# FofanovLab/mtsv_tools

Measured on AMD Instinct MI355X. Metric: reads/sec (whole node), 150bp reads vs MG-index, higher is better.
Workload: dtype u32/i16

## Files before the change

### include/mtsv_amd.h

```cpp
#ifndef MTSV_AMD_H
#define MTSV_AMD_H

#include <stddef.h>
#include <stdint.h>

#ifdef __cplusplus
extern "C" {
#endif

#define MTSV_OK 0
#define MTSV_E_ARG (-1)
#define MTSV_E_IO (-2)
#define MTSV_E_FORMAT (-3)
#define MTSV_E_DEVICE (-4)
#define MTSV_E_LIMIT (-5)
#define MTSV_E_NOMEM (-6)

typedef struct mtsv_index mtsv_index;
typedef struct mtsv_batch mtsv_batch;

typedef struct {
    double edit_rate;
    uint32_t seed_size;
    uint32_t seed_interval;
    double min_seed;
    uint64_t max_hits;
    uint64_t tune_max_hits;
    int64_t max_assignments;
    int64_t max_candidates;
} mtsv_params;

typedef struct {
    uint64_t read;
    uint32_t tax_id;
    uint32_t gi;
    uint32_t edit;
    uint8_t strand;
    uint8_t _pad[3];
    uint64_t offset;
} mtsv_hit;

typedef struct {
    uint64_t n;
    uint64_t n_bins;
    uint32_t occ_k;
    uint64_t sa_s;
    uint64_t file_bytes;
    uint64_t device_bytes;
    uint32_t kmer_k;
    uint32_t sa_full;
} mtsv_index_info_t;

#define MTSV_N_STAGES 8
typedef struct {
    float stage_ms[MTSV_N_STAGES];
    uint64_t n_reads;
    uint64_t n_seed_slots;
    uint64_t n_seed_hits;
    uint64_t lf_steps;
    uint64_t n_candidates;
    uint64_t n_verified;
    uint64_t window_bytes;
    uint64_t n_hits;
    uint64_t n_passes;
    uint64_t n_rounds;
    uint64_t n_lanes;
    uint64_t sw_cell_pairs;
    float sw_prefilter_ms;
    float sw_sweep_ms;
    uint64_t n_sw_passed;
    float sw_diag_ms;
    float sw_bound_ms;
    float edit_ms;
    uint64_t myers_columns;
    uint64_t n_sw_bound_refuted;
    uint64_t verify_turns;
    uint64_t verify_lanes_max;
    uint64_t myers_grid_max;
    uint64_t n_seed_tile_passes;
} mtsv_batch_stats;

const char *mtsv_last_error(void);
const char *mtsv_version(void);
void mtsv_params_default(mtsv_params *p);

int mtsv_device_count(void);

int mtsv_index_load(const char *path, mtsv_index **out);
int mtsv_index_build(uint64_t n_seqs, const uint32_t *tax_ids, const uint32_t *gis,
                     const uint8_t *const *seqs, const uint64_t *seq_lens, uint32_t occ_k,
                     uint64_t sa_s, int n_threads, mtsv_index **out);
int mtsv_index_build_fasta(const char *fasta_path, uint32_t occ_k, uint64_t sa_s, int n_threads,
                           mtsv_index **out);
int mtsv_set_build_device(int hip_device);
int mtsv_index_write(const mtsv_index *ix, const char *path);
int mtsv_index_info(const mtsv_index *ix, mtsv_index_info_t *info);
void mtsv_index_free(mtsv_index *ix);

#define MTSV_DEV_DEFAULT 0u
#define MTSV_DEV_SAMPLED_SA_ONLY 1u
#define MTSV_DEV_NO_KMER_TABLE 2u
#define MTSV_DEV_PACK_ON_DEVICE 4u
int mtsv_index_to_device(mtsv_index *ix, int hip_device, uint32_t flags);


#define MTSV_DEVPART_HEADER 0
#define MTSV_DEVPART_BLOCKS 1
#define MTSV_DEVPART_TEXT 2
#define MTSV_DEVPART_SA_SAMPLE 3
#define MTSV_DEVPART_BINS 4
#define MTSV_DEVPART_BIN_END 5
#define MTSV_DEVPART_BIN_LUT 6
typedef struct {
    uint32_t n, n_blocks;
    uint32_t C[5];
    uint32_t sentinel_row;
    uint32_t sa_s, sa_pow2_shift;
    uint32_t n_bins, bin_lut_shift;
    uint32_t kmer_k;
    uint32_t sa_full;
    uint32_t packed_on_device;
    uint32_t _pad;
    uint64_t device_bytes;
    float pack_ms, copy_ms, accel_build_ms;
    float _pad2;
} mtsv_device_header;
int mtsv_index_download_device(mtsv_index *ix, int hip_device, int part, void **out, uint64_t *bytes);

int mtsv_bin_batch(mtsv_index *ix, int hip_device, const uint8_t *bases, const uint64_t *read_off,
                   uint64_t n_reads, const mtsv_params *params, mtsv_hit **hits, uint64_t *n_hits);
void mtsv_hits_free(mtsv_hit *hits);
void *mtsv_host_alloc(size_t bytes);
void mtsv_host_free(void *p);
int mtsv_host_register(void *p, size_t bytes);
int mtsv_host_unregister(void *p);
int mtsv_bin_batch_multi(mtsv_index *ix, const int *devices, int n_devices, const uint8_t *bases,
                         const uint64_t *read_off, uint64_t n_reads, const mtsv_params *params,
                         mtsv_hit **hits, uint64_t *n_hits);
int mtsv_bin_batch_chunks(mtsv_index *const *chunks, const int *devices, int n_chunks,
                          const uint8_t *bases, const uint64_t *read_off, uint64_t n_reads,
                          const mtsv_params *params, mtsv_hit **hits, uint64_t *n_hits);
uint64_t mtsv_bin_batch_workspace_reads(uint64_t n_reads);

int mtsv_batch_create(mtsv_index *ix, int hip_device, uint64_t max_reads, uint64_t max_bases,
                      uint64_t max_hits_ws, mtsv_batch **out);
int mtsv_batch_create_lanes(mtsv_index *ix, int hip_device, uint64_t max_reads, uint64_t max_bases,
                            uint64_t max_hits_ws, int lanes, mtsv_batch **out);
int mtsv_batch_reserve_host(mtsv_batch *b, uint64_t n_reads, uint64_t n_bases, uint32_t warm_read_len);
#define MTSV_VERIFY_REFERENCE 0
#define MTSV_VERIFY_EDIT_FIRST 1
int mtsv_batch_set_verify_mode(mtsv_batch *b, int mode);
int mtsv_set_default_verify_mode(int mode);
int mtsv_batch_upload(mtsv_batch *b, const uint8_t *bases, const uint64_t *read_off,
                      uint64_t n_reads);
int mtsv_batch_run(mtsv_batch *b, const mtsv_params *params);
int mtsv_batch_run_host(mtsv_batch *b, const uint8_t *bases, const uint64_t *read_off,
                        uint64_t n_reads, const mtsv_params *params);
int mtsv_batch_run_host_parts(mtsv_batch *b, int n_parts, const uint8_t *const *bases, const uint64_t *const *read_off,
                              const uint64_t *n_reads, const mtsv_params *params);
int mtsv_batch_stats_get(const mtsv_batch *b, mtsv_batch_stats *st);

typedef struct {
    uint32_t tax_id;
    uint32_t _pad;
    uint64_t only_hit, only_best, tied_best, not_best;
} mtsv_taxon_stats;
int mtsv_batch_set_taxa_report(mtsv_batch *b, int on);
int mtsv_batch_taxa_report(mtsv_batch *b, mtsv_taxon_stats **rows, uint64_t *n_rows, uint64_t *total_reads,
                           float *device_ms, int reset);
int mtsv_merge_taxa_reports(const mtsv_taxon_stats *a, uint64_t n_a, const mtsv_taxon_stats *b, uint64_t n_b,
                            mtsv_taxon_stats **out, uint64_t *n_out);
int mtsv_format_taxa_report(const mtsv_taxon_stats *rows, uint64_t n_rows, uint64_t total_reads, char **out,
                            uint64_t *out_len);

#define MTSV_MATCH_OFF 0
#define MTSV_MATCH_WITH_HITS 1
#define MTSV_MATCH_ONLY 2
int mtsv_batch_set_match_flags(mtsv_batch *b, int mode);
int mtsv_batch_match_flags(mtsv_batch *b, uint64_t **words, uint64_t *n_reads, uint64_t *n_matched);

#define MTSV_KEEP_UNMATCHED 0
#define MTSV_KEEP_MATCHED 1
int mtsv_batch_take_reads(mtsv_batch *dst, mtsv_batch *src, int keep, uint64_t *n_kept, uint64_t *bases_kept,
                          float *device_ms);
int mtsv_batch_copy_reads(mtsv_batch *dst, mtsv_batch *src, float *device_ms);
int mtsv_batch_merge_runs(mtsv_batch *dst, mtsv_batch *const *srcs, int n_srcs, float *device_ms);
int mtsv_batch_read_map(mtsv_batch *b, uint64_t **map, uint64_t *n_reads);
int mtsv_batch_download_reads(mtsv_batch *b, uint8_t **codes, uint64_t **read_off, uint64_t *n_reads);
int mtsv_batch_download(mtsv_batch *b, mtsv_hit **hits, uint64_t *n_hits);

typedef struct {
    uint64_t read;
    uint32_t tax_id;
    uint32_t edit;
} mtsv_assignment;
#define MTSV_ASSIGN_OFF 0
#define MTSV_ASSIGN_WITH_HITS 1
#define MTSV_ASSIGN_ONLY 2
int mtsv_batch_set_assignments(mtsv_batch *b, int mode);
int mtsv_batch_download_assignments(mtsv_batch *b, mtsv_assignment **a, uint64_t *n, float *device_ms);
#define MTSV_GRAIN_TAXID 0
#define MTSV_GRAIN_TAXID_GI 1
#define MTSV_GRAIN_LONG 2
int mtsv_batch_set_assignment_grain(mtsv_batch *b, int grain);
typedef struct {
    uint64_t read;
    uint32_t tax_id, gi, offset, edit;
} mtsv_assignment_gi;
int mtsv_batch_download_assignments_gi(mtsv_batch *b, mtsv_assignment_gi **a, uint64_t *n, float *device_ms);
void mtsv_batch_free(mtsv_batch *b);

typedef struct mtsv_fold mtsv_fold;
int mtsv_fold_create(int hip_device, int grain, mtsv_fold **out);
void mtsv_fold_free(mtsv_fold *f);
int mtsv_fold_reset(mtsv_fold *f, uint64_t n_reads);
int mtsv_fold_add_run(mtsv_fold *f, mtsv_batch *src, float *device_ms);
int mtsv_fold_add_records(mtsv_fold *f, const void *records, uint64_t n, float *device_ms);
int mtsv_fold_count(const mtsv_fold *f, uint64_t *n);
int mtsv_fold_download(mtsv_fold *f, mtsv_assignment **a, uint64_t *n);
int mtsv_fold_download_gi(mtsv_fold *f, mtsv_assignment_gi **a, uint64_t *n);
int mtsv_fold_taxa_report(mtsv_fold *f, mtsv_taxon_stats **rows, uint64_t *n_rows, uint64_t *total_reads, float *device_ms);
int mtsv_fold_match_flags(mtsv_fold *f, uint64_t **words, uint64_t *n_reads, uint64_t *n_matched);

int mtsv_fold_add_text(mtsv_fold *f, const char *hits, const uint64_t *line_off, const uint32_t *line_read, uint64_t n_lines,
                       uint64_t *n_tokens, uint64_t *n_records, float *device_ms);

int mtsv_fold_format_text(mtsv_fold *f, const char *ids, const uint64_t *id_off, uint64_t n_reads, char **text, uint64_t *len,
                          float *device_ms);
int mtsv_batch_format_text(mtsv_batch *b, const char *ids, const uint64_t *id_off, uint64_t n_reads, char **text, uint64_t *len,
                           float *device_ms);

typedef struct mtsv_dupmap mtsv_dupmap;
int mtsv_dupmap_create(int hip_device, mtsv_dupmap **out);
void mtsv_dupmap_free(mtsv_dupmap *m);
int mtsv_batch_take_unique(mtsv_batch *dst, mtsv_batch *src, mtsv_dupmap *m, uint64_t *n_unique, uint64_t *bases_kept,
                           float *device_ms);
int mtsv_dupmap_download(const mtsv_dupmap *m, uint64_t **read, uint64_t **rep, uint64_t *n_reads, uint64_t *n_unique);
int mtsv_fold_expand(mtsv_fold *dst, mtsv_fold *src, const mtsv_dupmap *m, float *device_ms);

#define MTSV_RANK_UNKNOWN 0xffffffffu
typedef struct mtsv_taxonomy mtsv_taxonomy;
typedef struct {
    uint64_t n_nodes;
    uint64_t n_implied_roots;
    uint32_t n_ranks;
    uint32_t max_depth;
} mtsv_taxonomy_info_t;
int mtsv_taxonomy_load(const char *nodes_dmp, mtsv_taxonomy **out);
void mtsv_taxonomy_free(mtsv_taxonomy *tx);
int mtsv_taxonomy_info(const mtsv_taxonomy *tx, mtsv_taxonomy_info_t *info);
int mtsv_taxonomy_parent(const mtsv_taxonomy *tx, uint32_t tax_id, uint32_t *parent, uint32_t *rank);
const char *mtsv_taxonomy_rank_name(const mtsv_taxonomy *tx, uint32_t rank);
typedef struct {
    uint32_t tax_id, parent_tax_id, rank, depth;
    uint64_t direct, clade;
} mtsv_clade_stats;
int mtsv_fold_lca(mtsv_fold *f, const mtsv_taxonomy *tx, uint32_t edit_slack, mtsv_fold *out, mtsv_clade_stats **rows,
                  uint64_t *n_rows, uint64_t *total_reads, float *device_ms);
int mtsv_format_clade_report(const mtsv_clade_stats *rows, uint64_t n_rows, uint64_t total_reads, const mtsv_taxonomy *tx,
                             char **out, uint64_t *out_len);

#define MTSV_PAIR_BOTH 0
#define MTSV_PAIR_EITHER 1
#define MTSV_PAIR_PROPER 2
typedef struct {
// ... 42 lines not shown
```

### mtsv_tools_amd/__init__.py

```python
from ._lib import (
    ASSIGN_DTYPE,
    ASSIGN_GI_DTYPE,
    ASSIGN_OFF,
    ASSIGN_ONLY,
    ASSIGN_WITH_HITS,
    CLADE_STATS_DTYPE,
    Coverage,
    DEVPART_BIN_END,
    DEVPART_BIN_LUT,
    DEVPART_BINS,
    DEVPART_BLOCKS,
    DEVPART_HEADER,
    DEVPART_SA_SAMPLE,
    DEVPART_TEXT,
    DeviceHeader,
    GRAIN_LONG,
    GRAIN_TAXID,
    GRAIN_TAXID_GI,
    HIT_DTYPE,
    KEEP_MATCHED,
    KEEP_UNMATCHED,
    MATCH_OFF,
    MATCH_ONLY,
    MATCH_WITH_HITS,
    RANK_UNKNOWN,
    REF_COVERAGE_DTYPE,
    SLACK_ALL,
    TAXON_STATS_DTYPE,
    Taxonomy,
    HostBuffer,
    host_register,
    host_unregister,
    Batch,
    DupMap,
    Fold,
    MGIndex,
    MtsvError,
    PAIR_BOTH,
    PAIR_EITHER,
    PAIR_PROPER,
    PairStats,
    Params,
    bin_batch_chunks,
    bin_batch_multi,
    bin_batch_slice_reads,
    default_params,
    device_count,
    format_assignments,
    format_assignments_gi,
    format_clade_report,
    format_coverage_report,
    format_results,
    format_taxa_report,
    merge_taxa_reports,
    lib,
    lib_path,
    pack_bases,
    set_build_device,
    synth_reads,
    version,
)

DEV_DEFAULT = 0
DEV_SAMPLED_SA_ONLY = 1
DEV_NO_KMER_TABLE = 2
DEV_PACK_ON_DEVICE = 4
```

### mtsv_tools_amd/_lib.py

```python
import ctypes as C
import os

import numpy as np

_HERE = os.path.dirname(os.path.abspath(__file__))


def lib_path():
    return os.environ.get("MTSV_AMD_LIB") or os.path.join(_HERE, "libmtsv_amd.so")


class MtsvError(RuntimeError):
    def __init__(self, code, msg):
        super().__init__(f"mtsv error {code}: {msg}")
        self.code = code


E_ARG, E_IO, E_FORMAT, E_DEVICE, E_LIMIT, E_NOMEM = -1, -2, -3, -4, -5, -6
MATCH_OFF, MATCH_WITH_HITS, MATCH_ONLY = 0, 1, 2
ASSIGN_OFF, ASSIGN_WITH_HITS, ASSIGN_ONLY = 0, 1, 2
GRAIN_TAXID, GRAIN_TAXID_GI, GRAIN_LONG = 0, 1, 2
KEEP_UNMATCHED, KEEP_MATCHED = 0, 1
DEVPART_HEADER, DEVPART_BLOCKS, DEVPART_TEXT, DEVPART_SA_SAMPLE, DEVPART_BINS, DEVPART_BIN_END, DEVPART_BIN_LUT = range(7)


class Params(C.Structure):
    _fields_ = [("edit_rate", C.c_double), ("seed_size", C.c_uint32), ("seed_interval", C.c_uint32),
                ("min_seed", C.c_double), ("max_hits", C.c_uint64), ("tune_max_hits", C.c_uint64),
                ("max_assignments", C.c_int64), ("max_candidates", C.c_int64)]


class IndexInfo(C.Structure):
    _fields_ = [("n", C.c_uint64), ("n_bins", C.c_uint64), ("occ_k", C.c_uint32),
                ("sa_s", C.c_uint64), ("file_bytes", C.c_uint64), ("device_bytes", C.c_uint64),
                ("kmer_k", C.c_uint32), ("sa_full", C.c_uint32)]


class DeviceHeader(C.Structure):
    _fields_ = [("n", C.c_uint32), ("n_blocks", C.c_uint32), ("C", C.c_uint32 * 5), ("sentinel_row", C.c_uint32),
                ("sa_s", C.c_uint32), ("sa_pow2_shift", C.c_uint32), ("n_bins", C.c_uint32), ("bin_lut_shift", C.c_uint32),
                ("kmer_k", C.c_uint32), ("sa_full", C.c_uint32), ("packed_on_device", C.c_uint32), ("_pad", C.c_uint32),
                ("device_bytes", C.c_uint64), ("pack_ms", C.c_float), ("copy_ms", C.c_float), ("accel_build_ms", C.c_float),
                ("_pad2", C.c_float)]


N_STAGES = 8
STAGE_NAMES = ("search", "thin_scan", "expand", "locate", "coalesce", "verify", "gather", "total")


class BatchStats(C.Structure):
    _fields_ = [("stage_ms", C.c_float * N_STAGES), ("n_reads", C.c_uint64),
                ("n_seed_slots", C.c_uint64), ("n_seed_hits", C.c_uint64), ("lf_steps", C.c_uint64),
                ("n_candidates", C.c_uint64), ("n_verified", C.c_uint64),
                ("window_bytes", C.c_uint64), ("n_hits", C.c_uint64), ("n_passes", C.c_uint64),
                ("n_rounds", C.c_uint64), ("n_lanes", C.c_uint64), ("sw_cell_pairs", C.c_uint64), ("sw_prefilter_ms", C.c_float),
                ("sw_sweep_ms", C.c_float), ("n_sw_passed", C.c_uint64), ("sw_diag_ms", C.c_float), ("sw_bound_ms", C.c_float),
                ("edit_ms", C.c_float), ("myers_columns", C.c_uint64), ("n_sw_bound_refuted", C.c_uint64),
                ("verify_turns", C.c_uint64), ("verify_lanes_max", C.c_uint64), ("myers_grid_max", C.c_uint64),
                ("n_seed_tile_passes", C.c_uint64)]

    def as_dict(self):
        d = {n: (float(getattr(self, n)) if t is C.c_float else int(getattr(self, n))) for n, t in self._fields_[1:]}
        d["stage_ms"] = {STAGE_NAMES[i]: float(self.stage_ms[i]) for i in range(N_STAGES)}
        return d


HIT_DTYPE = np.dtype({"names": ["read", "tax_id", "gi", "edit", "strand", "offset"],
                      "formats": ["<u8", "<u4", "<u4", "<u4", "u1", "<u8"],
                      "offsets": [0, 8, 12, 16, 20, 24], "itemsize": 32})

TAXON_STATS_DTYPE = np.dtype({"names": ["tax_id", "only_hit", "only_best", "tied_best", "not_best"],
                              "formats": ["<u4", "<u8", "<u8", "<u8", "<u8"],
                              "offsets": [0, 8, 16, 24, 32], "itemsize": 40})

ASSIGN_DTYPE = np.dtype({"names": ["read", "tax_id", "edit"], "formats": ["<u8", "<u4", "<u4"], "offsets": [0, 8, 12], "itemsize": 16})

ASSIGN_GI_DTYPE = np.dtype({"names": ["read", "tax_id", "gi", "offset", "edit"], "formats": ["<u8", "<u4", "<u4", "<u4", "<u4"],
                            "offsets": [0, 8, 12, 16, 20], "itemsize": 24})

CLADE_STATS_DTYPE = np.dtype({"names": ["tax_id", "parent_tax_id", "rank", "depth", "direct", "clade"],
                              "formats": ["<u4", "<u4", "<u4", "<u4", "<u8", "<u8"], "offsets": [0, 4, 8, 12, 16, 24], "itemsize": 32})
RANK_UNKNOWN = 0xffffffff
SLACK_ALL = 0xffffffff
PAIR_BOTH, PAIR_EITHER, PAIR_PROPER = 0, 1, 2

REF_COVERAGE_DTYPE = np.dtype({"names": ["tax_id", "gi", "length", "reads", "alignments", "aligned_bases", "covered_bases"],
                               "formats": ["<u4", "<u4", "<u8", "<u8", "<u8", "<u8", "<u8"], "offsets": [0, 4, 8, 16, 24, 32, 40], "itemsize": 48})


class TaxonomyInfo(C.Structure):
    _fields_ = [("n_nodes", C.c_uint64), ("n_implied_roots", C.c_uint64), ("n_ranks", C.c_uint32), ("max_depth", C.c_uint32)]


class PairStats(C.Structure):
    _fields_ = [("pairs", C.c_uint64), ("both_mates_hit", C.c_uint64), ("one_mate_hit", C.c_uint64), ("joined", C.c_uint64),
                ("records", C.c_uint64)]

    def as_dict(self):
        return {n: int(getattr(self, n)) for n, _ in self._fields_}


EXPORTS = [
    "mtsv_last_error", "mtsv_version", "mtsv_params_default", "mtsv_device_count",
    "mtsv_index_load", "mtsv_index_build", "mtsv_index_build_fasta", "mtsv_index_write",
    "mtsv_index_info", "mtsv_index_free", "mtsv_set_build_device", "mtsv_index_to_device", "mtsv_bin_batch",
    "mtsv_hits_free", "mtsv_batch_create", "mtsv_batch_upload", "mtsv_batch_run", "mtsv_batch_run_host", "mtsv_batch_run_host_parts",
    "mtsv_batch_stats_get", "mtsv_batch_set_verify_mode", "mtsv_batch_download", "mtsv_batch_free", "mtsv_format_results",
    "mtsv_free", "mtsv_synth_index", "mtsv_synth_reads", "mtsv_bin_batch_workspace_reads",
    "mtsv_bin_batch_multi", "mtsv_bin_batch_chunks", "mtsv_set_default_verify_mode",
    "mtsv_host_alloc", "mtsv_host_free", "mtsv_host_register", "mtsv_host_unregister",
    "mtsv_batch_create_lanes", "mtsv_batch_reserve_host", "mtsv_pack_bases", "mtsv_host_pack_threads",
    "mtsv_batch_set_taxa_report", "mtsv_batch_taxa_report", "mtsv_merge_taxa_reports", "mtsv_format_taxa_report",
    "mtsv_batch_set_match_flags", "mtsv_batch_match_flags",
    "mtsv_batch_take_reads", "mtsv_batch_read_map", "mtsv_batch_download_reads",
    "mtsv_batch_copy_reads", "mtsv_batch_merge_runs",
    "mtsv_batch_set_assignments", "mtsv_batch_download_assignments", "mtsv_format_assignments",
    "mtsv_batch_set_assignment_grain", "mtsv_batch_download_assignments_gi", "mtsv_format_assignments_gi",
    "mtsv_fold_create", "mtsv_fold_free", "mtsv_fold_reset", "mtsv_fold_add_run", "mtsv_fold_add_records", "mtsv_fold_count",
    "mtsv_fold_download", "mtsv_fold_download_gi", "mtsv_fold_taxa_report", "mtsv_fold_match_flags",
    "mtsv_fold_format_text", "mtsv_batch_format_text",
    "mtsv_index_download_device",
    "mtsv_fold_add_text",
    "mtsv_taxonomy_load", "mtsv_taxonomy_free", "mtsv_taxonomy_info", "mtsv_taxonomy_parent", "mtsv_taxonomy_rank_name",
    "mtsv_fold_lca", "mtsv_format_clade_report",
    "mtsv_dupmap_create", "mtsv_dupmap_free", "mtsv_batch_take_unique", "mtsv_dupmap_download", "mtsv_fold_expand",
    "mtsv_fold_pair",
    "mtsv_coverage_create", "mtsv_coverage_free", "mtsv_coverage_add_index", "mtsv_coverage_add_refs", "mtsv_coverage_reset",
    "mtsv_coverage_add_fold", "mtsv_coverage_rows", "mtsv_format_coverage_report",
]

_lib = None


def lib():
    global _lib
    if _lib is None:
        p = lib_path()
        if not os.path.exists(p):
            raise MtsvError(E_DEVICE, f"{p} is missing: run `make -C mtsv_tools_amd/csrc` "
                                      "(or __graft_entry__.build()); there is no fallback path")
        L = C.CDLL(p)
        vp, u64, u32, i32 = C.c_void_p, C.c_uint64, C.c_uint32, C.c_int
        L.mtsv_last_error.restype = C.c_char_p
        L.mtsv_version.restype = C.c_char_p
        L.mtsv_params_default.argtypes = [C.POINTER(Params)]
        L.mtsv_index_load.argtypes = [C.c_char_p, C.POINTER(vp)]
        L.mtsv_index_build.argtypes = [u64, vp, vp, vp, vp, u32, u64, i32, C.POINTER(vp)]
        L.mtsv_index_build_fasta.argtypes = [C.c_char_p, u32, u64, i32, C.POINTER(vp)]
        L.mtsv_index_write.argtypes = [vp, C.c_char_p]
        L.mtsv_index_info.argtypes = [vp, C.POINTER(IndexInfo)]
        L.mtsv_index_free.argtypes = [vp]
        L.mtsv_index_free.restype = None
        L.mtsv_index_to_device.argtypes = [vp, i32, u32]
        L.mtsv_index_download_device.argtypes = [vp, i32, i32, C.POINTER(vp), C.POINTER(u64)]
        L.mtsv_bin_batch.argtypes = [vp, i32, vp, vp, u64, C.POINTER(Params), C.POINTER(vp),
                                     C.POINTER(u64)]
        L.mtsv_hits_free.argtypes = [vp]
        L.mtsv_hits_free.restype = None
        L.mtsv_bin_batch_multi.argtypes = [vp, vp, i32, vp, vp, u64, C.POINTER(Params), C.POINTER(vp), C.POINTER(u64)]
        L.mtsv_bin_batch_chunks.argtypes = [vp, vp, i32, vp, vp, u64, C.POINTER(Params), C.POINTER(vp), C.POINTER(u64)]
        L.mtsv_bin_batch_workspace_reads.argtypes = [u64]
        L.mtsv_bin_batch_workspace_reads.restype = u64
        L.mtsv_batch_create.argtypes = [vp, i32, u64, u64, u64, C.POINTER(vp)]
        L.mtsv_batch_create_lanes.argtypes = [vp, i32, u64, u64, u64, i32, C.POINTER(vp)]
        L.mtsv_batch_reserve_host.argtypes = [vp, u64, u64, u32]
        L.mtsv_pack_bases.argtypes = [vp, vp, u64, u64, C.c_uint8]
        L.mtsv_pack_bases.restype = C.c_uint8
        L.mtsv_batch_upload.argtypes = [vp, vp, vp, u64]
        L.mtsv_batch_run.argtypes = [vp, C.POINTER(Params)]
        L.mtsv_batch_run_host.argtypes = [vp, vp, vp, u64, C.POINTER(Params)]
        L.mtsv_batch_run_host_parts.argtypes = [vp, i32, vp, vp, vp, C.POINTER(Params)]
        L.mtsv_batch_set_verify_mode.argtypes = [vp, i32]
        L.mtsv_batch_stats_get.argtypes = [vp, C.POINTER(BatchStats)]
        L.mtsv_batch_download.argtypes = [vp, C.POINTER(vp), C.POINTER(u64)]
        L.mtsv_batch_free.argtypes = [vp]
        L.mtsv_batch_free.restype = None
# ... 759 lines not shown
```

### mtsv_tools_amd/csrc/batch.hip

```cpp
#include <atomic>
#include <chrono>
#include <cmath>
#include <condition_variable>
#include <exception>
#include <mutex>
#include <thread>
#include <cstdio>
#include <cstdlib>
#include <cstring>
#include <stdexcept>
#include <vector>

#include "batch.hpp"

namespace mtsv {

namespace {
template <class F>
void parallel_ranges(uint64_t n, F f) {
    static const int max_nt = [] {
        const char* e = getenv("MTSV_COPY_THREADS");
        return e ? std::max(1, std::min(16, atoi(e))) : 4;
    }();
    const int nt = std::min(max_nt, n >= (32ull << 20) ? 4 : n >= (4ull << 20) ? 2 : 1);
    if (nt == 1) return f(0, n);
    std::vector<std::thread> th;
    const uint64_t chunk = ((n + nt - 1) / nt + 4095) & ~4095ull;
    for (int k = 0; k < nt; k++) {
        uint64_t a = std::min(n, chunk * k), b = std::min(n, chunk * (k + 1));
        if (a < b) th.emplace_back([=] { f(a, b); });
    }
    for (auto& t : th) t.join();
}
double now_s() { return std::chrono::duration<double>(std::chrono::steady_clock::now().time_since_epoch()).count(); }
void parallel_copy(uint8_t* dst, const uint8_t* src, uint64_t n) {
    parallel_ranges(n, [=](uint64_t a, uint64_t b) { memcpy(dst + a, src + a, b - a); });
}
}

bool host_pinned(const void* p, uint64_t bytes) {
    if (!p || !bytes) return false;
    for (const uint8_t* q : {(const uint8_t*)p, (const uint8_t*)p + bytes - 1}) {
        hipPointerAttribute_t at;
        memset(&at, 0, sizeof at);
        if (hipPointerGetAttributes(&at, q) != hipSuccess) {
            (void)hipGetLastError();
            return false;
        }
        if (at.type != hipMemoryTypeHost) return false;
    }
    return true;
}

void* host_pinned_alloc(uint64_t bytes) {
    void* p = nullptr;
    if (hipHostMalloc(&p, bytes ? bytes : 1, hipHostMallocPortable) != hipSuccess) {
        (void)hipGetLastError();
        return nullptr;
    }
    return p;
}
void host_pinned_free(void* p) {
    if (p && hipHostFree(p) != hipSuccess) (void)hipGetLastError();
}
bool host_pinned_register(void* p, uint64_t bytes) {
    if (hipHostRegister(p, bytes, hipHostRegisterPortable) == hipSuccess) return true;
    (void)hipGetLastError();
    return false;
}
bool host_pinned_unregister(void* p) {
    if (hipHostUnregister(p) == hipSuccess) return true;
    (void)hipGetLastError();
    return false;
}

int g_default_verify_mode = MTSV_VERIFY_REFERENCE;

constexpr uint32_t kMyersWgsPerCuLanes = 3;
constexpr uint64_t kChunkMaxReads = 4ull << 20;

Batch::Batch(mtsv_index* ix_, DeviceIndex* di_, uint64_t max_reads_, uint64_t max_bases_, uint64_t hit_cap_, Batch* parent_, int lanes_)
    : ix(ix_), di(di_), max_reads(max_reads_), max_bases(max_bases_), hit_cap(hit_cap_), parent(parent_) {
    if (max_reads == 0) max_reads = 1;
    if (max_reads > 0x7fffffffull) throw std::runtime_error("limit: more than 2^31 reads in one batch");
    if (max_bases >= 0xffffffffull) throw std::runtime_error("limit: 4 GiB of bases or more in one batch");
    const uint64_t hit_cap_user = hit_cap;
    if (!parent) {
        n_lanes = 3;
        if (lanes_ > 0) n_lanes = std::min(8, lanes_);
        else if (const char* e = getenv("MTSV_LANES")) n_lanes = std::max(1, std::min(8, atoi(e)));
        if (max_reads < (uint64_t)n_lanes * kLaneMinReads) n_lanes = 1;
    }
    ws_reads = (max_reads + n_lanes - 1) / n_lanes;
    if (!parent && n_lanes > 1) {
        uint64_t cmax = kChunkMaxReads;
        if (const char* e = getenv("MTSV_CHUNK")) cmax = std::max<uint64_t>(kLaneMinReads, strtoull(e, nullptr, 10));
        ws_reads = std::min(ws_reads, cmax);
    }
    if (hit_cap == 0) hit_cap = std::max<uint64_t>(1ull << 20, 32 * ws_reads);
    if (hit_cap > 0xfffffff0ull) hit_cap = 0xfffffff0ull;
    uint64_t hits_cap = std::max<uint64_t>(1ull << 20, 16 * ws_reads);
    if (const char* e = getenv("MTSV_HITS_CAP")) hits_cap = std::max<uint64_t>(1024, strtoull(e, nullptr, 10));
    HIP_CHECK(hipSetDevice(di->device));
    stream.create(hipStreamNonBlocking);
    const uint64_t ns = 2 * ws_reads;
    if (!parent) {
        d_bases.alloc(max_bases + 64, "the resident bases");
        d_read_off.alloc(max_reads + 1, "the resident read offsets");
        d_codes.alloc(max_bases + 64, "the resident codes");
    }
    d_strand_hits.alloc(ns + 1, "strands: seed hits");
    d_strand_nseeds.alloc(ns, "strands: seeds kept");
    d_strand_off.alloc(ns + 1, "strands: seed-hit offsets");
    d_strand_ncand.alloc(ns, "strands: candidates");
    d_strand_nout.alloc(ns + 1, "strands: hits");
    d_heavy_list.alloc(2 * ns, "strands: lists");
    d_out_off.alloc(ns + 1, "strands: hit offsets");
    d_tile_sums.alloc((uint64_t)scan_tiles((uint32_t)ns) + 1, "the scans' tile sums");
    d_counters.alloc(kCounters, "the pass counters");
    hit_cap_first = hit_cap;
    size_hit_workspace(hit_cap_first);
    d_hits.alloc(hits_cap, "the result array");
    h_counters.renew(kCounters, hipHostMallocMapped);
    if (const char* e = getenv("MTSV_SW")) sw_pairs = strcmp(e, "packed") != 0;
    if (const char* e = getenv("MTSV_SW_DIAG")) sw_diag = atoi(e) != 0;
    if (const char* e = getenv("MTSV_SW_PREPASS")) sw_prepass = atoi(e) != 0;
    if (const char* e = getenv("MTSV_SW_TOP")) sw_top = atoi(e) != 0;
    if (const char* e = getenv("MTSV_SW_BOUND")) sw_bound = atoi(e) != 0;
    if (const char* e = getenv("MTSV_SW_FUSED")) sw_fused = atoi(e) != 0;
    verify_mode = g_default_verify_mode;
    if (const char* e = getenv("MTSV_VERIFY")) verify_mode = !strcmp(e, "edit_first") ? 1 : 0;
    if (!parent) {
        myers_wgs_per_cu = n_lanes > 1 ? kMyersWgsPerCuLanes : kMyersWgsPerCuMax;
        if (const char* e = getenv("MTSV_MYERS_WGS_PER_CU")) myers_wgs_per_cu = (uint32_t)std::max(1, std::min((int)kMyersWgsPerCuMax, atoi(e)));
        verify_turn.on = n_lanes > 1;
        if (const char* e = getenv("MTSV_VERIFY_TURN")) verify_turn.on = verify_turn.on && atoi(e) != 0;
        if (const char* e = getenv("MTSV_TAIL_FROM_LIST")) tail_from_list = atoi(e) != 0;
        if (const char* e = getenv("MTSV_FUSED_CLEAR")) fused_clear = atoi(e) != 0;
        if (const char* e = getenv("MTSV_SEED_STAGE")) seed_tiles = strcmp(e, "legacy") != 0;
    } else {
        myers_wgs_per_cu = parent->myers_wgs_per_cu;
        tail_from_list = parent->tail_from_list;
        fused_clear = parent->fused_clear;
        seed_tiles = parent->seed_tiles;
    }
    ev.create();
    for (int k = 1; k < n_lanes; k++) extra.emplace_back(new Batch(ix, di, ws_reads, 0, hit_cap_user, this));
}

Batch::~Batch() {
    extra.clear();
    (void)hipSetDevice(di->device);
    for (hipStream_t s : {stream.s, copy_stream.s, copy_stream2.s})
        if (s) (void)hipStreamSynchronize(s);
    if (h_hits_stage) pinned_hits_release(h_hits_stage);
    if (h_assign_stage) pinned_hits_release(h_assign_stage);
}

void Batch::size_hit_workspace(uint64_t cap) {
    hit_cap = 0;
    release_all(d_hit_row, d_hit_ref, d_hit_q, d_hit_key, d_cand_tmp, d_cand, d_out, d_cand_next, d_cand_status, d_worklist);
    d_hit_row.alloc(cap, "hit workspace: rows");
    d_hit_ref.alloc(cap, "hit workspace: references");
    d_hit_q.alloc(cap, "hit workspace: read positions");
    d_hit_key.alloc(cap, "hit workspace: keys");
    d_cand_tmp.alloc(2 * cap, "hit workspace: candidate scratch");
    d_cand.alloc(cap, "hit workspace: candidates");
    d_out.alloc(cap, "hit workspace: verified candidates");
    d_cand_next.alloc(cap, "hit workspace: successors");
    d_cand_status.alloc(cap, "hit workspace: status");
    d_worklist.alloc(cap, "hit workspace: work list");
    hit_cap = cap;
}

void Batch::grow_hit_workspace(uint64_t need) {
    if (getenv("MTSV_TRACE")) fprintf(stderr, "[workspace] seed-hit arrays grow %llu -> %llu entries\n", (unsigned long long)hit_cap, (unsigned long long)need);
    HIP_CHECK(hipStreamSynchronize(stream));
    size_hit_workspace(need);
}

void Batch::VerifyTurn::enter(uint64_t first_read, const Batch* lane) {
    std::unique_lock<std::mutex> lk(mu);
    if (on) {
        const std::pair<uint64_t, const Batch*> me{first_read, lane};
        waiting.push_back(me);
        cv.wait(lk, [&] { return !held && *std::min_element(waiting.begin(), waiting.end()) == me; });
        waiting.erase(std::find(waiting.begin(), waiting.end(), me));
        held = true;
        taken++;
    }
    max_in_verify = std::max(max_in_verify, ++in_verify);
}

void Batch::VerifyTurn::leave() {
    {
        std::lock_guard<std::mutex> lk(mu);
        in_verify--;
        held = false;
    }
    cv.notify_all();
}

void Batch::VerifyTurn::note_grid(uint32_t blocks) {
    std::lock_guard<std::mutex> lk(mu);
    myers_grid_max = std::max<uint64_t>(myers_grid_max, blocks);
}

void Batch::upload(const uint8_t* bases, const uint64_t* read_off, uint64_t n) {
    if (n > max_reads) throw std::runtime_error("arg: batch holds more reads than the workspace was created for");
    const uint64_t first = n ? read_off[0] : 0;
    const uint64_t nb = n ? read_off[n] - first : 0;
    if (nb > max_bases) throw std::runtime_error("arg: batch holds more bases than the workspace was created for");
    h_read_off.resize(n + 1);
    max_len = 0;
    for (uint64_t i = 0; i <= n; i++) {
        if (i && read_off[i] < read_off[i - 1]) throw std::runtime_error("arg: read_off is not ascending");
        h_read_off[i] = (uint32_t)(read_off[i] - first);
        if (i) max_len = std::max(max_len, h_read_off[i] - h_read_off[i - 1]);
    }
    if (n == 0) h_read_off[0] = 0;
    HIP_CHECK(hipSetDevice(di->device));
    if (nb) HIP_CHECK(hipMemcpyAsync(d_bases.p, bases + first, nb, hipMemcpyHostToDevice, stream));
    HIP_CHECK(hipMemcpyAsync(d_read_off.p, h_read_off.data(), (n + 1) * 4, hipMemcpyHostToDevice, stream));
    HIP_CHECK(hipStreamSynchronize(stream));
    n_reads = n;
    n_hits_total = 0;
    total_hits = 0;
    segments.clear();
    last_run = kRunNone;
    resident = true;
    codes_resident = mapped = false;
}

void Batch::reset_lane() {
    HIP_CHECK(hipSetDevice(di->device));
    memset(&stats, 0, sizeof stats);
    memset(stage_acc, 0, sizeof stage_acc);
    sw_ms_acc = 0;
    sweep_ms_acc = diag_ms_acc = bound_ms_acc = edit_ms_acc = 0;
    sw_passed_acc = 0;
    n_hits_total = 0;
    n_assign_total = 0;
    if (!hit_cap) size_hit_workspace(hit_cap_first);
    HIP_CHECK(hipMemsetAsync(d_counters.p, 0, kCounters * sizeof(uint64_t), stream));
    listed_zero = true;
    HIP_CHECK(hipEventRecord(ev[kEvRunBegin], stream));
}

void Batch::finish_lane() {
    HIP_CHECK(hipEventRecord(ev[kEvRunEnd], stream));
    launch_publish(stream, d_counters.p, h_counters.p, kCounters);
    HIP_CHECK(hipStreamSynchronize(stream));
    HIP_CHECK(hipEventElapsedTime(&stage_acc[7], ev[kEvRunBegin], ev[kEvRunEnd]));
    if (getenv("MTSV_TRACE")) fprintf(stderr, "[lane] last pass: %llu strands of 13..64 seed hits (or more than 4 candidates) to k_coalesce_mid, %llu heavier ones\n",
                                      (unsigned long long)(h_counters.p[kCtrMidStrands] & 0xffffffffull), (unsigned long long)(h_counters.p[kCtrWorklist] >> 32));
    if (getenv("MTSV_TRACE")) fprintf(stderr, "[lane] k_coalesce_heavy: %llu strands walked by runs, %llu by the wavefront walk (a run too long)\n",
                                      (unsigned long long)(h_counters.p[kCtrHeavyWalk] & 0xffffffffull), (unsigned long long)(h_counters.p[kCtrHeavyWalk] >> 32));
    stats.sw_cell_pairs = h_counters.p[kCtrSwCellPairs];
    stats.sw_prefilter_ms = sw_ms_acc;
    stats.sw_sweep_ms = sweep_ms_acc;
    stats.sw_diag_ms = diag_ms_acc;
    stats.sw_bound_ms = bound_ms_acc;
    stats.edit_ms = edit_ms_acc;
    stats.myers_columns = h_counters.p[kCtrMyersColumns];
    stats.n_sw_bound_refuted = h_counters.p[kCtrBoundRefuted];
    stats.n_sw_passed = sw_passed_acc + h_counters.p[kCtrListPassed];
    stats.lf_steps = h_counters.p[kCtrLfSteps];
    stats.n_candidates = h_counters.p[kCtrCandidates];
    stats.n_verified = h_counters.p[kCtrVerified];
    stats.window_bytes = h_counters.p[kCtrWindowBytes];
}

void Batch::begin_run(const mtsv_params& p, uint64_t read_base) {
    if (!(p.edit_rate >= 0.0 && p.edit_rate <= 1.0)) throw std::runtime_error("arg: edit_rate must be within [0, 1]");
    if (!(p.min_seed >= 0.0) || !std::isfinite(p.min_seed)) throw std::runtime_error("arg: min_seed must be finite and >= 0");
    if (p.seed_size == 0 || p.seed_interval == 0) throw std::runtime_error("arg: seed_size and seed_interval must be > 0");
    segments.clear();
    total_hits = 0;
    lanes_used = 1;
    staged_valid = false;
    assign_staged_valid = false;
    staged_assign = 0;
    host_hits_dropped = false;
    last_run = kRunNone;
    run_t0 = now_s();
    {
        std::lock_guard<std::mutex> lk(verify_turn.mu);
        verify_turn.taken = verify_turn.max_in_verify = verify_turn.myers_grid_max = 0;
    }
    reset_lane();
    for (auto& l : extra) {
        l->verify_mode = verify_mode;
        l->sw_pairs = sw_pairs;
        l->sw_diag = sw_diag;
        l->sw_prepass = sw_prepass;
        l->sw_top = sw_top;
        l->sw_bound = sw_bound;
// ... 1235 lines not shown
```

### mtsv_tools_amd/csrc/batch.hpp

```cpp
#pragma once
#include <condition_variable>
#include <memory>
#include <mutex>
#include <vector>

#include "../../include/mtsv_amd.h"
#include "host_pack.hpp"
#include "dev_index.hpp"
#include "dev_mem.hpp"
#include "kernels.hpp"

namespace mtsv {

struct Batch {
    mtsv_index* ix;
    DeviceIndex* di;
    DevStream stream, copy_stream, copy_stream2;
    mtsv_hit* h_hits_stage = nullptr;
    uint64_t h_hits_cap = 0, staged_hits = 0, last_total_hits = 0;
    bool staged_valid = false;
    struct Arena {
        DevBuf<uint8_t> d_bases;
        DevBuf<uint8_t> d_packed;
        DevBuf<uint32_t> d_off;
        uint64_t cap_bases = 0, cap_reads = 0;
        void resize(int k, uint64_t bases, uint64_t reads);
    };
    static constexpr uint64_t kArenaBases = 3ull << 30;
    static constexpr uint64_t kArenaReads = 1ull << 30;
    Arena arena[2];
    HostBuf<uint32_t> h_off_all;
    static constexpr int kStage = 4;
    HostBuf<uint8_t> h_stage[kStage];
    DevEventList chunk_ev;
    std::mutex* commit_mu = nullptr;
    uint64_t max_reads, max_bases;
    uint64_t hit_cap, hit_cap_first = 0;
    Batch* parent = nullptr;
    Batch* root() { return parent ? parent : this; }
    const Batch* root() const { return parent ? parent : this; }
    std::vector<std::unique_ptr<Batch>> extra;
    int n_lanes = 1;
    uint64_t ws_reads = 0;
    struct Segment {
        Batch* lane;
        uint64_t offset, count;
        uint64_t first_read = 0, n_reads = 0;
        uint64_t a_offset = 0, a_count = 0;
    };
    std::vector<Segment> segments;
    uint64_t total_hits = 0;
    double run_t0 = 0;
    uint64_t lanes_used = 1;

    DevBuf<uint8_t> d_codes;
    DevBuf<uint8_t> d_bases;
    DevBuf<uint32_t> d_read_off;
    DevBuf<uint32_t> d_seed_lo, d_seed_cnt, d_seed_pre;
    uint64_t seed_cap = 0;
    DevBuf<uint32_t> d_strand_hits, d_strand_nseeds, d_strand_off, d_strand_ncand, d_worklist, d_strand_nout, d_out_off;
    DevBuf<uint64_t> d_tile_sums;
    DevBuf<uint64_t> d_counters;
    DevBuf<uint32_t> d_hit_row, d_hit_ref, d_hit_q;
    DevBuf<uint64_t> d_hit_key, d_cand_tmp;
    DevBuf<uint4> d_cand, d_out;
    DevBuf<uint32_t> d_cand_next, d_cand_status, d_heavy_list;
    DevBuf<DevHit> d_hits;
    DevBuf<uint2> d_strip;
    DevBuf<uint32_t> d_planes;
    HostBuf<uint64_t> h_counters;
    enum Ev {
        kEvPassBegin = 0, kEvSearched, kEvSeeded, kEvExpanded, kEvLocated, kEvCoalesced, kEvVerified, kEvGathered,
        kEvRunBegin, kEvRunEnd,
        kEvSwBegin, kEvSwEnd,
        kEvDiagEnd,
        kEvBoundEnd,
        kEvEditEnd,
        kEvCount
    };
    DevEvents<kEvCount> ev;
    float sw_ms_acc = 0, sweep_ms_acc = 0, diag_ms_acc = 0, bound_ms_acc = 0, edit_ms_acc = 0;
    uint64_t sw_passed_acc = 0;

    std::vector<uint32_t> h_read_off;
    uint32_t max_len = 0;
    static constexpr int kCounters = kCtrCount;
    double listed_share = 0.125;
    bool sw_diag = true;
    bool sw_top = true;
    bool sw_bound = true;
    bool sw_fused = true;
    bool sw_prepass = true;
    bool sw_pairs = true;
    uint32_t myers_wgs_per_cu = kMyersWgsPerCuMax;
    bool tail_from_list = true;
    bool fused_clear = true;
    bool seed_tiles = true;
    bool listed_zero = false;
    struct VerifyTurn {
        bool on = false;
        std::mutex mu;
        std::condition_variable cv;
        bool held = false;
        std::vector<std::pair<uint64_t, const Batch*>> waiting;
        uint64_t taken = 0, in_verify = 0, max_in_verify = 0, myers_grid_max = 0;
        void enter(uint64_t first_read, const Batch* lane);
        void leave();
        void note_grid(uint32_t blocks);
        struct Guard {
            VerifyTurn* t = nullptr;
            Guard() = default;
            Guard(const Guard&) = delete;
            Guard& operator=(const Guard&) = delete;
            ~Guard() { release(); }
            void take(VerifyTurn& turn, uint64_t first_read, const Batch* lane) {
                if (t) return;
                turn.enter(first_read, lane);
                t = &turn;
            }
            void release() {
                if (t) t->leave();
                t = nullptr;
            }
        };
    };
    VerifyTurn verify_turn;
    int verify_mode = 0;
    uint64_t n_reads = 0;
    uint64_t n_hits_total = 0;
    mtsv_batch_stats stats{};
    float stage_acc[MTSV_N_STAGES] = {0};

    Batch(mtsv_index* ix, DeviceIndex* di, uint64_t max_reads, uint64_t max_bases, uint64_t hit_cap, Batch* parent = nullptr, int lanes = 0);
    ~Batch();
    Batch(const Batch&) = delete;
    Batch& operator=(const Batch&) = delete;

    void upload(const uint8_t* bases, const uint64_t* read_off, uint64_t n);
    void run(const mtsv_params& p);
    void run_host(const uint8_t* bases, const uint64_t* read_off, uint64_t n, const mtsv_params& p, uint64_t read_base = 0);
    struct HostPart {
        const uint8_t* bases;
        const uint64_t* read_off;
        uint64_t n;
    };
    void run_host_parts(const HostPart* parts, int n_parts, const mtsv_params& p, uint64_t read_base = 0);
    void reserve_host(uint64_t n, uint64_t n_bases);
    void download(mtsv_hit** hits, uint64_t* n);
    void download_into(mtsv_hit* dst, uint64_t n);
    bool keep_on_device = false;

    struct TaxaReport {
        bool on = false;
        bool dense = true;
        uint32_t hash_slots = kReportHashSlots;
        uint32_t n_taxa = 0;
        DevBuf<uint32_t> d_taxa;
        DevBuf<uint64_t> d_counts;
        bool trace = false;
        uint64_t launches = 0;
        std::vector<uint32_t> h_taxa;
        std::mutex mu;
        float ms = 0;
    };
    TaxaReport report;
    DevEvents<2> report_ev;
    void set_taxa_report(bool on);
    struct MatchFlags {
        int mode = MTSV_MATCH_OFF;
        DevBuf<uint64_t> d_words;
        uint64_t cap_words() const { return d_words.p ? d_words.cap - 1 : 0; }
        uint64_t n_reads = 0;
        uint64_t call_base = 0;
        bool trace = false;
        std::mutex mu;
        float ms = 0;
        uint64_t launches = 0;
    };
    MatchFlags match;
    DevEvents<2> match_ev;
    bool flags_only() const { return root()->match.mode == MTSV_MATCH_ONLY; }
    void set_match_flags(int mode);
    void match_flags(std::vector<uint64_t>& words, uint64_t* n_reads, uint64_t* n_matched);
    enum LastRun { kRunNone = 0, kRunResident, kRunHostOneSegment, kRunHostSegments, kRunMerged };
    int last_run = kRunNone;
    bool resident = false;
    bool codes_resident = false;
    bool mapped = false;
    DevBuf<uint32_t> d_read_map;
    DevBuf<uint64_t> d_compact;
    uint64_t compact_cap() const { return d_compact.p ? (d_compact.cap - 3) / 2 : 0; }
    DevEvents<4> compact_ev;
    void compact_room(uint64_t tiles);
    void take_reads(Batch& src, int keep, uint64_t* n_kept, uint64_t* bases_kept, float* device_ms);
    void copy_reads(Batch& src, float* device_ms);
    struct MergeState {
        DevBuf<uint32_t> d_nout, d_off;
        DevBuf<uint64_t> d_tiles;
        uint64_t cap_reads = 0;
        uint64_t cap_tiles() const { return d_tiles.cap - 2; }
        DevBuf<uint32_t> d_lo, d_base;
        uint64_t cap_sn = 0;
        DevBuf<MergePart> d_parts;
        DevEvents<2> ev;
    };
    MergeState merge;
    struct Assignments {
        int mode = MTSV_ASSIGN_OFF;
        int grain = MTSV_GRAIN_TAXID;
        uint64_t rec_bytes() const { return grain == MTSV_GRAIN_TAXID ? sizeof(mtsv_assignment) : sizeof(mtsv_assignment_gi); }
        uint64_t key_bytes() const { return grain == MTSV_GRAIN_TAXID ? 8 : 16; }
        uint32_t lane_max = kCollapseLaneMax, wave_max = 64, lds_max = kCollapseLdsKeys;
        bool trace = false;
        std::mutex mu;
        float ms = 0;
        uint64_t launches = 0;
        uint64_t tiers[5] = {0, 0, 0, 0, 0};
    };
    Assignments assign;
    uint8_t* h_assign_stage = nullptr;
    uint64_t h_assign_cap = 0, staged_assign = 0, last_total_assign = 0;
    bool assign_staged_valid = false;
    bool host_hits_dropped = false;
    void assign_stage_reserve(uint64_t n_needed);
    DevBuf<uint8_t> d_assign;
    uint64_t n_assign_total = 0;
    struct CollapseScratch {
        DevBuf<uint64_t> keys;
        uint64_t key_bytes = 0;
        DevBuf<uint32_t> flags, place;
        DevBuf<uint64_t> tiles;
        uint64_t cap_hits = 0;
        void resize(uint64_t hits, uint64_t key_bytes);
        DevBuf<uint32_t> list;
        uint64_t pending_hits = 0;
        DevBuf<uint64_t> d_ctr;
        HostBuf<uint64_t> h_ctr;
        DevEvents<2> ev;
    };
    CollapseScratch collapse;
    bool assign_only() const { return root()->assign.mode == MTSV_ASSIGN_ONLY; }
    void set_assignments(int mode);
    void set_assignment_grain(int grain);
    void download_assignments(void** a, uint64_t* n, float* device_ms, bool wide);
    std::shared_ptr<struct TextFormatter> text;
    void format_text(const char* ids, const uint64_t* id_off, uint64_t n_reads, char** text_out, uint64_t* len, float* device_ms);
    void merge_runs(Batch* const* srcs, int n_srcs, float* device_ms);
    void read_map(std::vector<uint64_t>& map);
    void download_reads(std::vector<uint8_t>& codes, std::vector<uint64_t>& read_off);
    void taxa_report(std::vector<mtsv_taxon_stats>& rows, uint64_t* total_reads, float* device_ms, bool reset);
// ... 61 lines not shown
```

### mtsv_tools_amd/csrc/batch_pass.hip

```cpp
#include <atomic>
#include <cstdio>
#include <cstdlib>
#include <thread>

#include "batch.hpp"

namespace mtsv {

void Batch::run_range(const mtsv_params& p, const uint8_t* raw, uint8_t* sb, const uint32_t* so, const uint32_t* h_off, uint64_t n,
                      uint32_t range_max_len, uint64_t read_base) {
    std::vector<Batch*> ls{this};
    for (auto& l : extra) ls.push_back(l.get());
    uint64_t per_lane = 2;
    if (const char* e = getenv("MTSV_CHUNKS_PER_LANE")) per_lane = std::max(1, atoi(e));
    const ChunkPlan cp = plan_chunks(n, ls.size(), ws_reads, per_lane);
    const uint64_t n_chunks = cp.n_chunks(), k = cp.k;
    lanes_used = std::max<uint64_t>(lanes_used, k);
    std::vector<Segment> segs(n_chunks);
    std::atomic<uint64_t> next{0};
    auto work = [&](Batch* lane) {
        for (;;) {
            const uint64_t c = next.fetch_add(1);
            if (c >= n_chunks) return;
            const uint64_t a = cp.bound[c], b = cp.bound[c + 1];
// ... 63 lines not shown
        if (getenv("MTSV_TRACE")) fprintf(stderr, "[lane] pass of %u reads, max_ns %u, longest read %u: seed stage %s\n", pl.nr, pl.max_ns, pl.pass_max_len, ps.tile_pass ? "by tiles" : "legacy");
        stats.n_seed_slots += pl.slots;
        stats.n_seed_hits += ps.total_hits;
        stage_locate(ps);
        stage_candidates(ps);
        stage_verify(ps);
        stage_gather(ps);
        stage_commit(ps);
        n_hits_total += ps.total_out;
        for (int s = 0; s < 7; s++) {
            float ms = 0;
            HIP_CHECK(hipEventElapsedTime(&ms, ev[s], ev[s + 1]));
            stage_acc[s] += ms;
        }
        r0 += pl.nr;
    }
}

void Batch::room_seed_slots(const PassPlan& pl) {
    if (pl.slots <= seed_cap) return;
    const uint64_t had = seed_cap;
    seed_cap = 0;
    release_all(d_seed_lo, d_seed_cnt, d_seed_pre);
    const uint64_t want = pl.tiled() ? pl.slots : std::max<uint64_t>(pl.slots, 2 * ws_reads * (uint64_t)pl.max_ns);
    if (getenv("MTSV_TRACE")) fprintf(stderr, "[workspace] seed slot arrays grow %llu -> %llu entries\n", (unsigned long long)had, (unsigned long long)want);
    d_seed_lo.alloc(want, "seed slots: ranges");
    d_seed_cnt.alloc(want, "seed slots: counts");
    d_seed_pre.alloc(want, "seed slots: prefix sums");
    seed_cap = want;
}

void Batch::room_planes(const PassPlan& pl) {
    if ((uint64_t)pl.nr * 3 * pl.plane_words <= d_planes.cap) return;
    d_planes.renew(std::max<uint64_t>(pl.nr, ws_reads) * 3 * pl.plane_words, "the reads' bit planes");
}

void Batch::room_strip(uint64_t need) {
    if (need <= d_strip.cap) return;
    d_strip.renew(need, "the band strips");
}

void Batch::room_hits(uint64_t total_out) {
    if (n_hits_total + total_out <= d_hits.cap) return;
    DevBuf<DevHit> grown;
    grown.alloc(std::max(d_hits.cap * 2, n_hits_total + total_out), "the result array");
    if (n_hits_total) HIP_CHECK(hipMemcpyAsync(grown.p, d_hits.p, n_hits_total * sizeof(DevHit), hipMemcpyDeviceToDevice, stream));
    HIP_CHECK(hipStreamSynchronize(stream));
    std::unique_lock<std::mutex> commit_lk;
    if (root()->commit_mu) commit_lk = std::unique_lock<std::mutex>(*root()->commit_mu);
    if (root()->copy_stream2) HIP_CHECK(hipStreamSynchronize(root()->copy_stream2));
    d_hits.swap(grown);
}

Batch::Seeded Batch::stage_seeds(Pass& ps) {
    const PassPlan& pl = ps.plan;
    const mtsv_params& p = ps.p;
    const uint32_t K = p.seed_size, G = p.seed_interval, r0 = (uint32_t)ps.r0;
    uint32_t* planes = pl.myers() ? d_planes.p : nullptr;
    HIP_CHECK(hipEventRecord(ev[kEvPassBegin], stream));
    const uint32_t listed_cap = (uint32_t)std::min<uint64_t>(pl.slots, std::max<uint64_t>(4096, (uint64_t)((double)pl.slots * listed_share)));
    launch_search(stream, di->view, ps.sb, ps.so, r0, pl.nr, pl.max_ns, K, G, d_seed_lo.p, d_seed_cnt.p, d_seed_pre.p, (uint32_t*)(d_counters.p + kCtrListedSlots),
                  listed_cap, di->d_kmer_levels, fused_clear && listed_zero);
    listed_zero = false;
    HIP_CHECK(hipEventRecord(ev[kEvSearched], stream));
    ps.tile_pass = seed_tiles && pl.max_ns && seed_tile_fits(pl.max_ns, pl.pass_max_len, pl.slots);
    if (ps.tile_pass)
        launch_thin_tiled(stream, ps.sb, ps.so, r0, pl.nr, p.edit_rate, p.min_seed, pl.max_ns, K, G, p.max_hits, p.tune_max_hits, d_seed_cnt.p,
                          d_strand_hits.p, d_strand_nseeds.p, planes, pl.plane_words);
    else if (pl.max_ns)
        launch_thin(stream, ps.sb, ps.so, r0, pl.nr, p.edit_rate, p.min_seed, pl.max_ns, K, G, p.max_hits, p.tune_max_hits, d_seed_cnt.p,
                    d_seed_pre.p, d_strand_hits.p, d_strand_nseeds.p, planes, pl.plane_words);
    else {
        HIP_CHECK(hipMemsetAsync(d_strand_hits.p, 0, (uint64_t)ps.nstr * 4, stream));
        HIP_CHECK(hipMemsetAsync(d_strand_nseeds.p, 0, (uint64_t)ps.nstr * 4, stream));
    }
    launch_scan(stream, d_strand_hits.p, ps.nstr, d_tile_sums.p, d_counters.p + kCtrSeedHits, d_strand_off.p);
    launch_publish(stream, d_counters.p + kCtrSeedHits, h_counters.p + kCtrSeedHits, 1);
    launch_publish(stream, d_counters.p + kCtrListedSlots, h_counters.p + kCtrListedSlots, 1);
    HIP_CHECK(hipEventRecord(ev[kEvSeeded], stream));
    HIP_CHECK(hipStreamSynchronize(stream));
    const uint64_t n_listed = h_counters.p[kCtrListedSlots] & 0xffffffffull;
    const double share = pl.slots ? (double)n_listed / (double)pl.slots : 0.0;
    if (n_listed > listed_cap) {
        listed_share = std::min(1.0, share * 1.25 + 0.01);
        if (getenv("MTSV_TRACE")) fprintf(stderr, "[lane] %llu listed seed slots, grid for %u: pass again\n", (unsigned long long)n_listed, listed_cap);
        return Seeded::kSameReads;
    }
    listed_share = std::min(1.0, std::max(0.02, share * 1.5 + 0.005));
    ps.total_hits = h_counters.p[kCtrSeedHits];
    if (ps.total_hits > hit_cap) {
        if (pl.nr > 1) return Seeded::kHalfReads;
        if (ps.total_hits > 0xfffffff0ull)
            throw std::runtime_error("device: one read has " + std::to_string(ps.total_hits) + " seed hits, more than 2^32");
        grow_hit_workspace(ps.total_hits);
    }
    return Seeded::kGoOn;
}

void Batch::stage_locate(Pass& ps) {
    const DevIndexView& v = di->view;
    if (ps.tile_pass)
        launch_expand_tiled(stream, v, ps.nstr, ps.plan.max_ns, ps.p.seed_interval, d_seed_lo.p, d_seed_cnt.p, d_strand_off.p, d_hit_row.p, d_hit_ref.p, d_hit_q.p);
    else
        launch_expand(stream, v, ps.nstr, ps.plan.max_ns, ps.p.seed_interval, d_seed_lo.p, d_seed_cnt.p, d_seed_pre.p, d_strand_off.p, d_hit_row.p, d_hit_ref.p,
                      d_hit_q.p);
    HIP_CHECK(hipEventRecord(ev[kEvExpanded], stream));
    if (!v.sa_full)
        launch_locate(stream, v, (uint32_t)ps.total_hits, d_strand_off.p + ps.nstr, d_hit_row.p, d_hit_ref.p,
                      (unsigned long long*)(d_counters.p + kCtrLfSteps));
    HIP_CHECK(hipEventRecord(ev[kEvLocated], stream));
}

void Batch::stage_candidates(Pass& ps) {
    if (fused_clear) {
        launch_clear_counters(stream, d_counters.p, kCtrClearPass | (ps.plan.path == VerifyPath::kRounds ? kCtrClearRound0 : 0));
        listed_zero = true;
    } else {
        HIP_CHECK(hipMemsetAsync(d_counters.p + kCtrWorklist, 0, 8, stream));
        HIP_CHECK(hipMemsetAsync(d_counters.p + kCtrWlCursor, 0, 8, stream));
        HIP_CHECK(hipMemsetAsync(d_counters.p + kCtrMidStrands, 0, 8, stream));
    }
    launch_coalesce(stream, di->view, ps.so, (uint32_t)ps.r0, ps.nstr, ps.p.max_candidates, d_strand_off.p,
                    d_strand_nseeds.p, d_hit_ref.p, d_hit_q.p, d_hit_key.p, d_cand_tmp.p, d_cand.p, d_cand_next.p,
                    d_cand_status.p, d_strand_ncand.p, d_worklist.p, d_heavy_list.p, d_counters.p, fused_clear);
    HIP_CHECK(hipEventRecord(ev[kEvCoalesced], stream));
}

void Batch::stage_verify(Pass& ps) {
    const DevIndexView& v = di->view;
    const PassPlan& pl = ps.plan;
    if (ps.total_hits) ps.turn.take(root()->verify_turn, ps.read_base + ps.r0, this);
    EvalArgs a;
    a.bases = ps.sb;
    a.read_off = ps.so;
    a.r0 = (uint32_t)ps.r0;
    a.edit_rate = ps.p.edit_rate;
    a.max_candidates = ps.p.max_candidates;
    a.strand_off = d_strand_off.p;
    a.cand = d_cand.p;
    a.cand_next = d_cand_next.p;
    a.cand_status = d_cand_status.p;
    a.planes = pl.myers() ? d_planes.p : nullptr;
    a.plane_words = pl.plane_words;
    a.out = d_out.p;
    a.n_verified = (unsigned long long*)(d_counters.p + kCtrVerified);
    a.window_bytes = (unsigned long long*)(d_counters.p + kCtrWindowBytes);
    a.sw_columns = (unsigned long long*)(d_counters.p + kCtrSwCellPairs);
    a.worklist = d_worklist.p;
    a.wl_count = (const uint32_t*)(d_counters.p + kCtrWorklist);
    a.wl_cursor = (uint32_t*)(d_counters.p + kCtrWlCursor);
    stats.n_rounds = 1;
    switch (pl.path) {
        case VerifyPath::kTiled: verify_tiled(ps, a); break;
        case VerifyPath::kEditFirst: root()->verify_turn.note_grid(launch_edit_myers(stream, v, a, ps.total_hits, pl.pass_max_len, 0, root()->myers_wgs_per_cu)); break;
        case VerifyPath::kRounds: verify_rounds(ps, a); break;
        case VerifyPath::kPacked: launch_evaluate(stream, v, a, ps.total_hits, pl.pass_max_len); break;
    }
    launch_resolve(stream, ps.nstr, ps.p.max_candidates, flags_only() ? 1 : ps.p.max_assignments, d_strand_off.p, d_strand_ncand.p, d_cand_status.p,
                   d_out.p, d_strand_nout.p);
    HIP_CHECK(hipEventRecord(ev[kEvVerified], stream));
}

void Batch::verify_tiled(Pass& ps, EvalArgs& a) {
    HIP_CHECK(hipMemsetAsync(d_counters.p + kCtrMaxWindow, 0, sizeof(uint64_t), stream));
    launch_max_window(stream, ps.nstr, d_strand_off.p, d_strand_ncand.p, d_cand.p, (unsigned long long*)(d_counters.p + kCtrMaxWindow));
    launch_publish(stream, d_counters.p + kCtrMaxWindow, h_counters.p + kCtrMaxWindow, 1);
    HIP_CHECK(hipStreamSynchronize(stream));
    const uint32_t strip_len = (uint32_t)std::max<uint64_t>(h_counters.p[kCtrMaxWindow], 1);
    room_strip((uint64_t)tiled_groups(ps.total_hits, strip_len) * strip_len);
    a.strip = d_strip.p;
    a.strip_len = strip_len;
    launch_evaluate_tiled(stream, di->view, a, ps.total_hits);
}

struct Batch::Round {
    uint32_t round = 0;
    uint64_t items = 0;
    uint64_t tail_items = 0;
    bool tail_listed = false;
    bool fused = false;
    EvalArgs sw;
    uint32_t *pass_list = nullptr, *sweep_list = nullptr, *next_list = nullptr;
    uint64_t* next_slot = nullptr;
};

void Batch::verify_rounds(Pass& ps, const EvalArgs& a) {
    Round r;
    r.fused = sw_bound && sw_fused;
    r.pass_list = (uint32_t*)d_hit_key.p;
    r.sweep_list = (uint32_t*)d_hit_key.p + hit_cap;
    uint32_t* next_lists[2] = {(uint32_t*)d_cand_tmp.p, (uint32_t*)d_cand_tmp.p + hit_cap};
    const uint32_t* wl = d_worklist.p;
    uint32_t wl_slot = kCtrWorklist;
    r.items = ps.total_hits;
    for (;; r.round++) {
        r.next_slot = d_counters.p + kCtrNext0 + (r.round & 1);
        r.next_list = next_lists[r.round & 1];
        if (!fused_clear) {
            HIP_CHECK(hipMemsetAsync(d_counters.p + kCtrSwCursor, 0, 3 * sizeof(uint64_t), stream));
            HIP_CHECK(hipMemsetAsync(r.next_slot, 0, sizeof(uint64_t), stream));
        } else if (r.round) {
            launch_clear_counters(stream, d_counters.p, ctr_clear_round(r.round));
        }
        r.tail_items = r.items;
        r.tail_listed = tail_from_list && r.round > 0;
        r.sw = a;
        r.sw.worklist = wl;
        r.sw.wl_count = (const uint32_t*)(d_counters.p + wl_slot);
        r.sw.wl_cursor = (uint32_t*)(d_counters.p + kCtrSwCursor);
        r.sw.wl_reverse = r.round == 0;
        r.sw.counters = d_counters.p;
        r.sw.wl_count_slot = wl_slot;
        r.sw.pass_list = r.pass_list;
        r.sw.pass_count = (uint32_t*)(d_counters.p + kCtrPassCount);
#ifdef MTSV_SW_HIST
        if (!d_strip.p) room_strip(4096);
        HIP_CHECK(hipMemsetAsync(d_strip.p, 0, 768 * 4, stream));
        r.sw.strip = d_strip.p;
#endif
        if (r.round == 0) {
            HIP_CHECK(hipEventRecord(ev[kEvSwBegin], stream));
            if (sw_diag && sw_prepass && !r.fused) round0_diag(ps, r);
            if (sw_bound) round0_bound(ps, r);
            else if (sw_diag && sw_prepass && sw_top) round0_top(ps, r);
        }
        round_tail(ps, r, a);
        if (r.round == 0) round0_times();
        const uint64_t n_next = h_counters.p[kCtrNext0] & 0xffffffffull;
        if (n_next == 0) break;
        stats.n_rounds++;
        wl = r.next_list;
        wl_slot = kCtrNext0 + (r.round & 1);
        r.items = n_next;
    }
    ps.turn.release();
}

void Batch::round0_diag(Pass& ps, Round& r) {
    HIP_CHECK(hipMemsetAsync(d_counters.p + kCtrSweepCount, 0, sizeof(uint64_t), stream));
    launch_sw_diag(stream, di->view, r.sw, r.items, ps.plan.pass_max_len, r.sweep_list, kCtrSweepCount);
    HIP_CHECK(hipEventRecord(ev[kEvDiagEnd], stream));
    r.sw.worklist = r.sweep_list;
    r.sw.wl_count_slot = kCtrSweepCount;
    r.sw.wl_reverse = 0;
}

void Batch::round0_bound(Pass& ps, Round& r) {
    if (!fused_clear) HIP_CHECK(hipMemsetAsync(d_counters.p + kCtrUndecided, 0, 2 * sizeof(uint64_t), stream));
    EvalArgs bd = r.sw;
    bd.wl_count = (const uint32_t*)(d_counters.p + r.sw.wl_count_slot);
    bd.wl_cursor = (uint32_t*)(d_counters.p + kCtrBoundCursor);
    bd.und_list = (uint32_t*)d_hit_row.p;
    bd.und_slot = kCtrUndecided;
    bd.myers_ctr = (unsigned long long*)(d_counters.p + kCtrMyersColumns);
    root()->verify_turn.note_grid(launch_edit_myers(stream, di->view, bd, r.items, ps.plan.pass_max_len, r.fused ? 3 : 2, root()->myers_wgs_per_cu));
    HIP_CHECK(hipEventRecord(ev[kEvBoundEnd], stream));
    r.sw.worklist = bd.und_list;
    r.sw.wl_count_slot = kCtrUndecided;
    r.sw.wl_reverse = 0;
    if (r.fused && tail_from_list) {
        launch_publish(stream, d_counters.p + kCtrUndecided, h_counters.p + kCtrUndecided, 1);
        HIP_CHECK(hipStreamSynchronize(stream));
        r.tail_items = h_counters.p[kCtrUndecided] & 0xffffffffull;
        r.tail_listed = true;
    }
}

void Batch::round0_top(Pass& ps, Round& r) {
    HIP_CHECK(hipMemsetAsync(d_counters.p + kCtrUndecided, 0, sizeof(uint64_t), stream));
    r.sw.und_list = (uint32_t*)d_hit_row.p;
    r.sw.und_slot = kCtrUndecided;
    launch_sw_pairs(stream, di->view, r.sw, r.items, ps.plan.pass_max_len, false, true);
    HIP_CHECK(hipMemsetAsync(d_counters.p + kCtrSwCursor, 0, sizeof(uint64_t), stream));
    r.sw.worklist = r.sw.und_list;
    r.sw.wl_count_slot = kCtrUndecided;
}

void Batch::round_tail(Pass& ps, Round& r, const EvalArgs& a) {
    const DevIndexView& v = di->view;
    const uint32_t max_len = ps.plan.pass_max_len;
    const bool first = r.round == 0, tail_empty = r.tail_listed && r.tail_items == 0;
    if (!tail_empty) launch_sw_pairs(stream, v, r.sw, r.tail_items, max_len, sw_diag, false, first && sw_bound && !r.tail_listed);
#ifdef MTSV_SW_HIST
    {
        static uint32_t hh[768];
        HIP_CHECK(hipMemcpyAsync(hh, d_strip.p, sizeof hh, hipMemcpyDeviceToHost, stream));
        HIP_CHECK(hipStreamSynchronize(stream));
        fprintf(stderr, "SWHIST round %u steps/4:", r.round);
        for (int i = 0; i < 128; i++) if (hh[i]) fprintf(stderr, " %d:%u", i * 4, hh[i]);
        fprintf(stderr, "\nSWHIST halves sweeping 0/1/2: %u %u %u\nSWHIST fail best:", hh[128], hh[129], hh[130]);
        for (int i = 0; i < 256; i++) if (hh[256 + i]) fprintf(stderr, " %d:%u", i, hh[256 + i]);
        fprintf(stderr, "\nSWHIST pass best:");
        for (int i = 0; i < 256; i++) if (hh[512 + i]) fprintf(stderr, " %d:%u", i, hh[512 + i]);
        fprintf(stderr, "\n");
    }
#endif
    if (first) HIP_CHECK(hipEventRecord(ev[kEvSwEnd], stream));
    EvalArgs my = a;
    my.worklist = r.pass_list;
    my.wl_count = (const uint32_t*)(d_counters.p + kCtrPassCount);
    my.wl_cursor = (uint32_t*)(d_counters.p + kCtrMyersCursor);
    my.next_list = r.next_list;
    my.next_count = (uint32_t*)r.next_slot;
    my.myers_ctr = (unsigned long long*)(d_counters.p + kCtrMyersColumns);
    if (!tail_empty) root()->verify_turn.note_grid(launch_edit_myers(stream, v, my, r.tail_items, max_len, 1, root()->myers_wgs_per_cu, r.tail_listed));
    if (first) HIP_CHECK(hipEventRecord(ev[kEvEditEnd], stream));
    if (tail_empty) {
        h_counters.p[kCtrPassCount] = h_counters.p[kCtrNext0] = 0;
        if (first) HIP_CHECK(hipEventSynchronize(ev[kEvEditEnd]));
    } else {
        launch_publish(stream, r.next_slot, h_counters.p + kCtrNext0, 1);
        launch_publish(stream, d_counters.p + kCtrPassCount, h_counters.p + kCtrPassCount, 1);
        HIP_CHECK(hipStreamSynchronize(stream));
    }
    sw_passed_acc += h_counters.p[kCtrPassCount] & 0xffffffffull;
}

void Batch::round0_times() {
    float ms = 0;
    HIP_CHECK(hipEventElapsedTime(&ms, ev[kEvSwBegin], ev[kEvSwEnd]));
    sw_ms_acc += ms;
    int from = kEvSwBegin;
    if (sw_diag && sw_prepass && !(sw_bound && sw_fused)) {
        HIP_CHECK(hipEventElapsedTime(&ms, ev[kEvSwBegin], ev[kEvDiagEnd]));
        diag_ms_acc += ms;
        from = kEvDiagEnd;
    }
    if (sw_bound) {
        HIP_CHECK(hipEventElapsedTime(&ms, ev[from], ev[kEvBoundEnd]));
        bound_ms_acc += ms;
        from = kEvBoundEnd;
    }
    HIP_CHECK(hipEventElapsedTime(&ms, ev[from], ev[kEvSwEnd]));
    sweep_ms_acc += ms;
    HIP_CHECK(hipEventElapsedTime(&ms, ev[kEvSwEnd], ev[kEvEditEnd]));
    edit_ms_acc += ms;
}

void Batch::stage_gather(Pass& ps) {
    const bool only_flags = flags_only();
    if (!only_flags) {
        launch_scan(stream, d_strand_nout.p, ps.nstr, d_tile_sums.p, d_counters.p + kCtrOutTotal, d_out_off.p);
        launch_publish(stream, d_counters.p, h_counters.p, kCtrWlCursor + 1);
        HIP_CHECK(hipStreamSynchronize(stream));
        ps.total_out = h_counters.p[kCtrOutTotal];
        ps.turn.release();
    }
    room_hits(ps.total_out);
    if (!only_flags) launch_gather(stream, ps.nstr, ps.read_base + ps.r0, d_strand_off.p, d_strand_nout.p, d_out_off.p, d_out.p, d_hits.p, n_hits_total);
    if (!only_flags && root()->mapped) launch_remap_reads(stream, d_hits.p + n_hits_total, ps.total_out, root()->d_read_map.p);
    HIP_CHECK(hipEventRecord(ev[kEvGathered], stream));
}

void Batch::stage_commit(Pass& ps) {
    const uint32_t nr = ps.plan.nr;
    TaxaReport& rep = root()->report;
    if (rep.on) {
        if (!report_ev.created()) report_ev.create();
        HIP_CHECK(hipEventRecord(report_ev[0], stream));
        launch_report(stream, nr, d_strand_nout.p, d_out_off.p, d_hits.p + n_hits_total, rep.d_taxa.p, rep.n_taxa, rep.dense, rep.hash_slots, rep.d_counts.p,
                      rep.d_counts.p + 4ull * rep.n_taxa, rep.trace ? rep.d_counts.p + 4ull * rep.n_taxa + 1 : nullptr);
        HIP_CHECK(hipEventRecord(report_ev[1], stream));
    }
    MatchFlags& mf = root()->match;
    if (mf.mode != MTSV_MATCH_OFF) {
        const uint64_t first_bit = ps.read_base + ps.r0 - mf.call_base;
        if (first_bit + nr > mf.n_reads) throw std::runtime_error("internal: match flags of a pass beyond the run's reads");
        if (!match_ev.created()) match_ev.create();
        HIP_CHECK(hipEventRecord(match_ev[0], stream));
        launch_match(stream, nr, d_strand_nout.p, first_bit, mf.d_words.p, mf.d_words.p + mf.cap_words());
        HIP_CHECK(hipEventRecord(match_ev[1], stream));
    }
    const bool collapse_on = !flags_only() && root()->assign.mode != MTSV_ASSIGN_OFF;
    if (collapse_on) collapse_enqueue(nr, d_strand_nout.p, d_out_off.p, d_hits.p + n_hits_total, ps.total_out);
    HIP_CHECK(hipStreamSynchronize(stream));
    HIP_CHECK(hipGetLastError());
    ps.turn.release();
    if (collapse_on) collapse_commit();
    if (mf.mode != MTSV_MATCH_OFF) {
        float ms = 0;
        HIP_CHECK(hipEventElapsedTime(&ms, match_ev[0], match_ev[1]));
        std::lock_guard<std::mutex> lk(mf.mu);
        mf.ms += ms;
        mf.launches++;
    }
    if (rep.on) {
        float ms = 0;
        HIP_CHECK(hipEventElapsedTime(&ms, report_ev[0], report_ev[1]));
        std::lock_guard<std::mutex> lk(rep.mu);
        rep.ms += ms;
        rep.launches++;
    }
}

}
```

### mtsv_tools_amd/csrc/capi.cpp

```cpp
#include <algorithm>
#include <cstdio>
#include <cstdlib>
#include <cstring>
#include <memory>
#include <stdexcept>
#include <string>
#include <thread>
#include <vector>

#include "../../include/mtsv_amd.h"
#include "batch.hpp"
#include "cover.hpp"
#include "dedup.hpp"
#include "dev_index.hpp"
#include "fold.hpp"
#include "mgindex.hpp"

using namespace mtsv;

static thread_local std::string g_err;
static int g_build_device = -1;

static int fail(const std::exception& e) {
    g_err = e.what();
// ... 81 lines not shown
    }
}
}

extern "C" {

const char* mtsv_last_error(void) { return g_err.c_str(); }
const char* mtsv_version(void) { return "mtsv_tools_amd 0.1.0 (gfx950)"; }

void mtsv_params_default(mtsv_params* p) {
    p->edit_rate = 0.13;
    p->seed_size = 18;
    p->seed_interval = 15;
    p->min_seed = 0.015;
    p->max_hits = 2000;
    p->tune_max_hits = 200;
    p->max_assignments = -1;
    p->max_candidates = -1;
}

int mtsv_device_count(void) {
    int n = 0;
    if (hipGetDeviceCount(&n) != hipSuccess) return 0;
    return n;
}

int mtsv_index_load(const char* path, mtsv_index** out) {
    if (!path || !out) return fail_arg("null argument");
    GUARD({
        auto ix = std::make_unique<mtsv_index>();
        load_index(path, ix->host);
        *out = ix.release();
    })
}

int mtsv_index_build(uint64_t n_seqs, const uint32_t* tax_ids, const uint32_t* gis, const uint8_t* const* seqs,
                     const uint64_t* seq_lens, uint32_t occ_k, uint64_t sa_s, int n_threads, mtsv_index** out) {
    if (!out || (n_seqs && (!tax_ids || !gis || !seqs || !seq_lens))) return fail_arg("null argument");
    GUARD({
        std::vector<SeqEntry> e(n_seqs);
        for (uint64_t i = 0; i < n_seqs; i++) e[i] = SeqEntry{tax_ids[i], gis[i], seqs[i], seq_lens[i]};
        auto ix = std::make_unique<mtsv_index>();
        build_index(std::move(e), occ_k, sa_s, n_threads, ix->host, g_build_device);
        *out = ix.release();
    })
}

int mtsv_set_build_device(int hip_device) {
    g_build_device = hip_device;
    return MTSV_OK;
}

int mtsv_index_build_fasta(const char* fasta_path, uint32_t occ_k, uint64_t sa_s, int n_threads, mtsv_index** out) {
    if (!fasta_path || !out) return fail_arg("null argument");
    GUARD({
        auto ix = std::make_unique<mtsv_index>();
        build_index_from_fasta(fasta_path, occ_k, sa_s, n_threads, ix->host, g_build_device);
        *out = ix.release();
    })
}

int mtsv_index_write(const mtsv_index* ix, const char* path) {
    if (!ix || !path) return fail_arg("null argument");
    GUARD({
        write_index(ix->host, path);
        const_cast<mtsv_index*>(ix)->host.file_bytes = 0;
    })
}

int mtsv_index_info(const mtsv_index* ix, mtsv_index_info_t* info) {
    if (!ix || !info) return fail_arg("null argument");
    info->n = ix->host.n();
    info->n_bins = ix->host.bins.size();
    info->occ_k = ix->host.k;
    info->sa_s = ix->host.s;
    info->file_bytes = ix->host.file_bytes;
    info->device_bytes = 0;
    info->kmer_k = 0;
    info->sa_full = 0;
    for (auto& kv : ix->dev) {
        info->device_bytes = kv.second->bytes;
        info->kmer_k = kv.second->view.kmer_tab ? kv.second->view.kmer_k : 0;
        info->sa_full = kv.second->view.sa_full ? 1 : 0;
    }
    return MTSV_OK;
}

void mtsv_index_free(mtsv_index* ix) {
    if (!ix) return;
    for (auto& kv : ix->cached_batch) delete kv.second->b;
    delete ix;
}

int mtsv_index_to_device(mtsv_index* ix, int hip_device, uint32_t flags) {
    if (!ix) return fail_arg("null index");
    GUARD({
        std::lock_guard<std::mutex> lk(ix->mu);
        auto it = ix->dev.find(hip_device);
        if (it == ix->dev.end() || it->second->flags != flags) {
            for (auto cb = ix->cached_batch.begin(); cb != ix->cached_batch.end();) {
                if (cb->first.first == hip_device) {
                    {
                        std::lock_guard<std::mutex> wl(cb->second->mu);
                        delete cb->second->b;
                        cb->second->b = nullptr;
                    }
                    cb = ix->cached_batch.erase(cb);
                } else
                    ++cb;
            }
            if (it != ix->dev.end()) ix->dev.erase(it);
            ix->dev[hip_device] = upload_index(ix->host, hip_device, flags);
        }
    })
}

static DeviceIndex* device_index(mtsv_index* ix, int dev) {
    auto it = ix->dev.find(dev);
    if (it == ix->dev.end()) throw std::runtime_error("arg: index is not resident on device " + std::to_string(dev) + " (call mtsv_index_to_device)");
    return it->second.get();
}

int mtsv_index_download_device(mtsv_index* ix, int hip_device, int part, void** out, uint64_t* bytes) {
    if (!ix || !out || !bytes) return fail_arg("null argument");
    GUARD({
        std::lock_guard<std::mutex> lk(ix->mu);
        const DeviceIndex* di = device_index(ix, hip_device);
        const DevIndexView& v = di->view;
        mtsv_device_header h;
        memset(&h, 0, sizeof h);
        const void* src = nullptr;
        uint64_t len = 0;
        switch (part) {
        case MTSV_DEVPART_HEADER:
            h.n = v.n;
            h.n_blocks = v.n_blocks;
            for (int a = 0; a < 5; a++) h.C[a] = v.C[a];
            h.sentinel_row = v.sentinel_row;
            h.sa_s = v.sa_s;
            h.sa_pow2_shift = v.sa_pow2_shift;
            h.n_bins = v.n_bins;
            h.bin_lut_shift = v.bin_lut_shift;
            h.kmer_k = v.kmer_tab ? v.kmer_k : 0;
            h.sa_full = v.sa_full ? 1 : 0;
            h.packed_on_device = di->packed_on_device ? 1 : 0;
            h.device_bytes = di->bytes;
            h.pack_ms = di->pack_ms;
            h.copy_ms = di->copy_ms;
            h.accel_build_ms = di->accel_build_ms;
            len = sizeof h;
            break;
        case MTSV_DEVPART_BLOCKS: src = di->d_blocks, len = (uint64_t)v.n_blocks * sizeof(RankBlock); break;
        case MTSV_DEVPART_TEXT: src = di->d_text, len = di->text_bytes; break;
        case MTSV_DEVPART_SA_SAMPLE: src = di->d_sa_sample, len = di->sa_sample_bytes; break;
        case MTSV_DEVPART_BINS: src = di->d_bins, len = (uint64_t)v.n_bins * sizeof(DevBin); break;
        case MTSV_DEVPART_BIN_END: src = di->d_bin_end, len = (uint64_t)v.n_bins * 4; break;
        case MTSV_DEVPART_BIN_LUT: src = di->d_bin_lut, len = di->bin_lut_bytes; break;
        default: throw std::runtime_error("arg: unknown MTSV_DEVPART_* " + std::to_string(part));
        }
        void* p = malloc(len ? len : 1);
        if (!p) throw std::bad_alloc();
        if (part == MTSV_DEVPART_HEADER) {
            memcpy(p, &h, sizeof h);
        } else if (len) {
            hipError_t e = hipSetDevice(hip_device);
            if (e == hipSuccess) e = hipMemcpy(p, src, len, hipMemcpyDeviceToHost);
            if (e != hipSuccess) {
                free(p);
                throw std::runtime_error(std::string("device: ") + hipGetErrorString(e) + " at mtsv_index_download_device");
            }
        }
        *out = p;
        *bytes = len;
    })
}

int mtsv_batch_create(mtsv_index* ix, int hip_device, uint64_t max_reads, uint64_t max_bases, uint64_t max_hits_ws,
                      mtsv_batch** out) {
    if (!ix || !out) return fail_arg("null argument");
    GUARD({
        std::lock_guard<std::mutex> lk(ix->mu);
        *out = new mtsv_batch(ix, device_index(ix, hip_device), max_reads, max_bases, max_hits_ws);
    })
}

int mtsv_batch_create_lanes(mtsv_index* ix, int hip_device, uint64_t max_reads, uint64_t max_bases, uint64_t max_hits_ws, int lanes,
                            mtsv_batch** out) {
    if (!ix || !out || lanes < 0) return fail_arg("null argument");
    GUARD({
        std::lock_guard<std::mutex> lk(ix->mu);
        *out = new mtsv_batch(ix, device_index(ix, hip_device), max_reads, max_bases, max_hits_ws, nullptr, lanes);
    })
}

int mtsv_batch_reserve_host(mtsv_batch* b, uint64_t n_reads, uint64_t n_bases, uint32_t warm_read_len) {
    if (!b) return fail_arg("null argument");
    GUARD({
        b->impl.reserve_host(n_reads, n_bases);
        struct ReportOff {
            bool& on;
            const bool was;
            explicit ReportOff(bool& o) : on(o), was(o) { on = false; }
            ~ReportOff() { on = was; }
        } report_off(b->impl.report.on);
        struct MatchOff {
            int& mode;
            const int was;
            explicit MatchOff(int& m) : mode(m), was(m) { mode = MTSV_MATCH_OFF; }
            ~MatchOff() { mode = was; }
        } match_off(b->impl.match.mode);
        const std::vector<uint8_t>& text = b->impl.ix->host.text;
        if (warm_read_len && text.size() >= (uint64_t)warm_read_len * 2 + 16) {
            const uint64_t n = std::min<uint64_t>(std::max<uint64_t>(n_reads, 1), std::max<uint64_t>(4096, (uint64_t)b->impl.n_lanes * 32768));
            std::vector<uint8_t> bases(n * warm_read_len);
            std::vector<uint64_t> off(n + 1);
            if (mtsv_synth_reads(b->impl.ix, 0x7761726d, n, warm_read_len, bases.data(), off.data()) != MTSV_OK)
                throw std::runtime_error(std::string("internal: ") + mtsv_last_error());
            mtsv_params p;
            mtsv_params_default(&p);
            b->impl.run_host(bases.data(), off.data(), n, p);
            mtsv_hit* h = nullptr;
            uint64_t nh = 0;
            b->impl.download(&h, &nh);
            mtsv_hits_free(h);
        }
    })
}

int mtsv_batch_upload(mtsv_batch* b, const uint8_t* bases, const uint64_t* read_off, uint64_t n_reads) {
    if (!b || !read_off || (!bases && n_reads && read_off[n_reads] != read_off[0])) return fail_arg("null argument");
    GUARD(b->impl.upload(bases, read_off, n_reads))
}

int mtsv_batch_run(mtsv_batch* b, const mtsv_params* params) {
    if (!b || !params) return fail_arg("null argument");
    GUARD(b->impl.run(*params))
}

int mtsv_batch_run_host(mtsv_batch* b, const uint8_t* bases, const uint64_t* read_off, uint64_t n_reads,
                        const mtsv_params* params) {
    if (!b || !read_off || !params || (!bases && n_reads && read_off[n_reads] > read_off[0])) return fail_arg("null argument");
    GUARD(b->impl.run_host(bases, read_off, n_reads, *params))
}

int mtsv_batch_run_host_parts(mtsv_batch* b, int n_parts, const uint8_t* const* bases, const uint64_t* const* read_off,
                              const uint64_t* n_reads, const mtsv_params* params) {
    if (!b || n_parts < 0 || (n_parts && (!bases || !read_off || !n_reads)) || !params) return fail_arg("null argument");
    GUARD({
        std::vector<mtsv::Batch::HostPart> parts((size_t)n_parts);
        for (int k = 0; k < n_parts; k++) {
            if (n_reads[k] && !read_off[k]) throw std::runtime_error("arg: null read_off");
            parts[(size_t)k] = mtsv::Batch::HostPart{bases[k], read_off[k], n_reads[k]};
        }
        b->impl.run_host_parts(parts.data(), n_parts, *params);
    })
}

int mtsv_batch_stats_get(const mtsv_batch* b, mtsv_batch_stats* st) {
    if (!b || !st) return fail_arg("null argument");
    *st = b->impl.stats;
    return MTSV_OK;
}

int mtsv_batch_set_taxa_report(mtsv_batch* b, int on) {
    if (!b) return fail_arg("null argument");
    GUARD(b->impl.set_taxa_report(on != 0))
}

int mtsv_batch_taxa_report(mtsv_batch* b, mtsv_taxon_stats** rows, uint64_t* n_rows, uint64_t* total_reads, float* device_ms, int reset) {
    if (!b || !rows || !n_rows || !total_reads) return fail_arg("null argument");
    GUARD({
        std::vector<mtsv_taxon_stats> r;
        float ms = 0;
        b->impl.taxa_report(r, total_reads, &ms, reset != 0);
        auto* out = (mtsv_taxon_stats*)malloc(std::max<size_t>(r.size(), 1) * sizeof(mtsv_taxon_stats));
        if (!out) throw std::bad_alloc();
        if (!r.empty()) memcpy(out, r.data(), r.size() * sizeof(mtsv_taxon_stats));
        *rows = out;
        *n_rows = r.size();
        if (device_ms) *device_ms = ms;
    })
}

int mtsv_batch_set_match_flags(mtsv_batch* b, int mode) {
    if (!b) return fail_arg("null argument");
    GUARD(b->impl.set_match_flags(mode))
}

int mtsv_batch_match_flags(mtsv_batch* b, uint64_t** words, uint64_t* n_reads, uint64_t* n_matched) {
    if (!b || !words || !n_reads || !n_matched) return fail_arg("null argument");
    GUARD({
        std::vector<uint64_t> w;
        b->impl.match_flags(w, n_reads, n_matched);
        auto* out = (uint64_t*)malloc(w.size() * sizeof(uint64_t));
        if (!out) throw std::bad_alloc();
        memcpy(out, w.data(), w.size() * sizeof(uint64_t));
        *words = out;
    })
}

int mtsv_batch_take_reads(mtsv_batch* dst, mtsv_batch* src, int keep, uint64_t* n_kept, uint64_t* bases_kept, float* device_ms) {
    if (!dst || !src || !n_kept || !bases_kept) return fail_arg("null argument");
    GUARD(dst->impl.take_reads(src->impl, keep, n_kept, bases_kept, device_ms))
}

int mtsv_batch_copy_reads(mtsv_batch* dst, mtsv_batch* src, float* device_ms) {
// ... 887 lines not shown
```

### mtsv_tools_amd/csrc/dev_index.hip

```cpp
#include <algorithm>
#include <chrono>
#include <cstdio>
#include <cstdlib>
#include <cstring>
#include <stdexcept>
#include <thread>
#include <vector>

#include "dev_mem.hpp"
#include "kernels.hpp"

namespace mtsv {

void throw_hip(hipError_t e, const char* what, const char* file, int line) {
    throw std::runtime_error(std::string("device: ") + hipGetErrorString(e) + " at " + what + " (" + file + ":" +
                             std::to_string(line) + ")");
}

DeviceIndex::~DeviceIndex() {
    if (device < 0) return;
    (void)hipSetDevice(device);
    (void)hipFree(d_blocks);
    (void)hipFree(d_sa_sample);
    (void)hipFree(d_sa_full);
// ... 23 lines not shown
__global__ void k_expand_sa(DevIndexView ix, uint32_t n_samples, uint32_t* __restrict__ sa_full) {
    uint32_t j = blockIdx.x * blockDim.x + threadIdx.x;
    if (j >= n_samples) return;
    uint32_t row = j * ix.sa_s;
    uint32_t v = ix.sa_sample[j];
    sa_full[row] = v;
    for (uint32_t guard = 0; guard <= ix.n; guard++) {
        uint32_t blk = row >> kBlockShift, off = row & (kBlockRows - 1);
        LoadedBlock b = load_block(ix.blocks, blk);
        uint32_t c = block_code(b, off);
        if (c == kCodeSentinel) break;
        row = less_of(ix, c) + block_rank(b, c, blk, off, ix.sentinel_row);
        v -= 1;
        if (row % ix.sa_s == 0) break;
        sa_full[row] = v;
    }
}

__global__ void k_kmer_level1(DevIndexView ix, uint2* __restrict__ tab) {
    uint32_t a = threadIdx.x;
    if (a >= 4) return;
    uint32_t lo = less_of(ix, a) + dev_rank(ix, a, 0);
    uint32_t hi = less_of(ix, a) + dev_rank(ix, a, ix.n);
    tab[a] = make_uint2(lo, hi);
}

__global__ void k_kmer_level(DevIndexView ix, const uint2* __restrict__ prev, uint2* __restrict__ cur,
                             uint32_t prev_shift) {
    const uint64_t total = 4ull << prev_shift, stride = (uint64_t)gridDim.x * blockDim.x;
    for (uint64_t t = (uint64_t)blockIdx.x * blockDim.x + threadIdx.x; t < total; t += stride) {
        uint32_t a = (uint32_t)(t >> prev_shift);
        uint64_t p = t & ((1ull << prev_shift) - 1);
        uint2 iv = prev[p];
        uint32_t lo = 0, hi = 0;
        if (iv.x < iv.y) {
            uint32_t b0 = iv.x >> kBlockShift, b1 = iv.y >> kBlockShift;
            LoadedBlock B0 = load_block(ix.blocks, b0);
            lo = less_of(ix, a) + block_rank(B0, a, b0, iv.x & (kBlockRows - 1), ix.sentinel_row);
            if (b1 == b0) {
                hi = less_of(ix, a) + block_rank(B0, a, b1, iv.y & (kBlockRows - 1), ix.sentinel_row);
            } else {
                LoadedBlock B1 = load_block(ix.blocks, b1);
                hi = less_of(ix, a) + block_rank(B1, a, b1, iv.y & (kBlockRows - 1), ix.sentinel_row);
            }
        }
        cur[t] = make_uint2(lo, hi);
    }
}

__global__ void k_kmer_tag(DevIndexView ix, uint2* __restrict__ tab, uint64_t total, unsigned long long* __restrict__ n_tagged) {
    const uint64_t stride = (uint64_t)gridDim.x * blockDim.x;
    uint32_t mine = 0;
    for (uint64_t t = (uint64_t)blockIdx.x * blockDim.x + threadIdx.x; t < total; t += stride) {
        const uint2 iv = tab[t];
        if (iv.y != iv.x + 1) continue;
        const uint32_t lo = iv.x;
        const uint32_t p = ix.sa_full[lo];
        const LoadedBlock b = load_block(ix.blocks, lo >> kBlockShift);
        const uint32_t c1 = block_code(b, lo & (kBlockRows - 1));
        const uint32_t c2 = p >= 2 ? ix.text[p - 2] : 7u;
        tab[t] = kmer_tag_entry(p, c1, c2);
        mine++;
    }
    for (int d = 32; d > 0; d >>= 1) mine += __shfl_down(mine, d);
    if ((threadIdx.x & 63) == 0 && mine) atomicAdd(n_tagged, (unsigned long long)mine);
}

template <class F>
void parallel_ranges(uint64_t n, int threads, F fn) {
    std::vector<std::thread> pool;
    uint64_t chunk = (n + threads - 1) / threads;
    for (int t = 0; t < threads; t++) {
        uint64_t lo = std::min(n, (uint64_t)t * chunk), hi = std::min(n, lo + chunk);
        pool.emplace_back(fn, lo, hi, t);
    }
    for (auto& th : pool) th.join();
}

}

static void pack_on_host(const HostIndex& hx, const uint32_t n, const uint32_t n_blocks, std::vector<RankBlock>& blocks, uint64_t& sentinel_row,
                         std::vector<uint8_t>& codes) {
    int threads = (int)std::max(1u, std::min(32u, std::thread::hardware_concurrency()));
    if (n_blocks < 4096) threads = 1;

    blocks.resize(n_blocks);
    std::vector<std::array<uint64_t, 6>> range_cnt(threads);
    uint64_t blocks_per = ((uint64_t)n_blocks + threads - 1) / threads;
    parallel_ranges(n_blocks, threads, [&](uint64_t, uint64_t, int t) {
        uint64_t b0 = std::min<uint64_t>(n_blocks, (uint64_t)t * blocks_per), b1 = std::min<uint64_t>(n_blocks, b0 + blocks_per);
        std::array<uint64_t, 6> c{};
        uint64_t lo = b0 << kBlockShift, hi = std::min<uint64_t>(n, b1 << kBlockShift);
        for (uint64_t i = lo; i < hi; i++) {
            uint32_t code = sym_code(hx.bwt[i]);
            if (code < 6) c[code]++;
        }
        range_cnt[t] = c;
    });
    std::vector<std::array<uint64_t, 6>> range_base(threads);
    {
        std::array<uint64_t, 6> acc{};
        for (int t = 0; t < threads; t++) {
            range_base[t] = acc;
            for (int a = 0; a < 6; a++) acc[a] += range_cnt[t][a];
        }
    }
    std::vector<std::string> errs(threads);
    std::vector<uint64_t> sentinel_rows(threads, UINT64_MAX);
    static const uint8_t syms[6] = {'A', 'C', 'G', 'T', 'N', '$'};
    parallel_ranges(n_blocks, threads, [&](uint64_t, uint64_t, int t) {
        uint64_t b0 = std::min<uint64_t>(n_blocks, (uint64_t)t * blocks_per), b1 = std::min<uint64_t>(n_blocks, b0 + blocks_per);
        std::array<uint64_t, 6> c = range_base[t];
        for (uint64_t b = b0; b < b1; b++) {
            RankBlock rb;
            for (int a = 0; a < 4; a++) rb.cnt[a] = (uint32_t)c[a];
            uint64_t p0[2] = {0, 0}, p1[2] = {0, 0}, p2[2] = {0, 0};
            for (uint32_t o = 0; o < kBlockRows; o++) {
                uint64_t i = (b << kBlockShift) + o;
                uint32_t code = 7;
                if (i < n) {
                    code = sym_code(hx.bwt[i]);
                    if (code >= 6) {
                        errs[t] = "format: bwt holds a symbol outside ACGTN$";
                        return;
                    }
                    c[code]++;
                    if (code == kCodeSentinel) sentinel_rows[t] = i;
                    if (i % hx.k == 0) {
                        uint64_t j = i / hx.k;
                        for (int a = 0; a < 6; a++)
                            if (hx.occ[syms[a]][j] != c[a]) {
                                errs[t] = "format: Occ checkpoint " + std::to_string(j) + " disagrees with the bwt";
                                return;
                            }
                    }
                }
                p0[o >> 6] |= (uint64_t)(code & 1) << (o & 63);
                p1[o >> 6] |= (uint64_t)((code >> 1) & 1) << (o & 63);
                p2[o >> 6] |= (uint64_t)((code >> 2) & 1) << (o & 63);
            }
            rb.p0[0] = p0[0]; rb.p0[1] = p0[1];
            rb.p1[0] = p1[0]; rb.p1[1] = p1[1];
            rb.p2[0] = p2[0]; rb.p2[1] = p2[1];
            blocks[b] = rb;
        }
    });
    for (auto& e : errs)
        if (!e.empty()) throw std::runtime_error(e);
    sentinel_row = UINT64_MAX;
    for (uint64_t s : sentinel_rows)
        if (s != UINT64_MAX) sentinel_row = s;
    if (sentinel_row == UINT64_MAX) throw std::runtime_error("format: bwt holds no sentinel");

    codes.assign(((uint64_t)n + 15) / 16 * 16 + 32, (uint8_t)7);
    parallel_ranges(n, threads, [&](uint64_t lo, uint64_t hi, int) {
        for (uint64_t i = lo; i < hi; i++) codes[i] = (uint8_t)sym_code(hx.text[i]);
    });
}

static uint64_t pack_on_device(const HostIndex& hx, const uint32_t n, const uint32_t n_blocks, DeviceIndex& di, double& copy_ms) {
    uint32_t tile = kPackTile;
    if (const char* e = getenv("MTSV_PACK_TILE")) {
        const int t = atoi(e);
        if (t >= 1 && t <= (int)kPackTileMax && !(t & (t - 1))) tile = (uint32_t)t;
    }
    static const uint8_t syms[6] = {'A', 'C', 'G', 'T', 'N', '$'};
    const uint64_t n_chk = ((uint64_t)n - 1) / hx.k + 1;
    for (uint8_t a : syms)
        if (hx.occ[a].size() < n_chk) throw std::runtime_error("format: occ checkpoint count != floor((n-1)/k)+1");
    const uint32_t tiles = pack_tiles(n_blocks, tile);
    const uint64_t raw_bytes = ((uint64_t)n + 15) / 16 * 16;
    DevEvents<7> ev;
    DevBuf<uint8_t> d_bwt, d_raw_text;
    DevBuf<uint64_t> d_occ;
    DevBuf<uint4> d_tiles;
    DevBuf<uint32_t> d_ctr;
    ev.create();

    HIP_CHECK(hipMalloc((void**)&di.d_blocks, (uint64_t)n_blocks * sizeof(RankBlock)));
    di.bytes += (uint64_t)n_blocks * sizeof(RankBlock);
    d_bwt.alloc(raw_bytes, "the raw bwt");
    d_occ.alloc(6 * n_chk, "the raw Occ arrays");
    d_tiles.alloc(tiles, "the pack's tiles");
    d_ctr.alloc(kPackCounters, "the pack's counters");
    uint32_t ctr[kPackCounters] = {0};
    ctr[kPackCtrForeignRow] = ctr[kPackCtrOccBadFirst] = 0xffffffffu;
    double t0 = now_ms();
    HIP_CHECK(hipMemcpy(d_bwt.p, hx.bwt.data(), n, hipMemcpyHostToDevice));
    for (int a = 0; a < 6; a++)
        HIP_CHECK(hipMemcpy(d_occ.p + a * n_chk, hx.occ[syms[a]].data(), n_chk * 8, hipMemcpyHostToDevice));
    HIP_CHECK(hipMemcpy(d_ctr.p, ctr, sizeof ctr, hipMemcpyHostToDevice));
    copy_ms += now_ms() - t0;

    HIP_CHECK(hipEventRecord(ev.e[0], 0));
    launch_pack_count(0, d_bwt.p, n, n_blocks, tile, d_tiles.p, d_ctr.p);
    HIP_CHECK(hipEventRecord(ev.e[1], 0));
    launch_pack_scan(0, d_tiles.p, tiles);
    HIP_CHECK(hipEventRecord(ev.e[2], 0));
    launch_pack_blocks(0, d_bwt.p, n, n_blocks, tile, d_tiles.p, di.d_blocks);
    HIP_CHECK(hipEventRecord(ev.e[3], 0));
    launch_pack_check_occ(0, di.d_blocks, n, hx.k, (uint32_t)n_chk, d_occ.p, d_ctr.p);
    HIP_CHECK(hipGetLastError());
    HIP_CHECK(hipEventRecord(ev.e[4], 0));
    HIP_CHECK(hipMemcpy(ctr, d_ctr.p, sizeof ctr, hipMemcpyDeviceToHost));
    d_bwt.release();
    d_occ.release();
    d_tiles.release();
    d_ctr.release();
    const uint64_t occ_row = ctr[kPackCtrOccBad] ? (uint64_t)ctr[kPackCtrOccBadFirst] * hx.k : UINT64_MAX;
    if (ctr[kPackCtrForeign] && ctr[kPackCtrForeignRow] <= occ_row) throw std::runtime_error("format: bwt holds a symbol outside ACGTN$");
    if (ctr[kPackCtrOccBad])
        throw std::runtime_error("format: Occ checkpoint " + std::to_string(ctr[kPackCtrOccBadFirst]) + " disagrees with the bwt");
    if (!ctr[kPackCtrSentinels]) throw std::runtime_error("format: bwt holds no sentinel");

    HIP_CHECK(hipMalloc((void**)&di.d_text, di.text_bytes));
    di.bytes += di.text_bytes;
    d_raw_text.alloc(raw_bytes, "the raw text");
    t0 = now_ms();
    HIP_CHECK(hipMemcpy(d_raw_text.p, hx.text.data(), n, hipMemcpyHostToDevice));
    copy_ms += now_ms() - t0;
    HIP_CHECK(hipEventRecord(ev.e[5], 0));
    launch_pack_text(0, d_raw_text.p, n, di.d_text, di.text_bytes);
    HIP_CHECK(hipGetLastError());
    HIP_CHECK(hipEventRecord(ev.e[6], 0));
    HIP_CHECK(hipEventSynchronize(ev.e[6]));
    d_raw_text.release();
    float ms[5] = {0.f, 0.f, 0.f, 0.f, 0.f};
    for (int k = 0; k < 4; k++) HIP_CHECK(hipEventElapsedTime(&ms[k], ev.e[k], ev.e[k + 1]));
    HIP_CHECK(hipEventElapsedTime(&ms[4], ev.e[5], ev.e[6]));
    di.pack_ms = ms[0] + ms[1] + ms[2] + ms[3] + ms[4];
    if (getenv("MTSV_TRACE"))
        fprintf(stderr, "[upload] pack on device, tile %u: k_pack_count %.3f k_pack_scan %.3f k_pack_blocks %.3f k_pack_check_occ %.3f k_pack_text %.3f ms\n",
                tile, ms[0], ms[1], ms[2], ms[3], ms[4]);
    return ctr[kPackCtrSentinelRow];
}

std::unique_ptr<DeviceIndex> upload_index(const HostIndex& hx, int device, uint32_t flags) {
    const uint64_t n64 = hx.n();
    if (n64 >= 0xFFFFFF00ull)
        throw std::runtime_error("limit: index of 2^32 symbols or more does not fit the u32 device layout; chunk the database (mtsv-chunk)");
    int ndev = 0;
    if (hipGetDeviceCount(&ndev) != hipSuccess || ndev <= 0)
        throw std::runtime_error("device: no HIP device visible (this library has no CPU path)");
    if (device < 0 || device >= ndev) throw std::runtime_error("device: invalid device ordinal " + std::to_string(device));
    HIP_CHECK(hipSetDevice(device));

    const uint32_t n = (uint32_t)n64;
    const uint32_t n_blocks = (n >> kBlockShift) + 1;
    const char* pack_env = getenv("MTSV_DEV_PACK");
    const bool on_device = (flags & 4u ) || (pack_env && !strcmp(pack_env, "device"));

    std::vector<RankBlock> blocks;
    std::vector<uint8_t> codes;
    uint64_t sentinel_row = UINT64_MAX;
    const double pack_t0 = now_ms();
    if (!on_device) pack_on_host(hx, n, n_blocks, blocks, sentinel_row, codes);
    const double host_pack_ms = now_ms() - pack_t0;

    std::vector<uint32_t> samp(hx.sample.size());
    for (size_t i = 0; i < samp.size(); i++) samp[i] = (uint32_t)hx.sample[i];
    std::vector<DevBin> bins(hx.bins.size());
    std::vector<uint32_t> bin_end(hx.bins.size());
    for (size_t i = 0; i < bins.size(); i++) {
        bins[i] = DevBin{(uint32_t)hx.bins[i].start, (uint32_t)hx.bins[i].end, hx.bins[i].tax_id, hx.bins[i].gi};
        bin_end[i] = (uint32_t)hx.bins[i].end;
    }

    uint32_t lut_shift = 0;
    while (((uint64_t)n >> lut_shift) > 65536) lut_shift++;
    std::vector<uint32_t> bin_lut(((uint64_t)n >> lut_shift) + 2);
    {
        uint32_t b = 0;
        for (size_t k = 0; k < bin_lut.size(); k++) {
            uint64_t p = (uint64_t)k << lut_shift;
            while (b + 1 < bins.size() && bin_end[b] <= p) b++;
            bin_lut[k] = b;
        }
    }

    auto di = std::make_unique<DeviceIndex>();
    di->device = device;
    di->flags = flags;
    double copy_ms = 0;
    auto up = [&](auto** dptr, const void* src, uint64_t bytes) {
        HIP_CHECK(hipMalloc((void**)dptr, bytes ? bytes : 16));
        const double t0 = now_ms();
        if (bytes) HIP_CHECK(hipMemcpy(*dptr, src, bytes, hipMemcpyHostToDevice));
        copy_ms += now_ms() - t0;
        di->bytes += bytes;
    };
    di->text_bytes = ((uint64_t)n + 15) / 16 * 16 + 32;
    di->sa_sample_bytes = samp.size() * 4;
    di->bin_lut_bytes = bin_lut.size() * 4;
    di->packed_on_device = on_device;
    if (on_device) {
        sentinel_row = pack_on_device(hx, n, n_blocks, *di, copy_ms);
        up(&di->d_sa_sample, samp.data(), samp.size() * 4);
    } else {
        di->pack_ms = (float)host_pack_ms;
        up(&di->d_blocks, blocks.data(), (uint64_t)n_blocks * sizeof(RankBlock));
        up(&di->d_sa_sample, samp.data(), samp.size() * 4);
        up(&di->d_text, codes.data(), codes.size());
    }
    up(&di->d_bin_end, bin_end.data(), bin_end.size() * 4);
    up(&di->d_bins, bins.data(), bins.size() * sizeof(DevBin));
    up(&di->d_bin_lut, bin_lut.data(), bin_lut.size() * 4);

    DevIndexView& v = di->view;
    v.blocks = di->d_blocks;
    v.n = n;
    v.n_blocks = n_blocks;
    v.C[0] = (uint32_t)hx.less['A'];
    v.C[1] = (uint32_t)hx.less['C'];
    v.C[2] = (uint32_t)hx.less['G'];
    v.C[3] = (uint32_t)hx.less['T'];
    v.C[4] = (uint32_t)hx.less['N'];
    v.sentinel_row = (uint32_t)sentinel_row;
    v.sa_sample = di->d_sa_sample;
    v.sa_s = (uint32_t)hx.s;
    v.sa_pow2_shift = 0xffffffffu;
    if (hx.s > 0xFFFFFFFFull) throw std::runtime_error("limit: suffix sampling interval does not fit u32");
    for (uint32_t sh = 0; sh < 32; sh++)
        if ((1ull << sh) == hx.s) v.sa_pow2_shift = sh;
    v.sa_full = nullptr;
    v.text = di->d_text;
    v.bin_end = di->d_bin_end;
    v.bins = di->d_bins;
    v.n_bins = (uint32_t)bins.size();
    v.bin_lut = di->d_bin_lut;
    v.bin_lut_shift = lut_shift;
    v.kmer_tab = nullptr;
    v.kmer_k = 0;

    hipEvent_t e0, e1;
    HIP_CHECK(hipEventCreate(&e0));
    HIP_CHECK(hipEventCreate(&e1));
    HIP_CHECK(hipEventRecord(e0, 0));
    if (!(flags & 1u )) {
        HIP_CHECK(hipMalloc((void**)&di->d_sa_full, (uint64_t)n * 4));
        di->bytes += (uint64_t)n * 4;
        uint32_t ns = (uint32_t)samp.size();
        hipLaunchKernelGGL(k_expand_sa, dim3((ns + 255) / 256), dim3(256), 0, 0, v, ns, di->d_sa_full);
        HIP_CHECK(hipGetLastError());
        v.sa_full = di->d_sa_full;
    }
    if (!(flags & 2u )) {
        uint32_t k = 1;
        while (k < 16 && (1ull << (2 * (k + 1))) <= 2 * (uint64_t)n) k++;
        if (k == 16 && n >= (1u << 31)) k = 17;
        if (const char* e = getenv("MTSV_KMER_K")) {
            int kk = atoi(e);
            if (kk >= 1 && kk <= 17) k = (uint32_t)kk;
        }
        size_t free_b = 0, total_b = 0;
        HIP_CHECK(hipMemGetInfo(&free_b, &total_b));
        if (k == 17 && (10ull << 34) + (48ull << 30) > (uint64_t)free_b) k = 16;
        while (k > 1 && k <= 16 && (10ull << (2 * k)) * 2 > (uint64_t)free_b) k--;
        uint64_t entries = 1ull << (2 * k);
        uint2 *ta = nullptr, *tb = nullptr;
        if (k == 17) {
            if (hipMalloc((void**)&ta, entries * 8) != hipSuccess || hipMalloc((void**)&tb, entries / 4 * 8) != hipSuccess) {
                (void)hipGetLastError();
                if (ta) (void)hipFree(ta);
                ta = tb = nullptr;
                k = 16;
                entries = 1ull << 32;
            }
        }
        if (!ta) {
            HIP_CHECK(hipMalloc((void**)&ta, entries * 8));
            HIP_CHECK(hipMalloc((void**)&tb, std::max<uint64_t>(entries / 4, 4) * 8));
        }
        const char* kl = getenv("MTSV_KMER_LEVELS");
        const uint32_t n_levels = ((kl && atoi(kl) == 0) || !v.sa_full) ? 0 : std::min(k, kKmerLevelsMax);
        uint64_t level_bytes = 0;
        if (n_levels) {
            level_bytes = (uint64_t)kmer_level_start(n_levels + 1) * sizeof(uint2);
            HIP_CHECK(hipMalloc((void**)&di->d_kmer_levels, level_bytes));
            di->bytes += level_bytes;
        }
        auto keep_level = [&](uint32_t lvl, const uint2* src) {
            if (lvl <= n_levels)
                HIP_CHECK(hipMemcpyAsync(di->d_kmer_levels + kmer_level_start(lvl), src, (sizeof(uint2)) << (2 * lvl),
                                         hipMemcpyDeviceToDevice, 0));
        };
        uint2* cur = (k % 2 == 1) ? ta : tb;
        uint2* oth = (k % 2 == 1) ? tb : ta;
        hipLaunchKernelGGL(k_kmer_level1, dim3(1), dim3(64), 0, 0, v, cur);
        keep_level(1, cur);
        for (uint32_t lvl = 2; lvl <= k; lvl++) {
            const uint64_t total = 1ull << (2 * lvl);
            hipLaunchKernelGGL(k_kmer_level, dim3((uint32_t)std::min<uint64_t>((total + 255) / 256, 1u << 22)), dim3(256), 0, 0, v, cur, oth,
                               2 * (lvl - 1));
            std::swap(cur, oth);
            keep_level(lvl, cur);
        }
        HIP_CHECK(hipGetLastError());
        HIP_CHECK(hipDeviceSynchronize());
        HIP_CHECK(hipFree(tb));
        di->d_kmer = ta;
        di->bytes += entries * 8;
        v.kmer_tab = di->d_kmer;
        v.kmer_k = k;
        if (getenv("MTSV_TRACE"))
            fprintf(stderr, "[upload] kmer levels 1..%u kept: %llu bytes\n", n_levels, (unsigned long long)level_bytes);
        const char* kp = getenv("MTSV_KMER_POS");
        if (v.sa_full && !(kp && atoi(kp) == 0)) {
            unsigned long long* d_n = nullptr;
            HIP_CHECK(hipMalloc((void**)&d_n, sizeof(unsigned long long)));
            HIP_CHECK(hipMemset(d_n, 0, sizeof(unsigned long long)));
            hipEvent_t t0, t1;
            HIP_CHECK(hipEventCreate(&t0));
            HIP_CHECK(hipEventCreate(&t1));
            HIP_CHECK(hipEventRecord(t0, 0));
            hipLaunchKernelGGL(k_kmer_tag, dim3((uint32_t)std::min<uint64_t>((entries + 255) / 256, 1u << 16)), dim3(256), 0, 0, v,
                               di->d_kmer, entries, d_n);
            HIP_CHECK(hipGetLastError());
            HIP_CHECK(hipEventRecord(t1, 0));
            unsigned long long n_tagged = 0;
            HIP_CHECK(hipMemcpy(&n_tagged, d_n, sizeof(n_tagged), hipMemcpyDeviceToHost));
            float ms = 0.f;
            HIP_CHECK(hipEventElapsedTime(&ms, t0, t1));
            (void)hipEventDestroy(t0);
            (void)hipEventDestroy(t1);
            (void)hipFree(d_n);
            if (getenv("MTSV_TRACE"))
                fprintf(stderr, "[upload] kmer table k=%u: %llu tagged entries of %llu (%.1f ms)\n", k, n_tagged,
                        (unsigned long long)entries, ms);
        } else if (getenv("MTSV_TRACE")) {
            fprintf(stderr, "[upload] kmer table k=%u: 0 tagged entries of %llu (0.0 ms)\n", k, (unsigned long long)entries);
        }
    }
    HIP_CHECK(hipEventRecord(e1, 0));
    HIP_CHECK(hipEventSynchronize(e1));
    HIP_CHECK(hipEventElapsedTime(&di->accel_build_ms, e0, e1));
    (void)hipEventDestroy(e0);
    (void)hipEventDestroy(e1);
    di->copy_ms = (float)copy_ms;
    return di;
}

}
```

### mtsv_tools_amd/csrc/dev_index.hpp

```cpp
#pragma once
#include <map>
#include <memory>
#include <mutex>
#include <string>

#include "dev_layout.hpp"
#include "mgindex.hpp"

namespace mtsv {

[[noreturn]] void throw_hip(hipError_t e, const char* what, const char* file, int line);
#define HIP_CHECK(expr)                                              \
    do {                                                             \
        hipError_t _e = (expr);                                      \
        if (_e != hipSuccess) ::mtsv::throw_hip(_e, #expr, __FILE__, __LINE__); \
    } while (0)

struct DeviceIndex {
    int device = -1;
    RankBlock* d_blocks = nullptr;
    uint32_t* d_sa_sample = nullptr;
    uint32_t* d_sa_full = nullptr;
    uint8_t* d_text = nullptr;
    uint32_t* d_bin_end = nullptr;
    DevBin* d_bins = nullptr;
    uint32_t* d_bin_lut = nullptr;
    uint2* d_kmer = nullptr;
    uint2* d_kmer_levels = nullptr;
    DevIndexView view{};
    uint64_t bytes = 0;
    uint32_t flags = 0;
    float accel_build_ms = 0.f;
    uint64_t text_bytes = 0, sa_sample_bytes = 0, bin_lut_bytes = 0;
    bool packed_on_device = false;
    float pack_ms = 0.f, copy_ms = 0.f;

    DeviceIndex() = default;
    DeviceIndex(const DeviceIndex&) = delete;
    DeviceIndex& operator=(const DeviceIndex&) = delete;
    ~DeviceIndex();
};

std::unique_ptr<DeviceIndex> upload_index(const HostIndex& hx, int device, uint32_t flags);

}

struct mtsv_cached_workspace {
    std::mutex mu;
    struct mtsv_batch* b = nullptr;
};
struct mtsv_index {
    mtsv::HostIndex host;
    std::mutex mu;
    std::map<int, std::unique_ptr<mtsv::DeviceIndex>> dev;
    std::map<std::pair<int, int>, std::unique_ptr<mtsv_cached_workspace>> cached_batch;
};
```

### mtsv_tools_amd/csrc/dev_layout.hpp

```cpp
#pragma once
#include <hip/hip_runtime.h>

#include <cstdint>

namespace mtsv {

constexpr uint32_t kCodeA = 0, kCodeC = 1, kCodeG = 2, kCodeT = 3, kCodeN = 4, kCodeSentinel = 5;
constexpr uint32_t kBlockRows = 128;
constexpr uint32_t kBlockShift = 7;

struct alignas(64) RankBlock {
    uint32_t cnt[4];
    uint64_t p0[2];
    uint64_t p1[2];
    uint64_t p2[2];
};
static_assert(sizeof(RankBlock) == 64, "rank block must be one 64-byte line");

struct DevBin {
    uint32_t start, end, tax_id, gi;
};

struct DevIndexView {
    const RankBlock* blocks;
    uint32_t n;
    uint32_t n_blocks;
    uint32_t C[5];
    uint32_t sentinel_row;
    const uint32_t* sa_sample;
    uint32_t sa_s;
    uint32_t sa_pow2_shift;
    const uint32_t* sa_full;
    const uint8_t* text;
    const uint32_t* bin_end;
    const DevBin* bins;
    uint32_t n_bins;
    const uint32_t* bin_lut;
    uint32_t bin_lut_shift;
    const uint2* kmer_tab;
    uint32_t kmer_k;
};

constexpr uint32_t kKmerTag = 0xFFFFFF00u;
__host__ __device__ inline bool kmer_tagged(uint2 e) { return (e.y & kKmerTag) == kKmerTag; }
__host__ __device__ inline uint32_t kmer_tag_c1(uint2 e) { return e.y & 7u; }
__host__ __device__ inline uint32_t kmer_tag_c2(uint2 e) { return (e.y >> 3) & 7u; }
__host__ __device__ inline uint2 kmer_tag_entry(uint32_t p, uint32_t c1, uint32_t c2) {
    return make_uint2(p, kKmerTag | c1 | (c2 << 3));
}

constexpr uint32_t kKmerLevelsMax = 12;
__host__ __device__ inline uint32_t kmer_level_start(uint32_t j) { return ((1u << (2 * j)) - 4u) / 3u; }

constexpr uint32_t kSeedAtPos = 0xFFFFFFFFu;

__host__ __device__ inline uint32_t base_code(uint8_t b) {
    switch (b) {
    case 'A': case 'a': return kCodeA;
    case 'C': case 'c': return kCodeC;
    case 'G': case 'g': return kCodeG;
    case 'T': case 't': return kCodeT;
    default: return kCodeN;
    }
}
__host__ __device__ inline uint32_t comp_code(uint32_t c) { return c < 4 ? 3 - c : c; }

#ifdef __HIPCC__
struct LoadedBlock {
    uint4 h, q0, q1, q2;
};

__device__ inline LoadedBlock load_block(const RankBlock* blocks, uint32_t blk) {
    const uint4* p = reinterpret_cast<const uint4*>(blocks + blk);
    LoadedBlock b;
    b.h = p[0];
    b.q0 = p[1];
    b.q1 = p[2];
    b.q2 = p[3];
    return b;
}

__device__ inline uint64_t u64_of(uint32_t lo, uint32_t hi) { return ((uint64_t)hi << 32) | lo; }

__device__ inline uint32_t block_code(const LoadedBlock& b, uint32_t off) {
    bool hi = off & 64;
    uint32_t sh = off & 63;
    uint64_t w0 = hi ? u64_of(b.q0.z, b.q0.w) : u64_of(b.q0.x, b.q0.y);
    uint64_t w1 = hi ? u64_of(b.q1.z, b.q1.w) : u64_of(b.q1.x, b.q1.y);
    uint64_t w2 = hi ? u64_of(b.q2.z, b.q2.w) : u64_of(b.q2.x, b.q2.y);
    return (uint32_t)((w0 >> sh) & 1) | ((uint32_t)((w1 >> sh) & 1) << 1) | ((uint32_t)((w2 >> sh) & 1) << 2);
}

__device__ inline uint32_t block_rank(const LoadedBlock& b, uint32_t a, uint32_t blk, uint32_t off,
                                      uint32_t sentinel_row) {
    uint64_t x0 = (a & 1) ? 0ull : ~0ull, x1 = (a & 2) ? 0ull : ~0ull, x2 = (a & 4) ? 0ull : ~0ull;
    uint64_t ma = (u64_of(b.q0.x, b.q0.y) ^ x0) & (u64_of(b.q1.x, b.q1.y) ^ x1) &
                  (u64_of(b.q2.x, b.q2.y) ^ x2);
    uint64_t mb = (u64_of(b.q0.z, b.q0.w) ^ x0) & (u64_of(b.q1.z, b.q1.w) ^ x1) &
                  (u64_of(b.q2.z, b.q2.w) ^ x2);
    uint64_t maskA = off >= 64 ? ~0ull : ((1ull << off) - 1);
    uint64_t maskB = off > 64 ? ((1ull << (off - 64)) - 1) : 0ull;
    uint32_t base;
    if (a < 4) {
        base = a == 0 ? b.h.x : a == 1 ? b.h.y : a == 2 ? b.h.z : b.h.w;
    } else {
        uint32_t before = blk << kBlockShift;
        base = before - (b.h.x + b.h.y + b.h.z + b.h.w) - (before > sentinel_row ? 1u : 0u);
    }
    return base + __popcll(ma & maskA) + __popcll(mb & maskB);
}

__device__ inline uint32_t less_of(const DevIndexView& ix, uint32_t a) {
    return a == 0 ? ix.C[0] : a == 1 ? ix.C[1] : a == 2 ? ix.C[2] : a == 3 ? ix.C[3] : ix.C[4];
}

__device__ inline uint32_t dev_rank(const DevIndexView& ix, uint32_t a, uint32_t pos) {
    uint32_t blk = pos >> kBlockShift;
    LoadedBlock b = load_block(ix.blocks, blk);
    return block_rank(b, a, blk, pos & (kBlockRows - 1), ix.sentinel_row);
}
#endif

}
```

### mtsv_tools_amd/csrc/k_verify.hip

```cpp
#include "kernels_common.hpp"

namespace mtsv {

namespace {

typedef short pk16 __attribute__((ext_vector_type(2)));

__device__ inline pk16 pk(int lo, int hi) {
    pk16 r;
    r.x = (short)lo;
    r.y = (short)hi;
    return r;
}
__device__ inline pk16 pk_max(pk16 a, pk16 b) { return __builtin_elementwise_max(a, b); }
__device__ inline int pk_bits(pk16 a) { return __builtin_bit_cast(int, a); }
__device__ inline pk16 pk_from_bits(int u) { return __builtin_bit_cast(pk16, u); }

constexpr uint32_t kGroup = 16;
constexpr uint32_t kRing = 1024;

__device__ inline int row_shr1(int v) { return __builtin_amdgcn_update_dpp(0, v, 0x111, 0xf, 0xf, true); }

__device__ inline uint32_t group_ballot(bool p, uint32_t group) { return (uint32_t)(__ballot(p) >> (group * kGroup)) & 0xffffu; }

// ... 947 lines not shown
        const bool have = index_of(it) < n_work;
        uint32_t gi_3 = 0, b0_1 = 0, L_1 = 0;
        uint4 c_2 = make_uint4(0, 0, 0, 0);
        if (index_of(it + 3) < n_work) gi_3 = item_at((uint32_t)index_of(it + 3));
        if (index_of(it + 2) < n_work) c_2 = a.cand[gi_2];
        if (index_of(it + 1) < n_work) {
            const uint32_t r1 = a.r0 + (c_1.w >> 1);
            b0_1 = a.read_off[r1];
            L_1 = a.read_off[r1 + 1] - b0_1;
        }
        bool decided = false;
        const uint32_t gi = gi_0;
        if (have) {
            const uint4 c = c_0;
            const uint32_t rs = c.w;
            const uint32_t b0 = b0_0, L = L_0;
            const uint32_t ED = (uint32_t)ceil((double)L * a.edit_rate);
            const uint32_t W = c.y - c.x;
            if (gl == 0) {
                verified++;
                wbytes += W;
            }
            if (2ull * ED <= (uint64_t)L && ED + L <= W) {
                const uint32_t p0 = gl * (4 * NW);
                uint32_t rd[NW];
                {
                    const bool rev = (rs & 1u) != 0;
                    const uint32_t pq = p0 < L ? p0 : 0u;
                    const long long ba = rev ? (long long)b0 + L - 4 * NW - pq : (long long)b0 + pq;
                    const long long w = ba >> 2;
                    const uint32_t sh = (uint32_t)(ba & 3);
                    uint32_t d[NW + 1];
#pragma unroll
                    for (int k = 0; k <= NW; k++) d[k] = b32[max(w + k, 0ll)];
                    uint32_t x[NW];
#pragma unroll
                    for (int k = 0; k < NW; k++) x[k] = __builtin_amdgcn_alignbyte(d[k + 1], d[k], sh);
#pragma unroll
                    for (int k = 0; k < NW; k++) rd[k] = rev ? comp_codes4(__builtin_bswap32(x[NW - 1 - k])) : x[k];
                }
                const uint32_t pc = c.x + ED + p0;
                const uint32_t wi = pc >> 2, sc = pc & 3u;
                uint32_t wv[NW + 2];
                wv[0] = t32[wi >= 1 ? min(wi - 1, lastw) : 0u];
#pragma unroll
                for (int k = 0; k <= NW; k++) wv[k + 1] = t32[min(wi + k, lastw)];
                int ca[3][NW];
#pragma unroll
                for (int k = 0; k < NW; k++) {
                    const uint32_t lo = wv[k + 1], hi = wv[k + 2], bl = wv[k];
                    const uint32_t s0 = sc == 0 ? __builtin_amdgcn_alignbyte(lo, bl, 3u) : __builtin_amdgcn_alignbyte(hi, lo, sc - 1u);
                    const uint32_t s1 = __builtin_amdgcn_alignbyte(hi, lo, sc);
                    const uint32_t s2 = sc == 3 ? hi : __builtin_amdgcn_alignbyte(hi, lo, sc + 1u);
                    const uint32_t pk_ = p0 + 4 * k;
                    const uint32_t nv = pk_ < L ? min(L - pk_, 4u) : 0u;
                    const uint32_t valid = nv >= 4 ? 0x01010101u : ((1u << (8 * nv)) - 1u) & 0x01010101u;
                    ca[0][k] = __popc(nz_bytes(rd[k] ^ s0) & valid);
                    ca[1][k] = __popc(nz_bytes(rd[k] ^ s1) & valid);
                    ca[2][k] = __popc(nz_bytes(rd[k] ^ s2) & valid);
                }
                int mm[3];
#pragma unroll
                for (int d = 0; d < 3; d++) {
                    mm[d] = 0;
#pragma unroll
                    for (int k = 0; k < NW; k++) mm[d] += ca[d][k];
                }
                decided = (uint32_t)row_sum16(mm[1]) <= ED;
                if (!decided && ED >= 1 && ED + L + 1 <= W) {
                    int below[3], above[3];
#pragma unroll
                    for (int d = 0; d < 3; d++) {
                        below[d] = row_prefix_incl16(mm[d]) - mm[d];
                        above[d] = row_suffix_incl16(mm[d]) - mm[d];
                    }
                    auto split = [&](int da, int db) {
                        int pa = 0, sb = mm[db], best = mm[db];
#pragma unroll
                        for (int k = 0; k < NW; k++) {
                            pa += ca[da][k];
                            sb -= ca[db][k];
                            best = min(best, pa + sb);
                        }
                        return below[da] + best + above[db];
                    };
                    int best = min(min(split(1, 0), split(1, 2)), min(split(0, 1), split(2, 1)));
                    best = -row_max16(-best);
                    decided = best <= (int)ED - 1;
                }
            }
        }
        const unsigned long long pm = __ballot(have && gl == 0 && decided), sm = __ballot(have && gl == 0 && !decided);
        const unsigned long long lower = (1ull << lane) - 1ull;
        if (have && gl == 0 && decided) pbuf[np + (uint32_t)__popcll(pm & lower)] = gi;
        if (have && gl == 0 && !decided) sbuf[nsw + (uint32_t)__popcll(sm & lower)] = gi;
        np += (uint32_t)__popcll(pm);
        nsw += (uint32_t)__popcll(sm);
        if (np + 4 > kDiagBuf) flush(pbuf, np, sw_pass_count(a), a.pass_list, 0u);
        if (nsw + 4 > kDiagBuf) flush(sbuf, nsw, reinterpret_cast<uint32_t*>(a.counters + sweep_slot), sweep_list, kSweepFlag);
        gi_0 = gi_1;
        gi_1 = gi_2;
        gi_2 = gi_3;
        c_0 = c_1;
        c_1 = c_2;
        b0_0 = b0_1;
        L_0 = L_1;
    }
    if (np) flush(pbuf, np, sw_pass_count(a), a.pass_list, 0u);
    if (nsw) flush(sbuf, nsw, reinterpret_cast<uint32_t*>(a.counters + sweep_slot), sweep_list, kSweepFlag);
    for (int d = 32; d > 0; d >>= 1) {
        verified += __shfl_down(verified, d);
        wbytes += __shfl_down(wbytes, d);
    }
    if (lane == 0 && verified) {
        atomicAdd((unsigned long long*)a.counters + kCtrVerified, verified);
        atomicAdd((unsigned long long*)a.counters + kCtrWindowBytes, wbytes);
    }
}

__device__ inline uint32_t clamp_codes4(uint32_t x) {
    const uint32_t t = x & 0x04040404u;
    return t | (x & 0x03030303u & ~((t >> 1) | (t >> 2)));
}
__device__ inline uint32_t clamp_codes_sw(uint32_t x) {
    const uint32_t t = x & 0x04040404u, lo = x & 0x03030303u;
    const uint32_t nz = (lo | (lo >> 1)) & 0x01010101u, m = t >> 2;
    return t | (lo & ~(m * 3u)) | ((nz ^ 0x01010101u) & m);
}
__device__ inline uint4 fetch_cols(const DevIndexView& ix, uint32_t start, uint32_t end, uint32_t strand, uint32_t j0, bool sw_matches) {
    uint4 r;
    if (!strand) {
        r = load16(ix.text, ix.n, start + j0);
    } else if (end >= j0 + 16) {
        const uint4 v = load16(ix.text, ix.n, end - j0 - 16);
        r.x = __builtin_amdgcn_perm(0, v.w, 0x00010203u);
        r.y = __builtin_amdgcn_perm(0, v.z, 0x00010203u);
        r.z = __builtin_amdgcn_perm(0, v.y, 0x00010203u);
        r.w = __builtin_amdgcn_perm(0, v.x, 0x00010203u);
    } else {
        uint32_t w[4] = {0, 0, 0, 0};
        for (uint32_t i = 0; i < 16; i++) {
            const uint32_t code = end >= j0 + 1 + i ? ix.text[end - j0 - 1 - i] : 7u;
            w[i >> 2] |= code << (8 * (i & 3));
        }
        r = make_uint4(w[0], w[1], w[2], w[3]);
    }
    r.x = sw_matches ? clamp_codes_sw(r.x) : clamp_codes4(r.x);
    r.y = sw_matches ? clamp_codes_sw(r.y) : clamp_codes4(r.y);
    r.z = sw_matches ? clamp_codes_sw(r.z) : clamp_codes4(r.z);
    r.w = sw_matches ? clamp_codes_sw(r.w) : clamp_codes4(r.w);
    return r;
}

enum : int { MY_CHAIN = 0, MY_LIST = 1, MY_BOUND = 2, MY_FUSED = 3 };
template <int W, int MODE>
__global__ __launch_bounds__(256) void k_edit_myers(DevIndexView ix, EvalArgs a) {
    constexpr bool FUSED = MODE == MY_FUSED, LIST = MODE == MY_LIST || FUSED, BOUND = MODE == MY_BOUND;
    constexpr int NROW = (BOUND || LIST) ? 6 : 5;
    __shared__ uint32_t eq_tab[NROW][W][256];
    const uint32_t tid = threadIdx.x;
    const uint32_t n_work = *a.wl_count;
    const uint32_t maxc = a.maxc;
    const uint32_t lane = lane_id();
    uint32_t verified = 0, wbytes = 0;
    uint32_t cols = 0, refuted = 0;
    uint32_t bnext = 0, bend = 0;
    bool active = false, exhausted = false;
    bool counted = false;
    uint32_t g = 0, o = 0, L = 0, ED = 0, strand = 0;
    bool thr_wrapped = false, hopeless = false;
    uint32_t pv0[W];
    uint32_t ph = 0, extra_passed = 0;
    bool read_n = false;
    for (;;) {
        unsigned long long need = __ballot(!active);
        if (need) {
            if (bnext == bend && !exhausted) {
                const uint32_t n_waves = gridDim.x * (256 / kWave);
                const uint32_t claim = min(256u, max(64u, (n_work / n_waves + 63u) & ~63u));
                uint32_t base = 0;
                if (lane == 0) base = atomicAdd(a.wl_cursor, claim);
                base = __builtin_amdgcn_readfirstlane(base);
                bnext = min(base, n_work);
                bend = min(base + claim, n_work);
                exhausted = bnext == bend;
            }
            const uint32_t take = bnext + __popcll(need & ((1ull << lane) - 1));
            if (!active && take < bend) {
                g = a.worklist[FUSED && a.wl_reverse ? n_work - 1 - take : take];
                if (BOUND) {
                    counted = (g & kSweepFlag) != 0;
                    g &= ~kSweepFlag;
                }
                const uint32_t rs = a.cand[g].w;
                const uint32_t r_ = a.r0 + (rs >> 1);
                strand = rs & 1;
                o = a.strand_off[rs];
                const uint32_t b0 = a.read_off[r_];
                L = a.read_off[r_ + 1] - b0;
                ED = (uint32_t)ceil((double)L * a.edit_rate);
                thr_wrapped = 2ull * ED > (uint64_t)L;
                const int pad = 32 * W - (int)L;
                const uint32_t nw = (L + 31) >> 5, pw = (uint32_t)(pad + 31) >> 5, sh = (uint32_t)(-pad) & 31u;
                const uint32_t* img = a.planes + ((uint64_t)(rs >> 1) * a.plane_words) * 3;
                uint32_t P0[W + 1], P1[W + 1], PN[W + 1];
#pragma unroll
                for (int j = 0; j <= W; j++) {
                    const uint32_t idx = (uint32_t)j - pw;
                    P0[j] = P1[j] = PN[j] = 0;
                    if (idx < nw) {
                        P0[j] = img[3 * idx];
                        P1[j] = img[3 * idx + 1];
                        PN[j] = img[3 * idx + 2];
                    }
                }
                uint32_t read_ns = 0;
#pragma unroll
                for (int k = 0; k < W; k++) {
                    const uint32_t p0 = __builtin_amdgcn_alignbit(P0[k + 1], P0[k], sh), p1 = __builtin_amdgcn_alignbit(P1[k + 1], P1[k], sh),
                                   pn = __builtin_amdgcn_alignbit(PN[k + 1], PN[k], sh);
                    const int below = pad - 32 * k;
                    const uint32_t wild = below >= 32 ? 0xffffffffu : below <= 0 ? 0u : (1u << below) - 1u;
                    const uint32_t mA = ~(p0 | p1 | pn), mC = (p0 & ~p1 & ~pn) | wild, mG = (p1 & ~p0 & ~pn) | wild,
                                   mT = (p0 & p1 & ~pn) | wild;
                    read_ns += __popc(pn);
                    eq_tab[0][k][tid] = strand ? mT : mA;
                    eq_tab[1][k][tid] = strand ? mG : mC;
                    eq_tab[2][k][tid] = strand ? mC : mG;
                    eq_tab[3][k][tid] = strand ? mA : mT;
                    eq_tab[4][k][tid] = wild;
                    if (NROW == 6) eq_tab[5][k][tid] = pn | wild;
                    pv0[k] = ~wild;
                }
                hopeless = thr_wrapped || (!BOUND && read_ns > ED);
                read_n = read_ns != 0;
                ph = FUSED ? 1 : 0;
                active = true;
            }
            bnext = min(bnext + (uint32_t)__popcll(need), bend);
        }
        if (!__any(active)) {
            if (exhausted) break;
            continue;
        }
        uint32_t verdict = 0, vg = 0;
        if ((FUSED ? thr_wrapped : !LIST && hopeless) && active) {
            const uint4 c = a.cand[g];
            if (!BOUND || !counted) {
                verified++;
                wbytes += c.y - c.x;
            }
            counted = false;
            a.cand_status[g] = 1;
            const uint32_t nxt = a.cand_next[g];
            if (nxt == 0xffffffffu || nxt >= maxc) active = false;
            else g = o + nxt;
        } else if (active) {
            const uint4 c = a.cand[g];
            uint32_t Pv[W], Mv[W];
#pragma unroll
            for (int k = 0; k < W; k++) {
                Pv[k] = pv0[k];
                Mv[k] = 0;
            }
            const uint32_t Wn = c.y - c.x;
            int score = (int)L, best = (int)L;
            const bool swm = BOUND || (LIST && ph == 1);
            uint4 nxt4 = Wn ? fetch_cols(ix, c.x, c.y, strand, 0, swm) : make_uint4(0, 0, 0, 0);
            const uint32_t* lane_tab = &eq_tab[0][0][tid];
            uint32_t j0 = 0;
            uint32_t win_n = 0;
            for (; j0 < Wn; j0 += 16) {
                if (swm) {
                    if (BOUND && best <= (int)ED) break;
                    if (best > 2 * (int)ED && score - (int)(Wn - j0) > 2 * (int)ED) break;
                }
                const uint4 cur = nxt4;
                if (LIST) win_n |= cur.x | cur.y | cur.z | cur.w;
                if (j0 + 16 < Wn) nxt4 = fetch_cols(ix, c.x, c.y, strand, j0 + 16, swm);
                const uint32_t lim = min(16u, Wn - j0);
#pragma unroll
                for (int jj = 0; jj < 16; jj++) {
                    if ((uint32_t)jj < lim) {
                        const uint32_t word = jj < 4 ? cur.x : jj < 8 ? cur.y : jj < 12 ? cur.z : cur.w;
                        const uint32_t tc = (word >> ((jj & 3) * 8)) & 0xffu;
                        const uint32_t* row = lane_tab + tc * (W * 256);
                        uint32_t ph_below = 0, mh_below = 0;
#pragma unroll
                        for (int k = 0; k < W; k++) {
                            const uint32_t Eq = row[k * 256];
                            const uint32_t pv = Pv[k], mv = Mv[k];
                            const uint32_t Xv = Eq | mv;
                            const uint32_t Eqh = k ? (Eq | (mh_below >> 31)) : Eq;
                            const uint32_t Xh = __builtin_amdgcn_bitop3_b32((Eqh & pv) + pv, pv, Eqh, 0xBE);
                            const uint32_t Ph = mv | ~(Xh | pv);
                            const uint32_t Mh = pv & Xh;
                            const uint32_t Phs = k ? __builtin_amdgcn_alignbit(Ph, ph_below, 31) : (Ph << 1);
                            const uint32_t Mhs = k ? __builtin_amdgcn_alignbit(Mh, mh_below, 31) : (Mh << 1);
                            Pv[k] = Mhs | ~(Xv | Phs);
                            Mv[k] = Phs & Xv;
                            ph_below = Ph;
                            mh_below = Mh;
                        }
                        const uint32_t hp = ph_below >> 31, hm = mh_below >> 31;
                        score += (int)hp - (int)hm;
                        best = min(best, score);
                    }
                }
            }
            cols += min(j0, Wn);
            if (LIST ? ph == 1 : (!BOUND || !counted)) {
                verified++;
                wbytes += Wn;
            }
            counted = false;
            const uint32_t ed = (uint32_t)best;
            if (BOUND) {
                if (!thr_wrapped && ed <= ED) {
                    verdict = 1;
                    vg = g;
                    active = false;
                } else if (!thr_wrapped && ed <= 2 * ED) {
                    verdict = 2;
                    vg = g;
                    active = false;
                } else {
                    refuted++;
                    a.cand_status[g] = 1;
                    const uint32_t nxt = a.cand_next[g];
                    if (nxt == 0xffffffffu || nxt >= maxc) active = false;
                    else g = o + nxt;
                }
            } else if (LIST && ph == 1) {
                if (ed > 2 * ED) {
                    if (FUSED) refuted++;
                    a.cand_status[g] = 1;
                    const uint32_t nxt = a.cand_next[g];
                    if (nxt == 0xffffffffu || nxt >= maxc) active = false;
                    else g = o + nxt;
                } else if (ed > ED) {
                    if (FUSED) {
                        verdict = 2;
                    } else {
                        a.next_list[atomicAdd(a.next_count, 1u)] = g | kSweepFlag;
                    }
                    active = false;
                } else {
                    extra_passed++;
                    if (!read_n || !(win_n & 0x04040404u)) {
                        const DevBin bin = ix.bins[c.z];
                        a.out[g] = make_uint4(bin.tax_id, bin.gi, c.x >= bin.start ? c.x - bin.start : 0, ed);
                        a.cand_status[g] = 2;
                        active = false;
                    } else {
                        ph = 2;
                    }
                }
            } else {
            const bool pass = !thr_wrapped && ed <= ED;
            if (pass) {
                const DevBin bin = ix.bins[c.z];
                a.out[g] = make_uint4(bin.tax_id, bin.gi, c.x >= bin.start ? c.x - bin.start : 0, ed);
                a.cand_status[g] = 2;
                active = false;
            } else {
                a.cand_status[g] = 1;
                const uint32_t nxt = a.cand_next[g];
                if (nxt == 0xffffffffu || nxt >= maxc) active = false;
                else {
                    g = o + nxt;
                    if (LIST) ph = 1;
                }
            }
            }
        }
        if (BOUND || FUSED) {
            const unsigned long long pm = BOUND ? __ballot(verdict == 1) : 0ull, um = __ballot(verdict == 2);
            const unsigned long long lower = (1ull << lane) - 1ull;
            if (pm) {
                uint32_t base = 0;
                if (lane == 0) base = atomicAdd(sw_pass_count(a), (uint32_t)__popcll(pm));
                base = __builtin_amdgcn_readfirstlane(base);
                if (verdict == 1) a.pass_list[base + (uint32_t)__popcll(pm & lower)] = vg;
            }
            if (um) {
                uint32_t base = 0;
                if (lane == 0) base = atomicAdd(reinterpret_cast<uint32_t*>(a.counters + a.und_slot), (uint32_t)__popcll(um));
                base = __builtin_amdgcn_readfirstlane(base);
                if (verdict == 2) a.und_list[base + (uint32_t)__popcll(um & lower)] = (FUSED ? g : vg) | kSweepFlag;
            }
        }
    }
    unsigned long long v64 = verified, w64 = wbytes;
    for (int d = 32; d > 0; d >>= 1) {
        v64 += __shfl_down(v64, d);
        w64 += __shfl_down(w64, d);
    }
    if (lane == 0 && v64) {
        atomicAdd(a.n_verified, v64);
        atomicAdd(a.window_bytes, w64);
    }
    if (a.myers_ctr) {
        unsigned long long c64 = cols, r64 = refuted;
        for (int d = 32; d > 0; d >>= 1) {
            c64 += __shfl_down(c64, d);
            r64 += __shfl_down(r64, d);
        }
        unsigned long long e64 = extra_passed;
        for (int d = 32; d > 0; d >>= 1) e64 += __shfl_down(e64, d);
        if (lane == 0) {
            atomicAdd(a.myers_ctr, c64);
            if ((BOUND || FUSED) && r64) atomicAdd(a.myers_ctr + 1, r64);
            if (LIST && e64) atomicAdd(a.myers_ctr + 2, e64);
        }
    }
}

__global__ __launch_bounds__(256) void k_resolve(uint32_t n_strands, int64_t max_candidates, int64_t max_assignments,
                                                 const uint32_t* __restrict__ strand_off,
                                                 const uint32_t* __restrict__ strand_ncand,
                                                 const uint32_t* __restrict__ cand_status, uint4* __restrict__ out,
                                                 uint32_t* __restrict__ strand_nout) {
    const uint32_t rs = blockIdx.x * blockDim.x + threadIdx.x;
    const bool valid = rs < n_strands;
    uint32_t nc = valid ? strand_ncand[rs] : 0;
    uint32_t nout = 0;
    const uint32_t o = nc ? strand_off[rs] : 0;
    if (max_candidates >= 0 && (uint64_t)nc > (uint64_t)max_candidates) nc = (uint32_t)max_candidates;
    constexpr uint32_t kCoop = 32;
    const bool big = nc > kCoop;
    if (nc && !big) {
        for (uint32_t i = 0; i < nc; i++) {
            if (cand_status[o + i] == 2) {
                if (nout != i) out[o + nout] = out[o + i];
                nout++;
                if (max_assignments >= 0 && (uint64_t)nout >= (uint64_t)max_assignments) break;
            }
        }
    }
    const uint32_t lane = lane_id();
    const uint64_t cap = max_assignments < 0 ? ~0ull : (uint64_t)(max_assignments > 1 ? max_assignments : 1);
    for (unsigned long long m = __ballot(big); m; m &= m - 1) {
        const int l = __builtin_ctzll(m);
        const uint32_t o_l = __builtin_amdgcn_readlane(o, l), nc_l = __builtin_amdgcn_readlane(nc, l);
        uint32_t nout_l = 0;
        for (uint32_t base = 0; base < nc_l; base += kWave) {
            const uint32_t i = base + lane;
            const bool pass = i < nc_l && cand_status[o_l + i] == 2;
            uint4 v = make_uint4(0, 0, 0, 0);
            if (pass) v = out[o_l + i];
            const unsigned long long pm = __ballot(pass);
            const uint32_t pos = nout_l + (uint32_t)__popcll(pm & ((1ull << lane) - 1));
            if (pass && (uint64_t)pos < cap) out[o_l + pos] = v;
            nout_l += (uint32_t)__popcll(pm);
            if ((uint64_t)nout_l >= cap) {
                nout_l = (uint32_t)cap;
                break;
            }
        }
        if ((int)lane == l) nout = nout_l;
    }
    if (!valid) return;
    strand_nout[rs] = nout;
}

__global__ __launch_bounds__(256) void k_gather(uint32_t n_strands, uint64_t r0, const uint32_t* __restrict__ strand_off,
                                                const uint32_t* __restrict__ strand_nout,
                                                const uint32_t* __restrict__ out_off, const uint4* __restrict__ out,
                                                DevHit* __restrict__ hits, uint64_t hits_base) {
    uint32_t rs = blockIdx.x * blockDim.x + threadIdx.x;
    if (rs >= n_strands) return;
    uint32_t n = strand_nout[rs];
    if (!n) return;
    uint32_t src = strand_off[rs];
    uint64_t dst = hits_base + out_off[rs];
    for (uint32_t i = 0; i < n; i++) {
        uint4 v = out[src + i];
        DevHit h;
        h.read = r0 + (rs >> 1);
        h.tax_id = v.x;
        h.gi = v.y;
        h.edit = v.w;
        h.strand = rs & 1;
        h.offset = v.z;
        hits[dst + i] = h;
    }
}

}

void launch_evaluate(hipStream_t s, const DevIndexView& ix, const EvalArgs& a_, uint64_t max_items, uint32_t max_len) {
    EvalArgs a = a_;
    a.maxc = rank_bound(a.max_candidates);
#define EVAL_CASE(RR, WW, GG) hipLaunchKernelGGL((k_evaluate<RR, WW, GG>), dim3(std::max<uint32_t>(1, std::min<uint32_t>(cdiv(max_items, 256 / GG), 256 * 8))), dim3(256), 0, s, ix, a)
    if (max_len <= 32) EVAL_CASE(2, false, 16);
    else if (max_len <= 64) EVAL_CASE(4, false, 16);
    else if (max_len <= 80) EVAL_CASE(5, false, 16);
    else if (max_len <= 112) EVAL_CASE(7, false, 16);
    else if (max_len <= 128) EVAL_CASE(8, false, 16);
    else if (max_len <= 160) EVAL_CASE(10, false, 16);
    else if (max_len <= 208) EVAL_CASE(13, false, 16);
    else if (max_len < 254) EVAL_CASE(16, false, 16);
    else if (max_len <= kMaxRegisterReadLen) EVAL_CASE(16, true, 16);
    else throw std::runtime_error("internal: launch_evaluate called for a read beyond the register-resident kernels");
#undef EVAL_CASE
}

uint32_t tiled_groups(uint64_t max_items, uint32_t strip_len) {
    const uint64_t by_mem = std::max<uint64_t>(1, (1ull << 30) / (16ull * 8 * std::max<uint32_t>(strip_len, 1)));
    const uint32_t blocks = (uint32_t)std::max<uint64_t>(1, std::min<uint64_t>(std::min<uint64_t>(cdiv(max_items, 16), 256 * 2), by_mem));
    return blocks * 16;
}

void launch_evaluate_tiled(hipStream_t s, const DevIndexView& ix, const EvalArgs& a_, uint64_t max_items) {
    EvalArgs a = a_;
    a.maxc = rank_bound(a.max_candidates);
    const uint32_t blocks = tiled_groups(max_items, a.strip_len) / 16;
    hipLaunchKernelGGL((k_evaluate<16, true, 16, true>), dim3(blocks), dim3(256), 0, s, ix, a);
}

void launch_sw_pairs(hipStream_t s, const DevIndexView& ix, const EvalArgs& a_, uint64_t max_items_, uint32_t max_len, bool diag, bool top, bool sparse) {
    const uint64_t max_items = sparse ? std::max<uint64_t>(max_items_ / 64, 1024) : max_items_;
    EvalArgs a = a_;
    a.maxc = rank_bound(a.max_candidates);
    if (top) {
#define SW_TOP(RR)                                                                                                       \
    do {                                                                                                                 \
        const uint32_t grid = std::max<uint32_t>(1, std::min<uint32_t>(cdiv(max_items, 32), 256 * kSwTopOcc));           \
        a.claim_shift = 0;                                                                                               \
        while ((1ull << a.claim_shift) < (uint64_t)grid * 16 * 2) a.claim_shift++;                                       \
        hipLaunchKernelGGL((k_sw_pairs<RR, false, true>), dim3(grid), dim3(256), 0, s, ix, a);                           \
    } while (0)
        if (max_len <= 64) SW_TOP(2);
        else if (max_len <= 96) SW_TOP(3);
        else if (max_len <= 128) SW_TOP(4);
        else if (max_len <= 160) SW_TOP(5);
        else if (max_len <= 208) SW_TOP(7);
        else SW_TOP(8);
#undef SW_TOP
        return;
    }
#define SW_CASE(RR)                                                                                                      \
    do {                                                                                                                 \
        const uint32_t grid = std::max<uint32_t>(1, std::min<uint32_t>(cdiv(max_items, 32), 256 * ((RR) > 10 ? 3 : kSwOcc))); \
        a.claim_shift = 0;                                                                                               \
        while ((1ull << a.claim_shift) < (uint64_t)grid * 16 * 2) a.claim_shift++;                                       \
        if (diag) hipLaunchKernelGGL((k_sw_pairs<RR, true>), dim3(grid), dim3(256), 0, s, ix, a);                        \
        else hipLaunchKernelGGL((k_sw_pairs<RR, false>), dim3(grid), dim3(256), 0, s, ix, a);                            \
    } while (0)
    if (max_len <= 64) SW_CASE(4);
    else if (max_len <= 96) SW_CASE(6);
    else if (max_len <= 128) SW_CASE(8);
    else if (max_len <= 160) SW_CASE(10);
    else if (max_len <= 208) SW_CASE(13);
    else SW_CASE(16);
#undef SW_CASE
}

void launch_sw_diag(hipStream_t s, const DevIndexView& ix, const EvalArgs& a, uint64_t max_items, uint32_t max_len,
                    uint32_t* sweep_list, uint32_t sweep_slot) {
    const uint32_t grid = std::max<uint32_t>(16, std::min<uint32_t>(cdiv(max_items, 16 * 32), 256 * 6));
    if (max_len <= 128) hipLaunchKernelGGL(k_sw_diag<2>, dim3(grid), dim3(256), 0, s, ix, a, sweep_list, sweep_slot);
    else if (max_len <= 192) hipLaunchKernelGGL(k_sw_diag<3>, dim3(grid), dim3(256), 0, s, ix, a, sweep_list, sweep_slot);
    else hipLaunchKernelGGL(k_sw_diag<4>, dim3(grid), dim3(256), 0, s, ix, a, sweep_list, sweep_slot);
}

uint32_t launch_edit_myers(hipStream_t s, const DevIndexView& ix, const EvalArgs& a_, uint64_t max_items, uint32_t max_len,
                           int mode, uint32_t wgs_per_cu, bool listed) {
    EvalArgs a = a_;
    a.maxc = rank_bound(a.max_candidates);
    if (!a.planes || a.plane_words != myers_words(max_len)) throw std::runtime_error("internal: k_edit_myers needs the pass's read planes");
    const uint32_t resident = 256 * std::max<uint32_t>(1, std::min<uint32_t>(wgs_per_cu, kMyersWgsPerCuMax));
    uint32_t blocks = std::max<uint32_t>(16, std::min<uint32_t>(cdiv(max_items, listed ? 256 : 4096), resident));
    const uint32_t W = myers_words(max_len);
#define MYERS_CASE(WW)                                                                                   \
    do {                                                                                                 \
        if (mode == MY_LIST) hipLaunchKernelGGL((k_edit_myers<WW, MY_LIST>), dim3(blocks), dim3(256), 0, s, ix, a);        \
        else if (mode == MY_FUSED) hipLaunchKernelGGL((k_edit_myers<WW, MY_FUSED>), dim3(blocks), dim3(256), 0, s, ix, a); \
        else if (mode == MY_BOUND) hipLaunchKernelGGL((k_edit_myers<WW, MY_BOUND>), dim3(blocks), dim3(256), 0, s, ix, a); \
        else hipLaunchKernelGGL((k_edit_myers<WW, MY_CHAIN>), dim3(blocks), dim3(256), 0, s, ix, a);                      \
    } while (0)
    if (W == 2) MYERS_CASE(2);
    else if (W == 3) MYERS_CASE(3);
    else if (W == 4) MYERS_CASE(4);
    else if (W == 5) MYERS_CASE(5);
    else if (W == 6) MYERS_CASE(6);
    else if (W == 7) MYERS_CASE(7);
    else MYERS_CASE(8);
#undef MYERS_CASE
    return blocks;
}

void launch_resolve(hipStream_t s, uint32_t n_strands, int64_t max_candidates, int64_t max_assignments,
                    const uint32_t* strand_off, const uint32_t* strand_ncand, const uint32_t* cand_status, uint4* out,
                    uint32_t* strand_nout) {
    hipLaunchKernelGGL(k_resolve, dim3(cdiv(n_strands, 256)), dim3(256), 0, s, n_strands, max_candidates, max_assignments,
                       strand_off, strand_ncand, cand_status, out, strand_nout);
}

void launch_gather(hipStream_t s, uint32_t n_strands, uint64_t r0, const uint32_t* strand_off, const uint32_t* strand_nout,
                   const uint32_t* out_off, const uint4* out, DevHit* hits, uint64_t hits_base) {
    hipLaunchKernelGGL(k_gather, dim3(cdiv(n_strands, 256)), dim3(256), 0, s, n_strands, r0, strand_off, strand_nout,
                       out_off, out, hits, hits_base);
}

}
```

### mtsv_tools_amd/csrc/kernels.hpp

```cpp
#pragma once
#include <algorithm>

#include "dev_layout.hpp"
#include "pass_plan.hpp"

namespace mtsv {

struct DevHit {
    uint64_t read;
    uint32_t tax_id;
    uint32_t gi;
    uint32_t edit;
    uint8_t strand;
    uint8_t pad[3];
    uint64_t offset;
};
static_assert(sizeof(DevHit) == 32, "DevHit must match mtsv_hit");

enum CtrSlot : uint32_t {
    kCtrSeedHits = 0,
    kCtrWorklist = 1,
    kCtrLfSteps = 2,
    kCtrCandidates = 3,
    kCtrVerified = 4,
    kCtrWindowBytes = 5,
    kCtrOutTotal = 6,
    kCtrWlCursor = 7,
    kCtrSwCursor = 8,
    kCtrPassCount = 9,
    kCtrMyersCursor = 10,
    kCtrNext0 = 11,
    kCtrNext1 = 12,
    kCtrMaxWindow = 13,
    kCtrSwCellPairs = 14,
    kCtrMidStrands = 15,
    kCtrSweepCount = 16,
    kCtrUndecided = 17,
    kCtrBoundCursor = 18,
    kCtrMyersColumns = 19,
    kCtrBoundRefuted = 20,
    kCtrListPassed = 21,
    kCtrListedSlots = 22,
    kCtrHeavyWalk = 23,
    kCtrHeavyTicket = 24,
    kCtrCount
};
constexpr uint64_t ctr_bit(uint32_t slot) { return 1ull << slot; }
constexpr uint64_t kCtrClearPass = ctr_bit(kCtrWorklist) | ctr_bit(kCtrWlCursor) | ctr_bit(kCtrMidStrands) | ctr_bit(kCtrHeavyTicket) | ctr_bit(kCtrListedSlots);
constexpr uint64_t ctr_clear_round(uint32_t round) {
    return ctr_bit(kCtrSwCursor) | ctr_bit(kCtrPassCount) | ctr_bit(kCtrMyersCursor) | ctr_bit(kCtrNext0 + (round & 1));
}
constexpr uint64_t kCtrClearRound0 = ctr_clear_round(0) | ctr_bit(kCtrUndecided) | ctr_bit(kCtrBoundCursor);
static_assert(kCtrCount <= 64, "launch_clear_counters takes a mask of 64 slots");
static_assert(kCtrNext1 == kCtrNext0 + 1, "the rounds ping-pong between two adjacent slots");
static_assert(kCtrPassCount == kCtrSwCursor + 1 && kCtrMyersCursor == kCtrSwCursor + 2, "one memset zeroes the three of a round");
static_assert(kCtrBoundCursor == kCtrUndecided + 1, "one memset zeroes the bound pass's two");
static_assert(kCtrBoundRefuted == kCtrMyersColumns + 1 && kCtrListPassed == kCtrMyersColumns + 2, "EvalArgs::myers_ctr is an array of three");
static_assert(kCtrVerified == kCtrCandidates + 1 && kCtrWindowBytes == kCtrCandidates + 2, "k_coalesce adds to the three side by side");

struct EvalArgs {
    const uint8_t* bases;
    const uint32_t* read_off;
    uint32_t r0;
    double edit_rate;
    int64_t max_candidates;
    const uint32_t* strand_off;
    const uint4* cand;
    const uint32_t* cand_next;
    uint32_t* cand_status;
    const uint32_t* worklist;
    const uint32_t* wl_count;
    uint32_t* wl_cursor;
    uint32_t wl_reverse = 0;
    uint64_t* counters = nullptr;
    uint32_t wl_count_slot = 0;
    uint4* out;
    unsigned long long* n_verified;
    unsigned long long* window_bytes;
    unsigned long long* sw_columns = nullptr;
    uint32_t* pass_list = nullptr;
    uint32_t* pass_count = nullptr;
    uint32_t* next_list = nullptr;
    uint32_t* next_count = nullptr;
    unsigned long long* myers_ctr = nullptr;
    uint32_t* und_list = nullptr;
    uint32_t und_slot = 0;
    uint2* strip = nullptr;
    uint32_t strip_len = 0;
    const uint32_t* planes = nullptr;
    uint32_t plane_words = 0;
    uint32_t maxc = 0xffffffffu;
    uint32_t claim_shift = 0;
};


void launch_publish(hipStream_t s, const uint64_t* src, uint64_t* dst_host, uint32_t n);
void launch_clear_counters(hipStream_t s, uint64_t* counters, uint64_t mask);
void launch_normalise(hipStream_t s, const uint8_t* src, uint8_t* dst, uint64_t begin, uint64_t end);
void launch_unpack(hipStream_t s, const uint8_t* packed, uint8_t* dst, uint64_t lo, uint64_t hi);
void launch_search(hipStream_t s, const DevIndexView& ix, const uint8_t* bases, const uint32_t* read_off, uint32_t r0,
                   uint32_t n_reads, uint32_t max_ns, uint32_t K, uint32_t G, uint32_t* seed_lo, uint32_t* seed_cnt,
                   uint32_t* slow_list, uint32_t* slow_count, uint32_t listed_cap, const uint2* kmer_levels,
                   bool count_is_zero = false);
void launch_thin(hipStream_t s, const uint8_t* bases, const uint32_t* read_off, uint32_t r0, uint32_t n_reads, double edit_rate,
                 double min_seed, uint32_t max_ns, uint32_t K, uint32_t G, uint64_t max_hits, uint64_t tune, uint32_t* seed_cnt, uint32_t* seed_pre,
                 uint32_t* strand_hits, uint32_t* strand_nseeds, uint32_t* planes, uint32_t plane_words);
bool seed_tile_fits(uint32_t max_ns, uint32_t max_len, uint64_t n_slots);
uint32_t seed_tile_reads();
uint32_t seed_tile_max_ns();
void launch_thin_tiled(hipStream_t s, const uint8_t* bases, const uint32_t* read_off, uint32_t r0, uint32_t n_reads, double edit_rate,
                       double min_seed, uint32_t max_ns, uint32_t K, uint32_t G, uint64_t max_hits, uint64_t tune, uint32_t* seed_cnt,
                       uint32_t* strand_hits, uint32_t* strand_nseeds, uint32_t* planes, uint32_t plane_words);
void launch_expand_tiled(hipStream_t s, const DevIndexView& ix, uint32_t n_strands, uint32_t max_ns, uint32_t G, const uint32_t* seed_lo,
                         const uint32_t* seed_cnt, const uint32_t* strand_off, uint32_t* hit_row, uint32_t* hit_ref, uint32_t* hit_q);
void launch_scan(hipStream_t s, const uint32_t* in, uint32_t n, uint64_t* tile_sums, uint64_t* total, uint32_t* out);
uint32_t scan_tiles(uint32_t n);
void launch_expand(hipStream_t s, const DevIndexView& ix, uint32_t n_strands, uint32_t max_ns, uint32_t G,
                   const uint32_t* seed_lo, const uint32_t* seed_cnt, const uint32_t* seed_pre, const uint32_t* strand_off,
                   uint32_t* hit_row, uint32_t* hit_ref, uint32_t* hit_q);
void launch_locate(hipStream_t s, const DevIndexView& ix, uint32_t total_hits_host, const uint32_t* total_hits_dev,
                   const uint32_t* hit_row, uint32_t* hit_ref, unsigned long long* lf_steps);
void launch_coalesce(hipStream_t s, const DevIndexView& ix, const uint32_t* read_off, uint32_t r0, uint32_t n_strands,
                     int64_t max_candidates, const uint32_t* strand_off,
                     const uint32_t* strand_nseeds, const uint32_t* hit_ref, const uint32_t* hit_q, uint64_t* hit_key,
                     uint64_t* cand_tmp, uint4* cand, uint32_t* cand_next, uint32_t* cand_status,
                     uint32_t* strand_ncand, uint32_t* worklist, uint32_t* heavy_list, uint64_t* counters,
                     bool ticket_is_zero = false);
void launch_evaluate(hipStream_t s, const DevIndexView& ix, const EvalArgs& a, uint64_t max_items, uint32_t max_len);
void launch_evaluate_tiled(hipStream_t s, const DevIndexView& ix, const EvalArgs& a, uint64_t max_items);
uint32_t tiled_groups(uint64_t max_items, uint32_t strip_len);
void launch_max_window(hipStream_t s, uint32_t n_strands, const uint32_t* strand_off, const uint32_t* strand_ncand,
                       const uint4* cand, unsigned long long* out);
constexpr uint32_t kMyersWgsPerCuMax = 5;
uint32_t launch_edit_myers(hipStream_t s, const DevIndexView& ix, const EvalArgs& a, uint64_t max_items, uint32_t max_len,
                           int mode = 0, uint32_t wgs_per_cu = kMyersWgsPerCuMax, bool listed = false);
void launch_sw_pairs(hipStream_t s, const DevIndexView& ix, const EvalArgs& a, uint64_t max_items, uint32_t max_len,
                     bool diag = true, bool top = false, bool sparse = false);
void launch_sw_diag(hipStream_t s, const DevIndexView& ix, const EvalArgs& a, uint64_t max_items, uint32_t max_len,
                    uint32_t* sweep_list, uint32_t sweep_slot);
void launch_resolve(hipStream_t s, uint32_t n_strands, int64_t max_candidates, int64_t max_assignments,
                    const uint32_t* strand_off, const uint32_t* strand_ncand, const uint32_t* cand_status, uint4* out,
                    uint32_t* strand_nout);
void launch_gather(hipStream_t s, uint32_t n_strands, uint64_t r0, const uint32_t* strand_off, const uint32_t* strand_nout,
                   const uint32_t* out_off, const uint4* out, DevHit* hits, uint64_t hits_base);
constexpr uint32_t kReportDenseTaxa = 4095;
constexpr uint32_t kReportHashSlots = 4096;
void launch_report(hipStream_t s, uint32_t n_reads, const uint32_t* strand_nout, const uint32_t* out_off, const DevHit* hits,
                   const uint32_t* taxa, uint32_t n_taxa, bool dense, uint32_t hash_slots, uint64_t* counts, uint64_t* total_reads,
                   uint64_t* n_global);
void launch_match(hipStream_t s, uint32_t n_reads, const uint32_t* strand_nout, uint64_t first_bit, uint64_t* words, uint64_t* n_matched);
uint32_t compact_tiles(uint64_t n_reads);
void launch_compact_scan(hipStream_t s, uint32_t n_reads, const uint64_t* words, const uint32_t* read_off, int keep_matched, uint64_t* tile_cnt,
                         uint64_t* tile_bases, uint64_t* result);
void launch_compact_copy(hipStream_t s, uint32_t n_reads, const uint64_t* words, const uint32_t* read_off, const uint8_t* codes, int keep_matched,
                         const uint32_t* src_map, const uint64_t* tile_cnt, const uint64_t* tile_bases, const uint64_t* result, uint8_t* dst_codes,
                         uint32_t* dst_off, uint32_t* dst_map);
void launch_remap_reads(hipStream_t s, DevHit* hits, uint64_t n_hits, const uint32_t* map);
struct MergePart {
    const DevHit* hits;
    uint32_t count, first_read, n_reads, src;
    uint64_t pad;
};
static_assert(sizeof(MergePart) == 32, "MergePart is uploaded as it is");
void launch_merge_bounds(hipStream_t s, const MergePart* parts, uint32_t n_parts, uint32_t max_part_reads, uint32_t n_reads,
                         const uint32_t* map, uint32_t* lo, uint32_t* cnt);
void launch_merge_sum(hipStream_t s, uint32_t n_reads, uint32_t n_srcs, const uint32_t* lo, uint32_t* cnt_base, uint32_t* nout);
void launch_merge_copy(hipStream_t s, const MergePart* parts, uint32_t n_parts, uint32_t max_part_hits, uint32_t n_reads,
                       const uint32_t* map, const uint32_t* base, const uint32_t* out_off, DevHit* dst, uint32_t n_dst, uint64_t* n_dropped);
constexpr uint32_t kCollapseLaneMax = 16, kCollapseLdsKeys = 4096, kCollapseLdsKeysWide = 2048;
constexpr int kCollapseGrainTaxid = 0, kCollapseGrainTaxidGi = 1, kCollapseGrainLong = 2;
constexpr uint32_t kCollapseCtrTotal = 0, kCollapseCtrList = 1, kCollapseCtrTicket = 2, kCollapseCtrLane = 3, kCollapseCtrWave = 4,
                   kCollapseCtrListed = 5, kCollapseCtrLds = 6, kCollapseCtrGlobal = 7, kCollapseCounters = 8;
void launch_collapse(hipStream_t s, int grain, uint32_t n_reads, const uint32_t* strand_nout, const uint32_t* out_off, const DevHit* hits,
                     uint32_t n_hits, uint32_t lane_max, uint32_t wave_max, uint32_t lds_max, void* keys, uint32_t* flags, uint32_t* place,
                     uint64_t* tile_sums, uint32_t* list, uint64_t* ctr, void* out);
constexpr uint32_t kFoldTileMax = 1024, kFoldTile = 1024;
uint32_t fold_tiles(uint64_t n, uint32_t tile);
void launch_fold_count(hipStream_t s, int grain, const void* a, uint32_t n_a, const void* b, uint32_t n_b, uint32_t tile, uint32_t* tile_cnt);
void launch_fold_write(hipStream_t s, int grain, const void* a, uint32_t n_a, const void* b, uint32_t n_b, uint32_t tile, const uint32_t* tile_off,
                       void* out);
void launch_fold_flags(hipStream_t s, int grain, const void* rec, uint32_t n, uint64_t n_reads, uint64_t* words, uint64_t* ctr);
void launch_fold_report(hipStream_t s, int grain, const void* rec, uint32_t n, const uint32_t* taxa, uint32_t n_taxa, uint64_t* counts);
constexpr uint32_t kTextTileMax = 1024, kTextTile = 1024;
constexpr uint64_t kTextIdMax = 1ull << 20;
uint32_t text_tiles(uint64_t n, uint32_t tile);
uint32_t text_scan_blocks(uint32_t tiles);
uint32_t text_window_bytes(uint32_t tile);
void launch_text_measure(hipStream_t s, int grain, const void* rec, uint32_t n, const uint8_t* ids, const uint64_t* id_off, uint64_t n_reads,
                         uint64_t ids_bytes, uint32_t tile, uint32_t* rec_len, uint32_t* tile_cnt, uint64_t* ctr);
void launch_text_scan(hipStream_t s, const uint32_t* tile_cnt, uint32_t tiles, uint64_t* sums, uint64_t* total, uint64_t* tile_off);
void launch_text_write(hipStream_t s, int grain, const void* rec, uint32_t n, const uint8_t* ids, const uint64_t* id_off, uint32_t tile,
                       const uint32_t* rec_len, const uint64_t* tile_off, uint8_t* out);
constexpr uint32_t kPackTileMax = 64, kPackTile = 64;
constexpr uint32_t kPackCtrForeign = 0, kPackCtrForeignRow = 1, kPackCtrSentinels = 2, kPackCtrSentinelRow = 3, kPackCtrOccBad = 4,
                   kPackCtrOccBadFirst = 5, kPackCounters = 8;
uint32_t pack_tiles(uint32_t n_blocks, uint32_t tile);
void launch_pack_count(hipStream_t s, const uint8_t* bwt, uint32_t n, uint32_t n_blocks, uint32_t tile, uint4* tile_cnt, uint32_t* ctr);
void launch_pack_scan(hipStream_t s, uint4* tile_cnt, uint32_t n_tiles);
void launch_pack_blocks(hipStream_t s, const uint8_t* bwt, uint32_t n, uint32_t n_blocks, uint32_t tile, const uint4* tile_off, RankBlock* blocks);
void launch_pack_check_occ(hipStream_t s, const RankBlock* blocks, uint32_t n, uint32_t k, uint32_t n_chk, const uint64_t* occ, uint32_t* ctr);
void launch_pack_text(hipStream_t s, const uint8_t* text, uint32_t n, uint8_t* codes, uint64_t codes_bytes);
constexpr uint32_t kParseTileMax = 16384, kParseTile = 4096;
constexpr uint32_t kParseCtrFormat = 0, kParseCtrKeyOrder = 2, kParseCtrReadOrder = 4, kParseCtrReadRange = 6, kParseCounters = 8;
uint32_t parse_tiles(uint64_t n_bytes, uint32_t tile);
void launch_parse_count(hipStream_t s, const uint8_t* hits, uint64_t n_bytes, const uint64_t* line_off, uint64_t n_lines, uint32_t tile,
                        uint32_t* tile_cnt);
void launch_parse_tokens(hipStream_t s, int grain, const uint8_t* hits, uint64_t n_bytes, const uint64_t* line_off, const uint32_t* line_read,
                         uint64_t n_lines, uint32_t tile, const uint32_t* tile_off, uint32_t n_tok, void* raw_key, void* raw_val, uint64_t* ctr);
void launch_parse_heads(hipStream_t s, int grain, const void* raw_key, const void* raw_val, uint32_t n_tok, uint64_t n_reads, uint32_t* flag,
                        uint64_t* ctr);
void launch_parse_reduce(hipStream_t s, int grain, const void* raw_key, const void* raw_val, const uint32_t* flag, const uint32_t* place,
                         uint32_t n_tok, uint32_t n_rec, void* out, uint32_t* tax_out);

constexpr uint32_t kLcaTileMax = 1024, kLcaTile = 1024;
constexpr uint32_t kLcaCtrMissing = 0, kLcaCtrWalk = 1, kLcaCounters = 2;
uint32_t lca_tiles(uint64_t n, uint32_t tile);
void launch_lca_heads(hipStream_t s, int grain, const void* rec, uint32_t n, uint32_t tile, uint32_t* tile_cnt);
void launch_lca_min(hipStream_t s, int grain, const void* rec, uint32_t n, uint32_t tile, const uint32_t* tile_off, uint32_t n_slots, uint32_t* m,
                    void* out);
void launch_lca_span(hipStream_t s, int grain, const void* rec, uint32_t n, uint32_t tile, const uint32_t* tile_off, uint32_t n_slots,
                     const uint32_t* m, uint32_t slack, const uint32_t* u_tax, const uint32_t* u_node, uint32_t n_union, uint32_t* lo, uint32_t* hi,
                     uint64_t* ctr);
void launch_lca_walk(hipStream_t s, uint32_t n_slots, uint32_t n_nodes, uint32_t max_depth, const uint32_t* lo, const uint32_t* hi, const uint32_t* m,
                     const uint32_t* parent, const uint32_t* last, const uint32_t* tax, void* out, uint32_t* direct, uint64_t* ctr);
void launch_lca_clade(hipStream_t s, uint32_t n_nodes, const uint32_t* last, const uint32_t* prefix, uint32_t* clade);
void launch_dedup_hash(hipStream_t s, uint32_t n_reads, const uint32_t* read_off, const uint8_t* codes, uint64_t* hash);
void launch_dedup_insert(hipStream_t s, uint32_t n_reads, const uint32_t* read_off, const uint8_t* codes, const uint64_t* hash, uint32_t hash_bits,
                         uint64_t* table, uint32_t n_slots, uint32_t* slot_of, uint64_t* ctr);
void launch_dedup_resolve(hipStream_t s, uint32_t n_reads, const uint64_t* table, const uint32_t* slot_of, const uint32_t* src_map, uint64_t* words,
                          uint32_t* read, uint32_t* rep, uint64_t* ctr);
constexpr uint32_t kFanTileMax = 1024, kFanTile = 1024;
void launch_fan_count(hipStream_t s, int grain, uint32_t n_entries, const uint32_t* read, const uint32_t* rep, const void* rec, uint32_t n_rec,
                      uint32_t* first, uint32_t* cnt, uint64_t* ctr);
void launch_fan_write(hipStream_t s, int grain, uint32_t n_entries, const uint32_t* read, const uint32_t* first, const uint32_t* off, const void* rec,
                      uint32_t tile, uint32_t total, void* out);
constexpr int kPairBoth = 0, kPairEither = 1, kPairProper = 2;
constexpr uint32_t kPairTileMax = 1024, kPairTile = 1024, kPairLaneMax = 16, kPairLaneMaxMax = 1024;
constexpr uint32_t kPairCtrList = 0, kPairCtrBadEdit = 1, kPairCtrBeyond = 2, kPairCtrBoth = 3, kPairCtrOne = 4, kPairCtrJoined = 5, kPairCounters = 6;
uint32_t pair_tiles(uint64_t n, uint32_t tile);
void launch_pair_bounds(hipStream_t s, int grain, const void* rec, uint32_t n, uint64_t n_reads, uint32_t* off);
void launch_pair_join(hipStream_t s, int grain, int mode, const void* rec, uint32_t n, uint64_t n_reads, const uint32_t* off, uint32_t max_insert,
                      uint32_t unpaired, uint32_t lane_max, uint32_t* val, uint32_t* add, uint32_t* list, uint64_t* ctr);
void launch_pair_wave(hipStream_t s, int grain, int mode, const void* rec, uint32_t n, uint64_t n_reads, const uint32_t* off, uint32_t max_insert,
                      const uint32_t* list, const uint64_t* ctr, uint32_t* val, uint32_t* add);
void launch_pair_heads(hipStream_t s, int grain, const void* rec, uint32_t n, uint32_t tile, uint32_t* tile_cnt);
void launch_pair_min(hipStream_t s, int grain, const void* rec, uint32_t n, uint32_t tile, const uint32_t* tile_off, const uint32_t* val,
                     const uint32_t* add, uint32_t n_slots_cap, uint32_t* m, void* slot_rec);
void launch_pair_flags(hipStream_t s, const uint64_t* n_slots, uint32_t n_slots_cap, const void* slot_rec, uint32_t* m, uint32_t* flag_a, uint32_t* flag_b);
void launch_pair_write(hipStream_t s, const uint64_t* n_slots, uint32_t n_slots_cap, const void* slot_rec, const uint32_t* m, const uint32_t* pos_a,
                       const uint32_t* pos_b, uint32_t n_a, uint32_t n_b, void* out_a, void* out_b);
void launch_pair_stats(hipStream_t s, const uint32_t* off, uint64_t n_pairs, const void* out, uint32_t n_out, uint64_t* ctr);
constexpr uint32_t kCoverTileMax = 1024, kCoverTile = 1024, kCoverLaneMax = 8, kCoverLaneMaxMax = 1024, kCoverMinLane = 32;
constexpr uint32_t kCoverCtrUnknown = 0, kCoverCtrRange = 1, kCoverCtrBeyond = 2, kCoverCtrFirstBad = 3, kCoverCtrCounted = 4, kCoverCtrList = 5,
                   kCoverCounters = 6;
void launch_cover_min(hipStream_t s, const void* rec, uint32_t n, uint64_t n_reads, const uint32_t* off, uint32_t* m);
void launch_cover_map(hipStream_t s, const void* rec, uint32_t n, uint64_t n_reads, const uint32_t* m, uint32_t slack, const uint64_t* ref_key,
                      const uint32_t* ref_len, uint32_t n_refs, uint32_t* ref, uint32_t* head, uint64_t* ctr);
void launch_cover_mark(hipStream_t s, const void* rec, uint32_t n, const uint32_t* read_len, const uint32_t* ref, const uint32_t* run,
                       const uint32_t* ref_len, const uint32_t* word_off, uint32_t n_refs, uint32_t lane_max, uint64_t* bitmap, uint64_t* cnt,
                       uint32_t* run_hit, uint32_t* run_ref, uint32_t* list, uint64_t* ctr);
void launch_cover_wave(hipStream_t s, const void* rec, uint32_t n, const uint32_t* read_len, const uint32_t* ref, const uint32_t* ref_len,
                       const uint32_t* word_off, uint32_t n_refs, const uint32_t* list, const uint64_t* ctr, uint64_t* bitmap);
void launch_cover_reads(hipStream_t s, const uint64_t* n_runs, uint32_t n, const uint32_t* run_hit, const uint32_t* run_ref, uint32_t n_refs,
                        uint64_t* cnt);
void launch_cover_pop(hipStream_t s, const uint64_t* bitmap, uint32_t n_words, const uint32_t* word_off, uint32_t n_refs, uint32_t tile, uint64_t* cov);

}
```

Baseline: 439.8 million.

## Fetch reference text in Myers verify via quad-cooperative 64-byte sector loads

Pads the device text to 64-byte sectors. Adds a Myers kernel variant where each quad of lanes cooperatively loads four 64-byte sectors with 16-byte vector loads, then redistributes them with DPP quad permutes and byte-permute/alignbyte to form each lane's column stream. Per-lane statistics are gathered by wave ballots instead, and launch bounds ask for higher occupancy. This aims to replace scattered per-lane text reads with coalesced wide loads. It costs extra VGPRs and permute instructions, and the legacy path stays available through an environment variable.

```diff
diff --git a/include/mtsv_amd.h b/include/mtsv_amd.h
--- a/include/mtsv_amd.h
+++ b/include/mtsv_amd.h
@@ -111,6 +111,7 @@
 #define MTSV_DEVPART_BINS 4
 #define MTSV_DEVPART_BIN_END 5
 #define MTSV_DEVPART_BIN_LUT 6
+#define MTSV_DEVPART_TEXT_SECTORS 7
 typedef struct {
     uint32_t n, n_blocks;
     uint32_t C[5];
diff --git a/mtsv_tools_amd/__init__.py b/mtsv_tools_amd/__init__.py
--- a/mtsv_tools_amd/__init__.py
+++ b/mtsv_tools_amd/__init__.py
@@ -13,6 +13,7 @@
     DEVPART_HEADER,
     DEVPART_SA_SAMPLE,
     DEVPART_TEXT,
+    DEVPART_TEXT_SECTORS,
     DeviceHeader,
     GRAIN_LONG,
     GRAIN_TAXID,
diff --git a/mtsv_tools_amd/_lib.py b/mtsv_tools_amd/_lib.py
--- a/mtsv_tools_amd/_lib.py
+++ b/mtsv_tools_amd/_lib.py
@@ -21,7 +21,7 @@
 ASSIGN_OFF, ASSIGN_WITH_HITS, ASSIGN_ONLY = 0, 1, 2
 GRAIN_TAXID, GRAIN_TAXID_GI, GRAIN_LONG = 0, 1, 2
 KEEP_UNMATCHED, KEEP_MATCHED = 0, 1
-DEVPART_HEADER, DEVPART_BLOCKS, DEVPART_TEXT, DEVPART_SA_SAMPLE, DEVPART_BINS, DEVPART_BIN_END, DEVPART_BIN_LUT = range(7)
+DEVPART_HEADER, DEVPART_BLOCKS, DEVPART_TEXT, DEVPART_SA_SAMPLE, DEVPART_BINS, DEVPART_BIN_END, DEVPART_BIN_LUT, DEVPART_TEXT_SECTORS = range(8)
 
 
 class Params(C.Structure):
diff --git a/mtsv_tools_amd/csrc/batch.hip b/mtsv_tools_amd/csrc/batch.hip
--- a/mtsv_tools_amd/csrc/batch.hip
+++ b/mtsv_tools_amd/csrc/batch.hip
@@ -138,11 +138,13 @@
         if (const char* e = getenv("MTSV_TAIL_FROM_LIST")) tail_from_list = atoi(e) != 0;
         if (const char* e = getenv("MTSV_FUSED_CLEAR")) fused_clear = atoi(e) != 0;
         if (const char* e = getenv("MTSV_SEED_STAGE")) seed_tiles = strcmp(e, "legacy") != 0;
+        if (const char* e = getenv("MTSV_MYERS_FETCH")) myers_fetch_legacy = strcmp(e, "legacy") == 0;
     } else {
         myers_wgs_per_cu = parent->myers_wgs_per_cu;
         tail_from_list = parent->tail_from_list;
         fused_clear = parent->fused_clear;
         seed_tiles = parent->seed_tiles;
+        myers_fetch_legacy = parent->myers_fetch_legacy;
     }
     ev.create();
     for (int k = 1; k < n_lanes; k++) extra.emplace_back(new Batch(ix, di, ws_reads, 0, hit_cap_user, this));
diff --git a/mtsv_tools_amd/csrc/batch.hpp b/mtsv_tools_amd/csrc/batch.hpp
--- a/mtsv_tools_amd/csrc/batch.hpp
+++ b/mtsv_tools_amd/csrc/batch.hpp
@@ -96,6 +96,7 @@
     bool tail_from_list = true;
     bool fused_clear = true;
     bool seed_tiles = true;
+    bool myers_fetch_legacy = false;
     bool listed_zero = false;
     struct VerifyTurn {
         bool on = false;
diff --git a/mtsv_tools_amd/csrc/batch_pass.hip b/mtsv_tools_amd/csrc/batch_pass.hip
--- a/mtsv_tools_amd/csrc/batch_pass.hip
+++ b/mtsv_tools_amd/csrc/batch_pass.hip
@@ -239,7 +239,7 @@
     stats.n_rounds = 1;
     switch (pl.path) {
         case VerifyPath::kTiled: verify_tiled(ps, a); break;
-        case VerifyPath::kEditFirst: root()->verify_turn.note_grid(launch_edit_myers(stream, v, a, ps.total_hits, pl.pass_max_len, 0, root()->myers_wgs_per_cu)); break;
+        case VerifyPath::kEditFirst: root()->verify_turn.note_grid(launch_edit_myers(stream, v, a, ps.total_hits, pl.pass_max_len, 0, root()->myers_wgs_per_cu, false, root()->myers_fetch_legacy)); break;
         case VerifyPath::kRounds: verify_rounds(ps, a); break;
         case VerifyPath::kPacked: launch_evaluate(stream, v, a, ps.total_hits, pl.pass_max_len); break;
     }
@@ -340,7 +340,7 @@
     bd.und_list = (uint32_t*)d_hit_row.p;
     bd.und_slot = kCtrUndecided;
     bd.myers_ctr = (unsigned long long*)(d_counters.p + kCtrMyersColumns);
-    root()->verify_turn.note_grid(launch_edit_myers(stream, di->view, bd, r.items, ps.plan.pass_max_len, r.fused ? 3 : 2, root()->myers_wgs_per_cu));
+    root()->verify_turn.note_grid(launch_edit_myers(stream, di->view, bd, r.items, ps.plan.pass_max_len, r.fused ? 3 : 2, root()->myers_wgs_per_cu, false, root()->myers_fetch_legacy));
     HIP_CHECK(hipEventRecord(ev[kEvBoundEnd], stream));
     r.sw.worklist = bd.und_list;
     r.sw.wl_count_slot = kCtrUndecided;
@@ -390,7 +390,7 @@
     my.next_list = r.next_list;
     my.next_count = (uint32_t*)r.next_slot;
     my.myers_ctr = (unsigned long long*)(d_counters.p + kCtrMyersColumns);
-    if (!tail_empty) root()->verify_turn.note_grid(launch_edit_myers(stream, v, my, r.tail_items, max_len, 1, root()->myers_wgs_per_cu, r.tail_listed));
+    if (!tail_empty) root()->verify_turn.note_grid(launch_edit_myers(stream, v, my, r.tail_items, max_len, 1, root()->myers_wgs_per_cu, r.tail_listed, root()->myers_fetch_legacy));
     if (first) HIP_CHECK(hipEventRecord(ev[kEvEditEnd], stream));
     if (tail_empty) {
         h_counters.p[kCtrPassCount] = h_counters.p[kCtrNext0] = 0;
diff --git a/mtsv_tools_amd/csrc/capi.cpp b/mtsv_tools_amd/csrc/capi.cpp
--- a/mtsv_tools_amd/csrc/capi.cpp
+++ b/mtsv_tools_amd/csrc/capi.cpp
@@ -257,6 +257,7 @@
             break;
         case MTSV_DEVPART_BLOCKS: src = di->d_blocks, len = (uint64_t)v.n_blocks * sizeof(RankBlock); break;
         case MTSV_DEVPART_TEXT: src = di->d_text, len = di->text_bytes; break;
+        case MTSV_DEVPART_TEXT_SECTORS: src = di->d_text, len = di->text_alloc_bytes; break;
         case MTSV_DEVPART_SA_SAMPLE: src = di->d_sa_sample, len = di->sa_sample_bytes; break;
         case MTSV_DEVPART_BINS: src = di->d_bins, len = (uint64_t)v.n_bins * sizeof(DevBin); break;
         case MTSV_DEVPART_BIN_END: src = di->d_bin_end, len = (uint64_t)v.n_bins * 4; break;
diff --git a/mtsv_tools_amd/csrc/dev_index.hip b/mtsv_tools_amd/csrc/dev_index.hip
--- a/mtsv_tools_amd/csrc/dev_index.hip
+++ b/mtsv_tools_amd/csrc/dev_index.hip
@@ -199,7 +199,7 @@
         if (s != UINT64_MAX) sentinel_row = s;
     if (sentinel_row == UINT64_MAX) throw std::runtime_error("format: bwt holds no sentinel");
 
-    codes.assign(((uint64_t)n + 15) / 16 * 16 + 32, (uint8_t)7);
+    codes.assign(text_padded_bytes(n), (uint8_t)7);
     parallel_ranges(n, threads, [&](uint64_t lo, uint64_t hi, int) {
         for (uint64_t i = lo; i < hi; i++) codes[i] = (uint8_t)sym_code(hx.text[i]);
     });
@@ -260,14 +260,14 @@
         throw std::runtime_error("format: Occ checkpoint " + std::to_string(ctr[kPackCtrOccBadFirst]) + " disagrees with the bwt");
     if (!ctr[kPackCtrSentinels]) throw std::runtime_error("format: bwt holds no sentinel");
 
-    HIP_CHECK(hipMalloc((void**)&di.d_text, di.text_bytes));
-    di.bytes += di.text_bytes;
+    HIP_CHECK(hipMalloc((void**)&di.d_text, di.text_alloc_bytes));
+    di.bytes += di.text_alloc_bytes;
     d_raw_text.alloc(raw_bytes, "the raw text");
     t0 = now_ms();
     HIP_CHECK(hipMemcpy(d_raw_text.p, hx.text.data(), n, hipMemcpyHostToDevice));
     copy_ms += now_ms() - t0;
     HIP_CHECK(hipEventRecord(ev.e[5], 0));
-    launch_pack_text(0, d_raw_text.p, n, di.d_text, di.text_bytes);
+    launch_pack_text(0, d_raw_text.p, n, di.d_text, di.text_alloc_bytes);
     HIP_CHECK(hipGetLastError());
     HIP_CHECK(hipEventRecord(ev.e[6], 0));
     HIP_CHECK(hipEventSynchronize(ev.e[6]));
@@ -337,6 +337,7 @@
         di->bytes += bytes;
     };
     di->text_bytes = ((uint64_t)n + 15) / 16 * 16 + 32;
+    di->text_alloc_bytes = text_padded_bytes(n);
     di->sa_sample_bytes = samp.size() * 4;
     di->bin_lut_bytes = bin_lut.size() * 4;
     di->packed_on_device = on_device;
diff --git a/mtsv_tools_amd/csrc/dev_index.hpp b/mtsv_tools_amd/csrc/dev_index.hpp
--- a/mtsv_tools_amd/csrc/dev_index.hpp
+++ b/mtsv_tools_amd/csrc/dev_index.hpp
@@ -32,6 +32,7 @@
     uint32_t flags = 0;
     float accel_build_ms = 0.f;
     uint64_t text_bytes = 0, sa_sample_bytes = 0, bin_lut_bytes = 0;
+    uint64_t text_alloc_bytes = 0;
     bool packed_on_device = false;
     float pack_ms = 0.f, copy_ms = 0.f;
 
diff --git a/mtsv_tools_amd/csrc/dev_layout.hpp b/mtsv_tools_amd/csrc/dev_layout.hpp
--- a/mtsv_tools_amd/csrc/dev_layout.hpp
+++ b/mtsv_tools_amd/csrc/dev_layout.hpp
@@ -20,6 +20,8 @@
 struct DevBin {
     uint32_t start, end, tax_id, gi;
 };
+
+__host__ __device__ inline uint64_t text_padded_bytes(uint64_t n) { return (n + 63) / 64 * 64 + 64; }
 
 struct DevIndexView {
     const RankBlock* blocks;
diff --git a/mtsv_tools_amd/csrc/k_verify.hip b/mtsv_tools_amd/csrc/k_verify.hip
--- a/mtsv_tools_amd/csrc/k_verify.hip
+++ b/mtsv_tools_amd/csrc/k_verify.hip
@@ -1123,9 +1123,110 @@
     return r;
 }
 
+constexpr uint32_t kSectorNone = 0xffffffffu;
+constexpr uint32_t kSectorFill = 0x07070707u;
+
+template <int CTRL>
+__device__ inline uint32_t quad_perm(uint32_t v) {
+    return (uint32_t)__builtin_amdgcn_update_dpp(0, (int)v, CTRL, 0xf, 0xf, true);
+}
+
+struct Sector {
+    uint4 p0, p1, p2, p3;
+};
+
+__device__ inline Sector quad_fetch(const uint8_t* __restrict__ text, uint32_t code, uint32_t q) {
+    Sector D;
+#define MTSV_QUAD_FETCH(P, CTRL)                                                                                       \
+    {                                                                                                                  \
+        const uint32_t ci = quad_perm<CTRL>(code);                                                                     \
+        uint4 v = make_uint4(kSectorFill, kSectorFill, kSectorFill, kSectorFill);                                      \
+        if (ci != kSectorNone) v = *reinterpret_cast<const uint4*>(text + (ci & ~63u) + 16u * (q ^ ((ci & 1u) * 3u)));  \
+        D.P = v;                                                                                                       \
+    }
+    MTSV_QUAD_FETCH(p0, 0x00)
+    MTSV_QUAD_FETCH(p1, 0x55)
+    MTSV_QUAD_FETCH(p2, 0xAA)
+    MTSV_QUAD_FETCH(p3, 0xFF)
+#undef MTSV_QUAD_FETCH
+    return D;
+}
+
+__device__ inline Sector quad_transpose(Sector D, uint32_t q) {
+    const bool b0 = (q & 1u) != 0, b1 = (q & 2u) != 0;
+#define MTSV_QUAD_SWAP(A, B, f, CTRL, bit)                                         \
+    {                                                                              \
+        const uint32_t xa = quad_perm<CTRL>(D.A.f), xb = quad_perm<CTRL>(D.B.f);   \
+        const uint32_t na = bit ? xb : D.A.f, nb = bit ? D.B.f : xa;               \
+        D.A.f = na;                                                                \
+        D.B.f = nb;                                                                \
+    }
+#define MTSV_QUAD_STAGE(A, B, CTRL, bit) \
+    MTSV_QUAD_SWAP(A, B, x, CTRL, bit) MTSV_QUAD_SWAP(A, B, y, CTRL, bit) MTSV_QUAD_SWAP(A, B, z, CTRL, bit) MTSV_QUAD_SWAP(A, B, w, CTRL, bit)
+    MTSV_QUAD_STAGE(p0, p1, 0xB1, b0)
+    MTSV_QUAD_STAGE(p2, p3, 0xB1, b0)
+    MTSV_QUAD_STAGE(p0, p2, 0x4E, b1)
+    MTSV_QUAD_STAGE(p1, p3, 0x4E, b1)
+#undef MTSV_QUAD_STAGE
+#undef MTSV_QUAD_SWAP
+    return D;
+}
+
+__device__ inline uint4 piece_in_column_order(const uint4 t, uint32_t sel) {
+    return make_uint4(__builtin_amdgcn_perm(t.w, t.x, sel), __builtin_amdgcn_perm(t.z, t.y, sel), __builtin_amdgcn_perm(t.y, t.z, sel),
+                      __builtin_amdgcn_perm(t.x, t.w, sel));
+}
+__device__ inline Sector sector_in_column_order(const Sector T, uint32_t strand) {
+    const uint32_t sel = strand ? 0x04050607u : 0x03020100u;
+    Sector r;
+    r.p0 = piece_in_column_order(T.p0, sel);
+    r.p1 = piece_in_column_order(T.p1, sel);
+    r.p2 = piece_in_column_order(T.p2, sel);
+    r.p3 = piece_in_column_order(T.p3, sel);
+    return r;
+}
+
+template <int M>
+__device__ inline uint4 sector_cols(const Sector lo, const Sector hi, uint32_t boff) {
+    const uint32_t s4 = boff >> 4, dsel = (boff >> 2) & 3u, sh = boff & 3u;
+    auto pick = [s4](const uint4 p0, const uint4 p1, const uint4 p2, const uint4 p3) {
+        uint4 r;
+        r.x = s4 == 0 ? p0.x : s4 == 1 ? p1.x : s4 == 2 ? p2.x : p3.x;
+        r.y = s4 == 0 ? p0.y : s4 == 1 ? p1.y : s4 == 2 ? p2.y : p3.y;
+        r.z = s4 == 0 ? p0.z : s4 == 1 ? p1.z : s4 == 2 ? p2.z : p3.z;
+        r.w = s4 == 0 ? p0.w : s4 == 1 ? p1.w : s4 == 2 ? p2.w : p3.w;
+        return r;
+    };
+    uint4 a, b;
+    if constexpr (M == 0) {
+        a = pick(lo.p0, lo.p1, lo.p2, lo.p3);
+        b = pick(lo.p1, lo.p2, lo.p3, hi.p0);
+    } else if constexpr (M == 1) {
+        a = pick(lo.p1, lo.p2, lo.p3, hi.p0);
+        b = pick(lo.p2, lo.p3, hi.p0, hi.p1);
+    } else if constexpr (M == 2) {
+        a = pick(lo.p2, lo.p3, hi.p0, hi.p1);
+        b = pick(lo.p3, hi.p0, hi.p1, hi.p2);
+    } else {
+        a = pick(lo.p3, hi.p0, hi.p1, hi.p2);
+        b = pick(hi.p0, hi.p1, hi.p2, hi.p3);
+    }
+    const uint32_t e0 = dsel == 0 ? a.x : dsel == 1 ? a.y : dsel == 2 ? a.z : a.w;
+    const uint32_t e1 = dsel == 0 ? a.y : dsel == 1 ? a.z : dsel == 2 ? a.w : b.x;
+    const uint32_t e2 = dsel == 0 ? a.z : dsel == 1 ? a.w : dsel == 2 ? b.x : b.y;
+    const uint32_t e3 = dsel == 0 ? a.w : dsel == 1 ? b.x : dsel == 2 ? b.y : b.z;
+    const uint32_t e4 = dsel == 0 ? b.x : dsel == 1 ? b.y : dsel == 2 ? b.z : b.w;
+    uint4 r;
+    r.x = __builtin_amdgcn_alignbyte(e1, e0, sh);
+    r.y = __builtin_amdgcn_alignbyte(e2, e1, sh);
+    r.z = __builtin_amdgcn_alignbyte(e3, e2, sh);
+    r.w = __builtin_amdgcn_alignbyte(e4, e3, sh);
+    return r;
+}
+
 enum : int { MY_CHAIN = 0, MY_LIST = 1, MY_BOUND = 2, MY_FUSED = 3 };
-template <int W, int MODE>
-__global__ __launch_bounds__(256) void k_edit_myers(DevIndexView ix, EvalArgs a) {
+template <int W, int MODE, bool QUAD>
+__global__ __launch_bounds__(256, (QUAD && W <= 5) ? 5 : 1) void k_edit_myers(DevIndexView ix, EvalArgs a) {
     constexpr bool FUSED = MODE == MY_FUSED, LIST = MODE == MY_LIST || FUSED, BOUND = MODE == MY_BOUND;
     constexpr int NROW = (BOUND || LIST) ? 6 : 5;
     __shared__ uint32_t eq_tab[NROW][W][256];
@@ -1133,15 +1234,16 @@
     const uint32_t n_work = *a.wl_count;
     const uint32_t maxc = a.maxc;
     const uint32_t lane = lane_id();
-    uint32_t verified = 0, wbytes = 0;
-    uint32_t cols = 0, refuted = 0;
+    uint32_t wbytes = 0;
+    uint32_t cols = 0;
+    uint32_t verified = 0, refuted = 0, extra_passed = 0;
     uint32_t bnext = 0, bend = 0;
     bool active = false, exhausted = false;
     bool counted = false;
     uint32_t g = 0, o = 0, L = 0, ED = 0, strand = 0;
     bool thr_wrapped = false, hopeless = false;
     uint32_t pv0[W];
-    uint32_t ph = 0, extra_passed = 0;
+    uint32_t ph = 0;
     bool read_n = false;
     for (;;) {
         unsigned long long need = __ballot(!active);
@@ -1166,7 +1268,7 @@
                 const uint32_t rs = a.cand[g].w;
                 const uint32_t r_ = a.r0 + (rs >> 1);
                 strand = rs & 1;
-                o = a.strand_off[rs];
+                if (!QUAD) o = a.strand_off[rs];
                 const uint32_t b0 = a.read_off[r_];
                 L = a.read_off[r_ + 1] - b0;
                 ED = (uint32_t)ceil((double)L * a.edit_rate);
@@ -1214,74 +1316,147 @@
             if (exhausted) break;
             continue;
         }
+        bool verified_now = false, refuted_now = false, passed_now = false;
+        auto count_verified = [&]() { if (QUAD) verified_now = true; else verified++; };
+        auto count_refuted = [&]() { if (QUAD) refuted_now = true; else refuted++; };
+        auto count_passed = [&]() { if (QUAD) passed_now = true; else extra_passed++; };
         uint32_t verdict = 0, vg = 0;
-        if ((FUSED ? thr_wrapped : !LIST && hopeless) && active) {
+        const uint32_t* lane_tab = &eq_tab[0][0][tid];
+        auto columns16 = [&](const uint4 cur, const uint32_t lim, uint32_t (&Pv)[W], uint32_t (&Mv)[W], int& score, int& best) {
+#pragma unroll
+            for (int jj = 0; jj < 16; jj++) {
+                if ((uint32_t)jj < lim) {
+                    const uint32_t word = jj < 4 ? cur.x : jj < 8 ? cur.y : jj < 12 ? cur.z : cur.w;
+                    const uint32_t tc = (word >> ((jj & 3) * 8)) & 0xffu;
+                    const uint32_t* row = lane_tab + tc * (W * 256);
+                    uint32_t ph_below = 0, mh_below = 0;
+#pragma unroll
+                    for (int k = 0; k < W; k++) {
+                        const uint32_t Eq = row[k * 256];
+                        const uint32_t pv = Pv[k], mv = Mv[k];
+                        const uint32_t Xv = Eq | mv;
+                        const uint32_t Eqh = k ? (Eq | (mh_below >> 31)) : Eq;
+                        const uint32_t Xh = __builtin_amdgcn_bitop3_b32((Eqh & pv) + pv, pv, Eqh, 0xBE);
+                        const uint32_t Ph = mv | ~(Xh | pv);
+                        const uint32_t Mh = pv & Xh;
+                        const uint32_t Phs = k ? __builtin_amdgcn_alignbit(Ph, ph_below, 31) : (Ph << 1);
+                        const uint32_t Mhs = k ? __builtin_amdgcn_alignbit(Mh, mh_below, 31) : (Mh << 1);
+                        Pv[k] = Mhs | ~(Xv | Phs);
+                        Mv[k] = Phs & Xv;
+                        ph_below = Ph;
+                        mh_below = Mh;
+                    }
+                    const uint32_t hp = ph_below >> 31, hm = mh_below >> 31;
+                    score += (int)hp - (int)hm;
+                    best = min(best, score);
+                }
+            }
+        };
+        auto strand_base = [&](const uint4& cd) { return QUAD ? a.strand_off[cd.w] : o; };
+        const bool no_sweep = (FUSED ? thr_wrapped : !LIST && hopeless) && active;
+        const bool sweep = active && !no_sweep;
+        if (no_sweep) {
             const uint4 c = a.cand[g];
             if (!BOUND || !counted) {
-                verified++;
+                count_verified();
                 wbytes += c.y - c.x;
             }
             counted = false;
             a.cand_status[g] = 1;
             const uint32_t nxt = a.cand_next[g];
             if (nxt == 0xffffffffu || nxt >= maxc) active = false;
-            else g = o + nxt;
-        } else if (active) {
-            const uint4 c = a.cand[g];
-            uint32_t Pv[W], Mv[W];
-#pragma unroll
-            for (int k = 0; k < W; k++) {
-                Pv[k] = pv0[k];
-                Mv[k] = 0;
-            }
-            const uint32_t Wn = c.y - c.x;
-            int score = (int)L, best = (int)L;
-            const bool swm = BOUND || (LIST && ph == 1);
-            uint4 nxt4 = Wn ? fetch_cols(ix, c.x, c.y, strand, 0, swm) : make_uint4(0, 0, 0, 0);
-            const uint32_t* lane_tab = &eq_tab[0][0][tid];
-            uint32_t j0 = 0;
-            uint32_t win_n = 0;
-            for (; j0 < Wn; j0 += 16) {
-                if (swm) {
-                    if (BOUND && best <= (int)ED) break;
-                    if (best > 2 * (int)ED && score - (int)(Wn - j0) > 2 * (int)ED) break;
-                }
-                const uint4 cur = nxt4;
-                if (LIST) win_n |= cur.x | cur.y | cur.z | cur.w;
-                if (j0 + 16 < Wn) nxt4 = fetch_cols(ix, c.x, c.y, strand, j0 + 16, swm);
-                const uint32_t lim = min(16u, Wn - j0);
-#pragma unroll
-                for (int jj = 0; jj < 16; jj++) {
-                    if ((uint32_t)jj < lim) {
-                        const uint32_t word = jj < 4 ? cur.x : jj < 8 ? cur.y : jj < 12 ? cur.z : cur.w;
-                        const uint32_t tc = (word >> ((jj & 3) * 8)) & 0xffu;
-                        const uint32_t* row = lane_tab + tc * (W * 256);
-                        uint32_t ph_below = 0, mh_below = 0;
-#pragma unroll
-                        for (int k = 0; k < W; k++) {
-                            const uint32_t Eq = row[k * 256];
-                            const uint32_t pv = Pv[k], mv = Mv[k];
-                            const uint32_t Xv = Eq | mv;
-                            const uint32_t Eqh = k ? (Eq | (mh_below >> 31)) : Eq;
-                            const uint32_t Xh = __builtin_amdgcn_bitop3_b32((Eqh & pv) + pv, pv, Eqh, 0xBE);
-                            const uint32_t Ph = mv | ~(Xh | pv);
-                            const uint32_t Mh = pv & Xh;
-                            const uint32_t Phs = k ? __builtin_amdgcn_alignbit(Ph, ph_below, 31) : (Ph << 1);
-                            const uint32_t Mhs = k ? __builtin_amdgcn_alignbit(Mh, mh_below, 31) : (Mh << 1);
-                            Pv[k] = Mhs | ~(Xv | Phs);
-                            Mv[k] = Phs & Xv;
-                            ph_below = Ph;
-                            mh_below = Mh;
-                        }
-                        const uint32_t hp = ph_below >> 31, hm = mh_below >> 31;
-                        score += (int)hp - (int)hm;
-                        best = min(best, score);
-                    }
-                }
-            }
-            cols += min(j0, Wn);
+            else g = strand_base(c) + nxt;
+        }
+        uint4 c = make_uint4(0, 0, 0, 0);
+        if (sweep) c = a.cand[g];
+        uint32_t Pv[W], Mv[W];
+#pragma unroll
+        for (int k = 0; k < W; k++) {
+            Pv[k] = QUAD ? ~eq_tab[4][k][tid] : pv0[k];
+            Mv[k] = 0;
+        }
+        const uint32_t Wn = c.y - c.x;
+        int score = (int)L, best = (int)L;
+        const bool swm = BOUND || (LIST && ph == 1);
+        uint32_t win_n = 0;
+        uint32_t jstop = 0;
+        if constexpr (!QUAD) {
+            if (sweep) {
+                uint4 nxt4 = Wn ? fetch_cols(ix, c.x, c.y, strand, 0, swm) : make_uint4(0, 0, 0, 0);
+                uint32_t j0 = 0;
+                for (; j0 < Wn; j0 += 16) {
+                    if (swm) {
+                        if (BOUND && best <= (int)ED) break;
+                        if (best > 2 * (int)ED && score - (int)(Wn - j0) > 2 * (int)ED) break;
+                    }
+                    const uint4 cur = nxt4;
+                    if (LIST) win_n |= cur.x | cur.y | cur.z | cur.w;
+                    if (j0 + 16 < Wn) nxt4 = fetch_cols(ix, c.x, c.y, strand, j0 + 16, swm);
+                    columns16(cur, min(16u, Wn - j0), Pv, Mv, score, best);
+                }
+                jstop = j0;
+            }
+        } else {
+            const uint32_t q = lane & 3u;
+            const uint32_t first = strand ? c.y - 1u : c.x;
+            const uint32_t boff = strand ? 63u - (first & 63u) : first & 63u;
+            const uint32_t s0 = first >> 6, nblk = (Wn + 15u) >> 4;
+            const uint32_t nsec = nblk ? ((boff + 16u * nblk - 1u) >> 6) + 1u : 0u;
+            const uint32_t sec_end = (uint32_t)(text_padded_bytes(ix.n) >> 6);
+            bool run = sweep && Wn != 0;
+            auto sector_code = [&](uint32_t k) -> uint32_t {
+                if (!run || k >= nsec || (strand && k > s0)) return kSectorNone;
+                const uint32_t s = strand ? s0 - k : s0 + k;
+                return s < sec_end ? (s << 6) | strand : kSectorNone;
+            };
+            Sector lo = quad_fetch(ix.text, sector_code(0), q);
+            Sector hi = quad_fetch(ix.text, sector_code(1), q);
+            lo = sector_in_column_order(quad_transpose(lo, q), strand);
+            for (uint32_t j0 = 0;; j0 += 16) {
+                if (run) {
+                    bool stop = j0 >= Wn;
+                    if (!stop && swm) {
+                        if (BOUND && best <= (int)ED) stop = true;
+                        else if (best > 2 * (int)ED && score - (int)(Wn - j0) > 2 * (int)ED) stop = true;
+                    }
+                    if (stop) {
+                        run = false;
+                        cols += min(j0, Wn);
+                    }
+                }
+                if (!__any(run)) break;
+                const uint32_t m = (j0 >> 4) & 3u;
+                if (m == 0) {
+                    hi = sector_in_column_order(quad_transpose(hi, q), strand);
+                }
+                uint4 cur;
+                if (m == 0) cur = sector_cols<0>(lo, hi, boff);
+                else if (m == 1) cur = sector_cols<1>(lo, hi, boff);
+                else if (m == 2) cur = sector_cols<2>(lo, hi, boff);
+                else cur = sector_cols<3>(lo, hi, boff);
+                cur.x = swm ? clamp_codes_sw(cur.x) : clamp_codes4(cur.x);
+                cur.y = swm ? clamp_codes_sw(cur.y) : clamp_codes4(cur.y);
+                cur.z = swm ? clamp_codes_sw(cur.z) : clamp_codes4(cur.z);
+                cur.w = swm ? clamp_codes_sw(cur.w) : clamp_codes4(cur.w);
+                if (m == 3) {
+                    lo = hi;
+                    hi = quad_fetch(ix.text, sector_code((j0 >> 6) + 2u), q);
+                }
+                if (run) {
+                    if (LIST) win_n |= cur.x | cur.y | cur.z | cur.w;
+                    columns16(cur, min(16u, Wn - j0), Pv, Mv, score, best);
+                }
+            }
+        }
+        if constexpr (QUAD) {
+            uint32_t g_again = g;
+            asm volatile("" : "+v"(g_again));
+            if (sweep) c = a.cand[g_again];
+        }
+        if (sweep) {
+            if (!QUAD) cols += min(jstop, Wn);
             if (LIST ? ph == 1 : (!BOUND || !counted)) {
-                verified++;
+                count_verified();
                 wbytes += Wn;
             }
             counted = false;
@@ -1296,19 +1471,19 @@
                     vg = g;
                     active = false;
                 } else {
-                    refuted++;
+                    count_refuted();
                     a.cand_status[g] = 1;
                     const uint32_t nxt = a.cand_next[g];
                     if (nxt == 0xffffffffu || nxt >= maxc) active = false;
-                    else g = o + nxt;
+                    else g = strand_base(c) + nxt;
                 }
             } else if (LIST && ph == 1) {
                 if (ed > 2 * ED) {
-                    if (FUSED) refuted++;
+                    if (FUSED) count_refuted();
                     a.cand_status[g] = 1;
                     const uint32_t nxt = a.cand_next[g];
                     if (nxt == 0xffffffffu || nxt >= maxc) active = false;
-                    else g = o + nxt;
+                    else g = strand_base(c) + nxt;
                 } else if (ed > ED) {
                     if (FUSED) {
                         verdict = 2;
@@ -1317,7 +1492,7 @@
                     }
                     active = false;
                 } else {
-                    extra_passed++;
+                    count_passed();
                     if (!read_n || !(win_n & 0x04040404u)) {
                         const DevBin bin = ix.bins[c.z];
                         a.out[g] = make_uint4(bin.tax_id, bin.gi, c.x >= bin.start ? c.x - bin.start : 0, ed);
@@ -1339,7 +1514,7 @@
                 const uint32_t nxt = a.cand_next[g];
                 if (nxt == 0xffffffffu || nxt >= maxc) active = false;
                 else {
-                    g = o + nxt;
+                    g = strand_base(c) + nxt;
                     if (LIST) ph = 1;
                 }
             }
@@ -1361,7 +1536,13 @@
                 if (verdict == 2) a.und_list[base + (uint32_t)__popcll(um & lower)] = (FUSED ? g : vg) | kSweepFlag;
             }
         }
-    }
+        if constexpr (QUAD) {
+            verified += (uint32_t)__popcll(__ballot(verified_now));
+            if (BOUND || FUSED) refuted += (uint32_t)__popcll(__ballot(refuted_now));
+            if (LIST) extra_passed += (uint32_t)__popcll(__ballot(passed_now));
+        }
+    }
+    if (QUAD && lane) verified = refuted = extra_passed = 0;
     unsigned long long v64 = verified, w64 = wbytes;
     for (int d = 32; d > 0; d >>= 1) {
         v64 += __shfl_down(v64, d);
@@ -1537,19 +1718,24 @@
 }
 
 uint32_t launch_edit_myers(hipStream_t s, const DevIndexView& ix, const EvalArgs& a_, uint64_t max_items, uint32_t max_len,
-                           int mode, uint32_t wgs_per_cu, bool listed) {
+                           int mode, uint32_t wgs_per_cu, bool listed, bool legacy_fetch) {
     EvalArgs a = a_;
     a.maxc = rank_bound(a.max_candidates);
     if (!a.planes || a.plane_words != myers_words(max_len)) throw std::runtime_error("internal: k_edit_myers needs the pass's read planes");
     const uint32_t resident = 256 * std::max<uint32_t>(1, std::min<uint32_t>(wgs_per_cu, kMyersWgsPerCuMax));
     uint32_t blocks = std::max<uint32_t>(16, std::min<uint32_t>(cdiv(max_items, listed ? 256 : 4096), resident));
     const uint32_t W = myers_words(max_len);
-#define MYERS_CASE(WW)                                                                                   \
+#define MYERS_FETCH_CASE(WW, Q)                                                                              \
     do {                                                                                                 \
-        if (mode == MY_LIST) hipLaunchKernelGGL((k_edit_myers<WW, MY_LIST>), dim3(blocks), dim3(256), 0, s, ix, a);        \
-        else if (mode == MY_FUSED) hipLaunchKernelGGL((k_edit_myers<WW, MY_FUSED>), dim3(blocks), dim3(256), 0, s, ix, a); \
-        else if (mode == MY_BOUND) hipLaunchKernelGGL((k_edit_myers<WW, MY_BOUND>), dim3(blocks), dim3(256), 0, s, ix, a); \
-        else hipLaunchKernelGGL((k_edit_myers<WW, MY_CHAIN>), dim3(blocks), dim3(256), 0, s, ix, a);                      \
+        if (mode == MY_LIST) hipLaunchKernelGGL((k_edit_myers<WW, MY_LIST, Q>), dim3(blocks), dim3(256), 0, s, ix, a);        \
+        else if (mode == MY_FUSED) hipLaunchKernelGGL((k_edit_myers<WW, MY_FUSED, Q>), dim3(blocks), dim3(256), 0, s, ix, a); \
+        else if (mode == MY_BOUND) hipLaunchKernelGGL((k_edit_myers<WW, MY_BOUND, Q>), dim3(blocks), dim3(256), 0, s, ix, a); \
+        else hipLaunchKernelGGL((k_edit_myers<WW, MY_CHAIN, Q>), dim3(blocks), dim3(256), 0, s, ix, a);                      \
+    } while (0)
+#define MYERS_CASE(WW)                              \
+    do {                                            \
+        if (legacy_fetch) MYERS_FETCH_CASE(WW, false); \
+        else MYERS_FETCH_CASE(WW, true);            \
     } while (0)
     if (W == 2) MYERS_CASE(2);
     else if (W == 3) MYERS_CASE(3);
@@ -1559,6 +1745,7 @@
     else if (W == 7) MYERS_CASE(7);
     else MYERS_CASE(8);
 #undef MYERS_CASE
+#undef MYERS_FETCH_CASE
     return blocks;
 }
 
diff --git a/mtsv_tools_amd/csrc/kernels.hpp b/mtsv_tools_amd/csrc/kernels.hpp
--- a/mtsv_tools_amd/csrc/kernels.hpp
+++ b/mtsv_tools_amd/csrc/kernels.hpp
@@ -133,7 +133,7 @@
                        const uint4* cand, unsigned long long* out);
 constexpr uint32_t kMyersWgsPerCuMax = 5;
 uint32_t launch_edit_myers(hipStream_t s, const DevIndexView& ix, const EvalArgs& a, uint64_t max_items, uint32_t max_len,
-                           int mode = 0, uint32_t wgs_per_cu = kMyersWgsPerCuMax, bool listed = false);
+                           int mode = 0, uint32_t wgs_per_cu = kMyersWgsPerCuMax, bool listed = false, bool legacy_fetch = false);
 void launch_sw_pairs(hipStream_t s, const DevIndexView& ix, const EvalArgs& a, uint64_t max_items, uint32_t max_len,
                      bool diag = true, bool top = false, bool sparse = false);
 void launch_sw_diag(hipStream_t s, const DevIndexView& ix, const EvalArgs& a, uint64_t max_items, uint32_t max_len,
```

After: 448.7 million (median of 6 runs). 2.0% higher.
